# lachinov/brats2019

Measured on AMD Instinct MI355X. Metric: volumes_per_sec_fwd_bwd_128cubed_x4ch, higher is better.
Workload: dtype bf16

## Files before the change

brats2019_amd/_lib.py:

```python
from __future__ import annotations

import ctypes as C
import os

import torch

_PKG = os.path.dirname(os.path.abspath(__file__))
LIB_PATH = os.environ.get("RU_LIB_PATH") or os.path.join(_PKG, "lib", "libresunet_hip.so")

_lib = None
PRECISIONS = {"f32": 0, "bf16x3": 1}
GRAD_PRECISIONS = {"bf16x3": 1, "bf16": 2}
FUSE_GN_BWD_STATS, FUSE_GN_BWD_APPLY, FUSE_SIDE_STREAM, FUSE_BATCH_WREDUCE, FUSE_TAIL_FINALIZE, FUSE_PW_DGRAD = 1, 2, 4, 8, 16, 32

_vp, _f, _d, _i, _sz = C.c_void_p, C.c_float, C.c_double, C.c_int, C.c_size_t

SIGNATURES = {
    "ru_last_error": (C.c_char_p, []),
    "ru_version": (_i, []),
    "ru_device_ok": (_i, []),
    "ru_conv3d_workspace_bytes": (_sz, [_i] * 7),
    "ru_conv3d_fwd": (_i, [_vp, _vp, _vp, _vp] + [_i] * 7 + [_vp, _sz, _vp]),
    "ru_conv3d_bwd_data": (_i, [_vp, _vp, _vp] + [_i] * 7 + [_vp, _sz, _vp]),
    "ru_conv3d_fwd_p": (_i, [_vp, _vp, _vp, _vp] + [_i] * 8 + [_vp, _sz, _vp]),
# ... 65 lines not shown
    "ru_unet_probe": (_i, [_vp, _i]),
    "ru_unet_probe_read": (_i, [_vp, C.POINTER(C.c_double), C.POINTER(_i)]),
    "ru_unet_probe_read_families": (_i, [_vp, C.POINTER(C.c_double), C.POINTER(_i), _i]),
    "ru_unet_param_count": (_i, [_vp]),
    "ru_unet_param_name": (C.c_char_p, [_vp, _i]),
    "ru_unet_param_ndim": (_i, [_vp, _i]),
    "ru_unet_param_dim": (_i, [_vp, _i, _i]),
    "ru_unet_param_offset": (_sz, [_vp, _i]),
    "ru_unet_param_total": (_sz, [_vp]),
    "ru_unet_param_is_dead": (_i, [_vp, _i]),
    "ru_unet_workspace_bytes": (_sz, [_vp] + [_i] * 5),
    "ru_unet_forward": (_i, [_vp, _vp, _vp, _vp] + [_i] * 5 + [_vp, _sz, _vp]),
    "ru_unet_backward": (_i, [_vp] * 6),
    "ru_unet_backward_criterion": (_i, [_vp, _vp, _vp, _vp, _d, _f, _f, _f, _f, _vp, _vp, _vp]),
    "ru_unet_gn_stats": (_i, [_vp, _i, _vp, _vp, _vp]),
    "ru_comm_unique_id": (_i, [_vp]),
    "ru_comm_init": (_i, [C.POINTER(_vp), _vp, _i, _i]),
    "ru_comm_destroy": (_i, [_vp]),
    "ru_comm_rank": (_i, [_vp]),
    "ru_comm_world": (_i, [_vp]),
    "ru_allreduce": (_i, [_vp, _vp, _sz, _i, _vp]),
    "ru_comm_group_begin": (_i, []),
    "ru_comm_group_end": (_i, []),
    "ru_tta_merge": (_i, [_vp, _i, C.c_uint, _vp, _vp, _vp, _i, _i, _i, _i, _vp]),
    "ru_compose_labels": (_i, [_vp, _vp, C.c_ulonglong, _vp, _sz, _vp]),
    "ru_dice_counts": (_i, [_vp, _vp, _vp, _i, _i, _sz, _vp]),
    "ru_dice_accumulate": (_i, [_vp, _vp, _i, _i, _i, _vp]),
    "ru_hausdorff_workspace_bytes": (_sz, [_i] * 6),
    "ru_hausdorff_sq": (_i, [_vp, _vp] + [_i] * 6 + [_vp, _vp, _sz, _vp]),
    "ru_hausdorff_accumulate": (_i, [_vp, _vp] + [_i] * 4 + [_vp]),
    "ru_label_confusion": (_i, [_vp, _vp, _i, _i, _i, _sz, _vp, _vp, _vp]),
    "ru_overlap_accumulate": (_i, [_vp, _i, _i, _i, _i, _vp, _vp, _vp]),
    "ru_dice1d_accumulate": (_i, [_vp, _vp, _i, _i, _i, _vp]),
    "ru_rmse_accumulate": (_i, [_vp, _vp, _vp]),
    "ru_surface_workspace_bytes": (_sz, [_i] * 6),
    "ru_surface_metrics": (_i, [_vp, _vp] + [_i] * 6 + [_d, _vp, _vp, _vp, _sz, _vp]),
    "ru_surface_accumulate": (_i, [_vp, _vp] + [_i] * 4 + [_vp]),
    "ru_lesion_workspace_bytes": (_sz, [_i] * 7),
    "ru_lesion_metrics": (_i, [_vp, _vp] + [_i] * 7 + [C.c_longlong, _d, _vp, _vp, _vp, _i, _vp, _sz, _vp]),
    "ru_lesion_accumulate": (_i, [_vp, _vp] + [_i] * 4 + [_vp]),
    "ru_tile_gather": (_i, [_vp, _vp] + [_i] * 6 + [C.POINTER(_i), _i, _i, _i, _vp]),
    "ru_tile_scatter": (_i, [_vp, _vp] + [_i] * 6 + [C.POINTER(_i), _i, _i, _i, C.POINTER(_i), C.POINTER(_i), _vp]),
    "ru_blend_accumulate": (_i, [_vp, _vp, _vp] + [_i] * 8 + [C.POINTER(_i), _i, C.POINTER(_i), _i, C.POINTER(_i), _i, _i, _i, _vp]),
    "ru_blend_finalize": (_i, [_vp, _vp, _vp] + [_i] * 8 + [C.POINTER(_i), _i, C.POINTER(_i), _i, C.POINTER(_i), _i, _vp]),
    "ru_case_bbox": (_i, [_vp, _vp, _i, _i, _i, _i, _vp]),
    "ru_case_workspace_bytes": (_sz, [_i, _i, _i, _i]),
    "ru_case_stats": (_i, [_vp, _vp, _i, _i, _i, _i, C.POINTER(_i), C.POINTER(_i), _vp, _sz, _vp]),
    "ru_case_prepare": (_i, [_vp, _vp, _vp, _i, _i, _i, _i, C.POINTER(_i), C.POINTER(_i), C.POINTER(_i), C.POINTER(_i), _i, C.c_uint, _vp]),
    "ru_tta_merge_box": (_i, [_vp, _i, C.c_uint, _vp, _vp, _vp, _i, _i, _i, _i, C.POINTER(_i), C.POINTER(_i), _vp]),
    "ru_cc_workspace_bytes": (_sz, [_i, _i, _i]),
    "ru_cc_reject": (_i, [_vp, _i, _i, _i, _d, _vp, _sz, _vp]),
    "ru_paste_labels": (_i, [_vp, _vp, _i, _i, _i, C.POINTER(_i), C.POINTER(_i), _vp]),
    "ru_postprocess_workspace_bytes": (_sz, [_i, _i, _i, _i]),
    "ru_postprocess_regions": (_i, [_vp, _vp, _i, _i, _i, _i, C.POINTER(C.c_longlong), C.POINTER(C.c_ulonglong), C.c_uint, C.c_uint, _i, _vp, _vp, _vp, _vp, _sz, _vp]),
    "ru_ens_accumulate": (_i, [_vp, _i, C.c_uint, _vp, _i, _i, _i, _i, _i, C.POINTER(_i), C.POINTER(_i), _vp]),
    "ru_ens_finalize": (_i, [_vp, _i, _vp, _vp, _vp, _i, _sz, _vp]),
    "ru_ens_accumulate_finalize": (_i, [_vp, _i, C.c_uint, _vp, _i, _i, _vp, _vp, _vp, _i, _i, _i, _i, C.POINTER(_i), C.POINTER(_i), _vp]),
    "ru_ens_argmax": (_i, [_vp, _i, _vp, _i, _sz, _vp]),
    "ru_paste_probs": (_i, [_vp, _vp, _i, _i, _i, _i, C.POINTER(_i), C.POINTER(_i), _vp]),
    "ru_unc_accumulate": (_i, [_vp, _i, C.c_uint, _vp, _vp, _i, _i, _i, _i, _i, C.POINTER(_i), C.POINTER(_i), _vp]),
    "ru_unc_accumulate_finalize": (_i, [_vp, _i, C.c_uint, _vp, _vp, _i, _i, _i, _vp, _vp, _vp, _vp, _i, _i, _i, _i, C.POINTER(_i), C.POINTER(_i), _vp]),
    "ru_unc_finalize": (_i, [_vp, _vp, _i, _i, _i, _vp, _vp, _vp, _vp, _i, _sz, _vp]),
    "ru_unc_histogram": (_i, [_vp, _vp, _vp, _i, _i, _i, _vp, _vp, _vp]),
    "ru_unc_score": (_i, [_vp, C.POINTER(_i), _i, _vp, _vp, _vp]),
    "ru_paste_u8c": (_i, [_vp, _vp, _i, _i, _i, _i, C.POINTER(_i), C.POINTER(_i), _vp]),
    "ru_zscore_workspace_bytes": (_sz, [_i, _sz]),
    "ru_zscore_stats": (_i, [_vp, _vp, _i, _sz, _vp, _sz, _vp]),
    "ru_augment_patch": (_i, [_vp, _vp, _vp, _vp, _i, _i, _i, _i, _vp, _vp, _vp, _i, _vp, _vp, _vp, _vp, _vp]),
    "ru_augment_patch_soft": (_i, [_vp, _vp, _vp, _vp, _vp, _i, _i, _i, _i, _vp, _vp, _vp, _i, _vp, _vp, _vp, _vp, _vp]),
    "ru_augment_patch_affine": (_i, [_vp, _vp, _vp, _vp, _vp, _i, _i, _i, _i, _vp, _vp, _vp, _i, _vp, _vp, _i, _vp, _vp, _vp]),
    "ru_case_probe": (_i, [_vp, _vp, _vp, _i, _i, _i, _i, _vp, _vp]),
    "ru_case_pack": (_i, [_vp, _vp, _vp, _i, _i, _i, _i, _vp, _vp, _i, _vp, _vp, _vp, _vp]),
    "ru_case_unpack": (_i, [_vp, _vp, _vp, _i, _i, _i, _i, _i, _vp, _vp, _vp, _vp, _vp, _vp]),
    "ru_augment_batch_packed": (_i, [_vp, _vp, _i, _vp, _vp, _vp, _vp]),
    "ru_elastic_workspace_bytes": (_sz, [_i, _i, _i]),
    "ru_elastic_noise": (_i, [C.c_ulonglong, _i, _i, _i, _vp, _vp]),
    "ru_elastic_field": (_i, [_vp, _d, _d, _i, _i, _i, _vp, _vp, _sz, _vp]),
    "ru_elastic_warp": (_i, [_vp, _i, _vp, _i, _vp, _i, _i, _i, _i, _vp, _vp, _vp, _vp, _vp]),
    "ru_intensity_workspace_bytes": (_sz, [_i, _i, _i, _i]),
    "ru_intensity_augment": (_i, [_vp, _vp, _i, _i, _i, _i, _vp, _vp, _sz, _vp]),
    "ru_layout_convert": (_i, [_vp, _vp, _i, _i, _sz, _i, _vp]),
    "ru_upsample2x_trilinear_fwd_l": (_i, [_vp, _vp] + [_i] * 5 + [_f, _vp]),
    "ru_upsample2x_trilinear_bwd_l": (_i, [_vp, _vp] + [_i] * 5 + [_vp]),
    "ru_conv3d_fwd_l": (_i, [_vp, _vp, _vp, _vp] + [_i] * 7 + [_vp, _sz, _vp]),
    "ru_conv3d_bwd_weight_l": (_i, [_vp, _vp, _vp] + [_i] * 7 + [_vp, _sz, _vp]),
    "ru_conv1_l_workspace_bytes": (_sz, [_i, _i, _i]),
    "ru_conv1_l": (_i, [_vp, _i, _vp, _i, _vp, _i, _vp, _vp, _i, _vp, _f, _vp, _f, _i, _i, _sz, _i, _i, _i, _i, _vp, _vp, _f, _vp, _sz,
                        C.POINTER(_i), C.POINTER(_i), _vp, _sz, _vp]),
    "ru_conv3_l_workspace_bytes": (_sz, [_i] * 7),
    "ru_conv3_l": (_i, [_vp, _vp, _vp, _vp] + [_i] * 8 + [_vp, _vp, _vp, _f, _vp, _vp, _i, _i, _vp, _vp, _f, _vp, _sz, C.POINTER(_i), C.POINTER(_i), _vp, _sz, _vp, _vp]),
    "ru_gn_finalize_l": (_i, [_vp, _i] + [_vp] * 7 + [_i, _i, _sz, _i, _f, _i, _vp]),
    "ru_gn_apply_l": (_i, [_vp] * 7 + [_i, _i, _sz, _f, _f, _vp]),
    "ru_gn_bwd_finalize_l": (_i, [_vp, _i] + [_vp] * 6 + [_i, _i, _sz, _i, _i, _vp]),
    "ru_gn_bwd_l_nblk": (_i, [_sz]),
    "ru_gn_bwd_l_workspace_bytes": (_sz, [_i, _i, _sz]),
    "ru_gn_bwd_l": (_i, [_vp] * 7 + [_f] + [_vp] * 5 + [_i, _i, _sz, _i, _i, _vp, _sz, _vp]),
    "ru_head_grad_l_workspace_bytes": (_sz, [_i, _i, _sz, _i]),
    "ru_head_grad_l": (_i, [_vp] * 4 + [_d, _f, _f, _f, _f] + [_vp] * 3 + [_i, _i, _sz, _i, _vp, _sz, _vp]),
    "ru_wgrad1_l_workspace_bytes": (_sz, [_i, _i, _i, _sz]),
    "ru_wgrad3_l_workspace_bytes": (_sz, [_i] * 7),
    "ru_wgrad3_l": (_i, [_vp, _vp, _vp] + [_i] * 8 + [_vp, _vp, _f, _i, _i, _vp, _vp, _vp, _vp, _vp, _f, _vp, C.POINTER(_i), _vp, _sz, _vp]),
    "ru_wgrad1_l": (_i, [_vp, _vp, _i, _vp, _vp, _i, _i, _i, _i, _sz] + [_i] * 6 + [_vp, _i, _vp, _vp, _f, C.POINTER(_i), _vp, _sz, _vp]),
}


CRIT_KINDS = {"Dice_loss_joint": 0, "BCE_Loss": 1, "MSE_Loss": 2, "CE_Loss": 3, "Dice1D": 4, "GDL_joint": 5, "sens_loss_joint": 6,
              "Dice_loss_separate": 7}
CRIT_MOMENTS, CRIT_MAX_TERMS = 7, 8
CRIT_MASK_LOGS, CRIT_MASK_ALL = (1 << 4) | (1 << 5), 0x7F
CRIT_M_D2 = 6

CONF_PROB, CONF_LABEL, OVERLAP_MAX_LABELS = 0, 1, 8
OVERLAP_MODES = {"itk": 0, "wt": 1, "validate": 2}

UNC_MEASURES = {"std": 0, "entropy": 1}
UNC_REGIONS, UNC_LEVELS, UNC_CLASSES = 3, 101, 4

SURFACE_PROB, SURFACE_LABEL, SURFACE_REGIONS, SURFACE_COUNTS = 0, 1, 3, 6
SURFACE_COLUMNS = {"dice": 0, "sensitivity": 1, "specificity": 2, "hd95": 3}

LESION_COUNTS, LESION_TABLE_COLUMNS, LESION_CHUNK = 6, 5, 8
LESION_COLUMNS = {"dice": 0, "hd95": 1}

POSTPROCESS_MASKS, POSTPROCESS_LABELS, POSTPROCESS_REGIONS, POSTPROCESS_STATS = 0, 1, 3, 6


INT_BLUR, INT_LOWRES, INT_NOISE, INT_BRIGHTNESS, INT_CONTRAST, INT_GAMMA, INT_GAMMA_INVERT, INT_GAMMA_RETAIN = 1, 2, 4, 8, 16, 32, 64, 128
INT_MAXC, INT_MAX_RADIUS = 8, 8


AFFINE_MAPPINGS = {"default": 0, "row": 1, "brick": 2}


PACK_F32, PACK_U16 = 0, 1
PACK_KINDS = {"float32": PACK_F32, "uint16": PACK_U16}
AUG_ZOOM, AUG_AFFINE = 0, 1
AUG_BATCH_MAX = 8


class FinDesc(C.Structure):
    _fields_ = [("kind", _i), ("G", _i), ("s2_sign", _i), ("keep_ticket", _i), ("eps", _f), ("nblk", _i), ("N", _i), ("C", _i),
                ("gamma", _vp), ("beta", _vp), ("mean", _vp), ("rstd", _vp), ("scale", _vp), ("shift", _vp), ("bst_k", _vp),
                ("coef", _vp), ("dgamma", _vp), ("dbeta", _vp)]


class CaseDesc(C.Structure):
    _fields_ = [("image", _vp), ("label", _vp), ("soft", _vp), ("kind", _i), ("C", _i), ("dims", _i * 3), ("box_lo", _i * 3), ("box_size", _i * 3),
                ("mean", _f * 8), ("inv_std", _f * 8)]


class PatchDesc(C.Structure):
    _fields_ = [("mode", _i), ("flags", _i), ("mapping", _i), ("crop_lo", _i * 3), ("scale", _d * 3), ("matrix", _d * 9), ("offset", _d * 3),
                ("gain", _f * 8), ("bias", _f * 8)]


class IntensityParams(C.Structure):
    _fields_ = [("mask", _i * 8), ("blur_sigma", _d * 8), ("lowres_zoom", _d * 8), ("noise_variance", _d * 8), ("noise_seed", C.c_ulonglong * 8),
                ("brightness", _d * 8), ("contrast", _d * 8), ("gamma", _d * 8)]


class CritTerm(C.Structure):
    _fields_ = [("kind", _i), ("weight", _d), ("priority", _d), ("bg_weight", _d)]


def load():
    global _lib
# ... 57 lines not shown
```

brats2019_amd/csrc/engine.hip:

```cpp
#include "ru_common.h"
#include "arena.hpp"

#include <vector>
#include <math.h>
#include <stdlib.h>
#include <string.h>

#include <string>
#include <type_traits>

namespace ru {

static thread_local char g_err[512] = "";
void set_error(const char* fmt, ...) {
    va_list ap;
    va_start(ap, fmt);
    vsnprintf(g_err, sizeof(g_err), fmt, ap);
    va_end(ap);
}
int hip_fail(hipError_t e, const char* what) {
    set_error("%s: %s", what, hipGetErrorString(e));
    return RU_EHIP;
}

constexpr float kSlope = 1e-2f;
constexpr int kGroups = 8;
constexpr float kEps = 1e-5f;
constexpr int kInCh = 4;

static bool env_is(const char* name, char c) { const char* e = getenv(name); return e && *e == c; }
Switches switches_from_env() {
    Switches sw;
    sw.wz = !env_is("RU_WZ", '0');
    sw.wz32 = !(conv3_wz16_form_built() && env_is("RU_WZ32", '0'));
    sw.mx = !env_is("RU_MX", '0');
    sw.mx_wz = sw.mx && !env_is("RU_MX", '1');
    sw.mxg = !env_is("RU_MXG", '0');
    sw.head_form = !env_is("RU_HEAD_FORM", '0');
    sw.head_res = !env_is("RU_HEAD_RES", '0');
    return sw;
}
bool env_trace() { static const bool on = [] { const char* e = getenv("RU_TRACE"); return e && *e && *e != '0'; }(); return on; }
bool env_f32c_off() { static const bool off = env_is("RU_F32C", '0'); return off; }
bool env_sb1_no22() { static const bool on = env_is("RU_SB1_NO22", '1'); return on; }
int env_c1_scatter_cob() { static const int forced = [] { const char* e = getenv("RU_C1_SCATTER_COB"); return e ? atoi(e) : 0; }(); return forced; }
bool env_c1_pair_off() { static const bool off = env_is("RU_C1_PAIR", '0'); return off; }
unsigned env_fusion(unsigned fusion) {
    if (env_is("RU_SIDE_STREAM", '0')) fusion &= ~(unsigned)RU_FUSE_SIDE_STREAM;
    if (const char* e = getenv("RU_FUSION_OFF")) fusion &= ~(unsigned)strtoul(e, nullptr, 0);
    if (const char* e = getenv("RU_FUSION_ON")) fusion |= (unsigned)strtoul(e, nullptr, 0) & 63u;
    return fusion;
}

static int trace_sync(const char* what, hipStream_t s) {
    fprintf(stderr, "[ru] %s\n", what);
    const hipError_t e = hipStreamSynchronize(s);
    if (e != hipSuccess) { fprintf(stderr, "[ru]   -> %s\n", hipGetErrorString(e)); return hip_fail(e, what); }
    return RU_OK;
}

enum { FAM_CONV_L0 = 0, FAM_CONV_DEEP, FAM_WGRAD_L0, FAM_WGRAD_DEEP, FAM_GN, FAM_PW, FAM_OTHER, FAM_COUNT };
enum { INST_CONV16_FWD = 0, INST_CONV16_DGRAD, INST_CONV_DEEP_FWD, INST_CONV_DEEP_DGRAD, INST_WGRAD16_FUSED, INST_WGRAD16_PLAIN, INST_WGRAD_DEEP, INST_COUNT };
struct FamilySink {
    std::vector<hipEvent_t> ev;
    std::vector<int> fam;
    std::vector<int> inst;
    size_t used = 0;
    ~FamilySink() { for (hipEvent_t e : ev) (void)hipEventDestroy(e); }
};
static thread_local FamilySink* t_sink = nullptr;
static thread_local int t_hint_c = 16;
static thread_local int t_hint_inst = -1;
struct RedQueues { WgradRedList main, side; hipStream_t side_stream = nullptr; };
static thread_local RedQueues* t_red = nullptr;
static WgradRedList* red_for(hipStream_t s) { return t_red ? ((t_red->side_stream && s == t_red->side_stream) ? &t_red->side : &t_red->main) : nullptr; }
static int family_of(const char* call) {
    auto has = [&](const char* k) { return strstr(call, k) != nullptr; };
    if (has("wgrad3_launch")) return t_hint_c <= 16 ? FAM_WGRAD_L0 : FAM_WGRAD_DEEP;
    if (has("wgrad_reduce_flush")) return FAM_WGRAD_DEEP;
    if (has("conv3_launch") || has("conv3_sb_launch")) return t_hint_c <= 16 ? FAM_CONV_L0 : FAM_CONV_DEEP;
    if (has("gn_")) return FAM_GN;
    if (has("conv1_") || has("wgrad1_launch") || has("up2_") || has("s2d_launch") || has("d2s_launch") || has("lrelu_bwd_launch")) return FAM_PW;
    return FAM_OTHER;
}
static void sink_begin(const char* call, hipStream_t s) {
    FamilySink& k = *t_sink;
    while (k.ev.size() < k.used + 2) {
        hipEvent_t e;
        if (hipEventCreate(&e) != hipSuccess) return;
        k.ev.push_back(e);
    }
    if (k.fam.size() < k.ev.size() / 2) { k.fam.resize(k.ev.size() / 2); k.inst.resize(k.ev.size() / 2); }
    k.fam[k.used / 2] = family_of(call);
    k.inst[k.used / 2] = t_hint_inst;
    t_hint_inst = -1;
    (void)hipEventRecord(k.ev[k.used], s);
}
static void sink_end(hipStream_t s) {
    FamilySink& k = *t_sink;
    if (k.ev.size() < k.used + 2) return;
    (void)hipEventRecord(k.ev[k.used + 1], s);
    k.used += 2;
}

template <class F>
static int run_probed(const char* call, hipStream_t s, F&& launch) {
    if (t_sink) sink_begin(call, s);
    const int rc = launch();
    if (t_sink) sink_end(s);
    if (rc != RU_OK) return rc;
    return env_trace() ? trace_sync(call, s) : RU_OK;
}
#define RU_RUN(call) RU_ARENA_RUN(run_probed(#call, s, [&] { return (call); }))

}

using namespace ru;

struct ParamInfo {
    std::string name;
    int ndim;
    int dims[5];
    size_t offset, numel;
    bool dead;
};

struct PackRef { size_t off = 0; unsigned forms = 0; };

struct BlockP {
    int down = -1, conv1 = -1, conv2 = -1, n1w = -1, n1b = -1, n2w = -1, n2b = -1;
    int cin_down = 0, c = 0;
    size_t pk_f1 = 0, pk_f2 = 0, pk_d1 = 0, pk_d2 = 0, pk_downT = 0, pk_down16 = 0;
    PackRef fk_f1, fk_f2, fk_d1, fk_d2;
};

struct GNSave {
    float *mean = nullptr, *rstd = nullptr, *scale = nullptr, *shift = nullptr;
    float act_slope = 0.01f;
    float* k = nullptr;
};

struct BlockSave {
    const BlockP* bp = nullptr;
    const float* xprev = nullptr;
    const BlockSave* xprev_block = nullptr;
    float* xs2d = nullptr;
    const float* x = nullptr;
    const GNSave* xg = nullptr;
    float *y1 = nullptr, *y2 = nullptr, *out = nullptr;
    GNSave g1, g2;
    int N = 0, C = 0, D = 0, H = 0, W = 0;
};

struct DecSave {
    const float* z = nullptr;
    const BlockSave* z_block = nullptr;
    float *u = nullptr, *v = nullptr, *c = nullptr;
    const float* skip = nullptr;
    int level = 0;
};

constexpr int kOneProduct = 0x100;
struct ru_unet {
    int depth = 0, nout = 0;
    std::vector<int> enc, dec, ch;
    std::vector<ParamInfo> params;
    size_t total = 0;
    std::vector<std::vector<BlockP>> enc_blocks, dec_blocks;
    std::vector<BlockP> first_blocks;
    std::vector<int> up_w, dec1_w;
    std::vector<size_t> pk_upT, pk_decT;
    int conv_in = -1, nin_w = -1, nin_b = -1, conv_out_w = -1, conv_out_b = -1;
    size_t pk_in = 0, pk_out = 0, pk_out_d = 0, pk_total = 0;
    PackRef fk_in, fk_out, fk_out_d;
    size_t fk_total = 0;
    void set_pack(Conv3Args& a, const PackRef& r) const { conv3_set_pack(a, fpack + r.off, r.forms); }
    int precision = RU_PREC_F32;
    unsigned fusion = RU_FUSE_GN_BWD_STATS | RU_FUSE_GN_BWD_APPLY | RU_FUSE_SIDE_STREAM | RU_FUSE_BATCH_WREDUCE | RU_FUSE_PW_DGRAD;
    int grad_precision = RU_PREC_BF16X3;
    int grad_products() const { return (precision == RU_PREC_BF16X3 && grad_precision == RU_PREC_BF16) ? 1 : 3; }
    int wgrad_mode() const { return precision | (grad_products() == 1 ? kOneProduct : 0); }
    bool c16 = false;
    char* fpack = nullptr;

    bool have_fwd = false, training = false;
    int N = 0, D = 0, H = 0, W = 0;
    char* ws = nullptr;
    size_t ws_bytes = 0, fwd_end = 0, fwd_keep = 0;
    float* pack = nullptr;
    const float* x_in = nullptr;
    const float* x_in4 = nullptr;
    bool x_in4_planned = false;
    bool params_frozen = false;
    const float* packed_params = nullptr;
    const void* packed_base = nullptr;
    int packed_prec = -1;
    bool packed_c16 = false;
    ru::Switches sw;
    ru::Switches pack_sw;
    float *y0 = nullptr, *t0 = nullptr, *probs = nullptr;
    GNSave g0;
    const float* head_in = nullptr;
    const BlockSave* head_block = nullptr;
    std::vector<BlockSave> first_s;
    std::vector<std::vector<BlockSave>> enc_s, dec_s;
    std::vector<DecSave> dstage;
    std::vector<const float*> skips;
    std::vector<GNSave> gn_order;
    bool probe_on = false;
    bool probe_families = false;
    ru::FamilySink* sink = nullptr;
    std::vector<hipEvent_t> probe_ev;
    size_t probe_used = 0;
    hipStream_t side = nullptr;
    std::vector<hipEvent_t> fork_ev;
    ru::RedQueues red;
    unsigned* tickets = nullptr;
    int ticket_next = 0;
    unsigned* next_ticket() { return tickets ? tickets + (ticket_next++ & 255) : nullptr; }
    bool tails() const { return c16 && (fusion & RU_FUSE_TAIL_FINALIZE) && tickets != nullptr; }
    size_t fork_used = 0;
    ~ru_unet() {
        for (hipEvent_t e : probe_ev) (void)hipEventDestroy(e);
        for (hipEvent_t e : fork_ev) (void)hipEventDestroy(e);
        if (side) (void)hipStreamDestroy(side);
        if (tickets) (void)hipFree(tickets);
        delete sink;
    }
};

static int add_param(ru_unet* h, const std::string& name, std::initializer_list<int> dims, bool dead = false) {
    ParamInfo p;
    p.name = name;
    p.ndim = (int)dims.size();
    size_t n = 1;
    int i = 0;
    for (int d : dims) { p.dims[i++] = d; n *= (size_t)d; }
    for (; i < 5; ++i) p.dims[i] = 1;
    p.offset = h->total;
    p.numel = n;
    p.dead = dead;
    h->total += n;
    h->params.push_back(p);
    return (int)h->params.size() - 1;
}

static BlockP add_block(ru_unet* h, const std::string& prefix, int cin_down, int c, bool dead = false) {
    BlockP b;
    b.c = c;
    b.cin_down = cin_down;
    if (cin_down > 0) b.down = add_param(h, prefix + "downsample.0.weight", {c, cin_down, 2, 2, 2}, dead);
    b.conv1 = add_param(h, prefix + "conv1.conv1.weight", {c, c, 3, 3, 3}, dead);
    b.conv2 = add_param(h, prefix + "conv2.conv1.weight", {c, c, 3, 3, 3}, dead);
    b.n1w = add_param(h, prefix + "norm1.weight", {c}, dead);
    b.n1b = add_param(h, prefix + "norm1.bias", {c}, dead);
    b.n2w = add_param(h, prefix + "norm2.weight", {c}, dead);
    b.n2b = add_param(h, prefix + "norm2.bias", {c}, dead);
    return b;
}

static std::string fmt(const char* f, int a, int b = 0) {
    char buf[128];
    snprintf(buf, sizeof(buf), f, a, b);
    return buf;
}

static void assign_block_packs(ru_unet* h, BlockP& b) {
    const size_t n = conv3_packed_floats(b.c, b.c);
    b.pk_f1 = h->pk_total; h->pk_total += n;
    b.pk_f2 = h->pk_total; h->pk_total += n;
    b.pk_d1 = h->pk_total; h->pk_total += n;
    b.pk_d2 = h->pk_total; h->pk_total += n;
    if (b.down >= 0) {
        b.pk_downT = h->pk_total; h->pk_total += (size_t)8 * b.cin_down * b.c;
        b.pk_down16 = h->pk_total; h->pk_total += (size_t)2 * 8 * b.cin_down * b.c;
    }
    const size_t f = conv3_sb_frag_bytes(b.c, b.c);
    for (PackRef* r : {&b.fk_f1, &b.fk_f2, &b.fk_d1, &b.fk_d2}) { r->off = h->fk_total; h->fk_total += f; }
}

extern "C" ru_unet_t ru_unet_create(int depth, const int* encoder_layers, const int* decoder_layers,
                                    const int* number_of_channels, int number_of_outputs) {
    if (depth < 2 || depth > 8 || !encoder_layers || !decoder_layers || !number_of_channels || number_of_outputs < 1) {
        set_error("ru_unet_create: bad configuration");
        return nullptr;
    }
    for (int i = 0; i < depth; ++i) {
        if (number_of_channels[i] % kGroups != 0 || number_of_channels[i] <= 0 || encoder_layers[i] < 1 || decoder_layers[i] < 1) {
            set_error("ru_unet_create: channels must be positive multiples of 8 (GroupNorm(8, C)) and layer counts >= 1");
            return nullptr;
        }
    }
    ru_unet* h = new ru_unet();
    h->fusion = env_fusion(h->fusion);
    h->depth = depth;
    h->nout = number_of_outputs;
    h->enc.assign(encoder_layers, encoder_layers + depth);
    h->dec.assign(decoder_layers, decoder_layers + depth);
    h->ch.assign(number_of_channels, number_of_channels + depth);
    const std::vector<int>& ch = h->ch;
    h->enc_blocks.resize(depth - 1);
    for (int i = 0; i < depth - 1; ++i)
        for (int j = 0; j < h->enc[i + 1]; ++j)
            h->enc_blocks[i].push_back(add_block(h, fmt("encoder_convs.%d.%d.", i, j), j == 0 ? ch[i] : 0, ch[i + 1]));
    for (int i = 0; i < depth - 1; ++i) h->up_w.push_back(add_param(h, fmt("upsampling.%d.1.weight", i), {ch[i], ch[i + 1], 1, 1, 1}));
    h->dec_blocks.resize(depth);
    for (int i = 0; i < depth; ++i)
        for (int j = 0; j < h->dec[i]; ++j)
            h->dec_blocks[i].push_back(add_block(h, fmt("decoder_convs.%d.%d.", i, j), 0, ch[i], i == depth - 1));
    for (int i = 0; i < depth; ++i)
        h->dec1_w.push_back(add_param(h, fmt("decoder_convs1x1.%d.weight", i), {ch[i], 2 * ch[i], 1, 1, 1}, i == depth - 1));
    h->conv_in = add_param(h, "conv_input.weight", {ch[0], kInCh, 3, 3, 3});
    h->nin_w = add_param(h, "norm_input.weight", {ch[0]});
// ... 282 lines not shown
    for (int i = 0; i < depth; ++i) { Dl[i] = h->D >> i; Hl[i] = h->H >> i; Wl[i] = h->W >> i; }
    auto Vl = [&](int i) { return (size_t)Dl[i] * Hl[i] * Wl[i]; };
    h->gn_order.clear();
    const bool f32c_off = env_f32c_off();
    const bool f32c_fits = (size_t)h->D * h->H * h->W * 64 < ((size_t)1 << 31);
    h->c16 = (h->precision == RU_PREC_BF16X3 || (h->precision == RU_PREC_F32 && !h->training && !f32c_off && f32c_fits)) && (h->W & 3) == 0;
    for (int c : h->ch) h->c16 = h->c16 && (c % 16 == 0);
    h->pack = A.alloc(h->pk_total);
    h->fpack = reinterpret_cast<char*>(A.alloc(h->fk_total / sizeof(float) + 64));
    float* wf4_in = A.alloc(conv3_sb4_frag_bytes(h->ch[0]) / sizeof(float) + 64);
    const bool reuse_packs = h->params_frozen && !h->training && !A.dry && h->packed_params == params && h->packed_base == (const void*)h->pack &&
                             h->packed_prec == h->precision && h->packed_c16 == h->c16;
    int rc = RU_OK;
    if (!reuse_packs) {
        rc = pack_all(h, params, A, s);
        if (rc) return rc;
    }

    const int C0 = h->ch[0];
    const BlockSave* res_block = nullptr;
    h->x_in = x;
    h->x_in4 = nullptr;
    h->x_in4_planned = false;
    h->y0 = A.alloc((size_t)N * C0 * Vl(0));
    const size_t stem_mark = A.off;
    if (h->c16 && h->precision == RU_PREC_BF16X3 && conv3_sb4_usable(N, kInCh, C0, Dl[0], Hl[0], Wl[0])) {
        float* x4 = A.alloc((size_t)N * 4 * Vl(0));
        float* wf4 = wf4_in;
        h->x_in4 = x4;
        h->x_in4_planned = true;
        RU_RUN(pad_to_c4_launch(x, x4, N, kInCh, Vl(0), s));
        if (!reuse_packs) RU_RUN(conv3_sb4_pack_weights(P(h, params, h->conv_in), wf4, kInCh, C0, 0, s));
        rc = conv3_gn(h, A, s, x4, nullptr, wf4, PACK_HAS_SB4, h->y0, nullptr, P(h, params, h->nin_w), P(h, params, h->nin_b), h->g0,
                      N, kInCh, C0, Dl[0], Hl[0], Wl[0], false, true);
    } else {
        rc = conv3_gn(h, A, s, x, h->pack + h->pk_in, h->fpack + h->fk_in.off, h->fk_in.forms, h->y0, nullptr, P(h, params, h->nin_w), P(h, params, h->nin_b), h->g0, N, kInCh, C0, Dl[0], Hl[0], Wl[0], false);
    }
    if (rc) return rc;
    if (!h->training) A.rewind(stem_mark);
    h->g0.act_slope = 1.0f;
    const bool stem_fused = h->c16 && !h->first_blocks.empty() && h->first_blocks[0].down < 0;
    h->t0 = nullptr;
    if (!stem_fused) {
        h->t0 = A.alloc((size_t)N * C0 * Vl(0));
        if (h->c16) RU_RUN(gn_apply16_launch(h->y0, h->g0.scale, h->g0.shift, nullptr, h->t0, N, C0, Vl(0), 1.0f, s));
        else RU_RUN(gn_apply_launch(h->y0, h->g0.scale, h->g0.shift, nullptr, h->t0, N, C0, Vl(0), 1.0f, s));
    }
    const float* cur = stem_fused ? h->y0 : h->t0;
    const BlockSave* cur_block = nullptr;
    h->first_s.assign(h->first_blocks.size(), BlockSave());
    for (size_t j = 0; j < h->first_blocks.size(); ++j) {
        rc = block_fwd(h, params, A, s, h->first_blocks[j], cur, cur_block, N, Dl[0], Hl[0], Wl[0], h->first_s[j], &cur, (stem_fused && j == 0) ? &h->g0 : nullptr);
        if (rc) return rc;
        cur_block = &h->first_s[j];
    }
    h->skips.assign(depth - 1, nullptr);
    h->enc_s.assign(depth - 1, {});
    for (int i = 0; i < depth - 1; ++i) {
        h->skips[i] = cur;
        h->enc_s[i].assign(h->enc_blocks[i].size(), BlockSave());
        for (size_t j = 0; j < h->enc_blocks[i].size(); ++j) {
            const int lv = j == 0 ? i : i + 1;
            rc = block_fwd(h, params, A, s, h->enc_blocks[i][j], cur, cur_block, N, Dl[lv], Hl[lv], Wl[lv], h->enc_s[i][j], &cur);
            if (rc) return rc;
            cur_block = &h->enc_s[i][j];
        }
    }
    h->dstage.assign(depth - 1, DecSave());
    h->dec_s.assign(depth - 1, {});
    for (int i = depth - 2; i >= 0; --i) {
        DecSave& ds = h->dstage[i];
        ds.level = i;
        ds.z = cur;
        ds.z_block = cur_block;
        ds.skip = h->skips[i];
        const int Ci = h->ch[i], Cc = h->ch[i + 1];
        const bool recycle = !h->training;
        float* c_early = recycle ? A.alloc((size_t)N * Ci * Vl(i)) : nullptr;
        const size_t dmark = A.off;
        if (!h->c16) {
            ds.u = A.alloc((size_t)N * Cc * Vl(i));
            RU_RUN(up2_fwd_launch(cur, ds.u, N, Cc, Dl[i + 1], Hl[i + 1], Wl[i + 1], s));
        }
        ds.v = A.alloc((size_t)N * Ci * Vl(i));
        Conv1Args c1{};
        c1.x0 = ds.u; c1.C0 = Cc; c1.y = ds.v; c1.out_slope = kSlope;
        c1.N = N; c1.Cout = Ci; c1.V = Vl(i);
        ds.c = recycle ? c_early : A.alloc((size_t)N * Ci * Vl(i));
        Conv1Args c2{};
        c2.x0 = ds.skip; c2.C0 = Ci; c2.x1 = ds.v; c2.C1 = Ci;
        c2.y = ds.c; c2.out_slope = 1.f; c2.N = N; c2.Cout = Ci; c2.V = Vl(i);
        if (h->c16) {
            float* zc = A.alloc((size_t)N * Ci * Vl(i + 1));
            c1.x0 = cur; c1.y = zc; c1.out_slope = 1.f; c1.V = Vl(i + 1);
            c1.wT = P(h, params, h->up_w[i]); c1.ldw = Cc;
            RU_RUN(conv1_16_launch(c1, s));
            RU_RUN(up2_fwd16_launch(zc, ds.v, N, Ci, Dl[i + 1], Hl[i + 1], Wl[i + 1], kSlope, s));
            c2.wT = P(h, params, h->dec1_w[i]); c2.ldw = 2 * Ci;
            RU_RUN(conv1_16_launch(c2, s));
        } else {
            c1.wT = h->pack + h->pk_upT[i]; c1.ldw = Ci;
            RU_RUN(conv1_launch(c1, s));
            c2.wT = h->pack + h->pk_decT[i]; c2.ldw = Ci;
            RU_RUN(conv1_launch(c2, s));
        }
        if (recycle) A.rewind(dmark);
        cur = ds.c;
        cur_block = nullptr;
        h->dec_s[i].assign(h->dec_blocks[i].size(), BlockSave());
        for (size_t j = 0; j < h->dec_blocks[i].size(); ++j) {
            const bool defer = i == 0 && j + 1 == h->dec_blocks[i].size() && h->c16 &&
                               (h->precision == RU_PREC_BF16X3 ? conv3_sb_head_takes_residual(h->sw, N, C0, h->nout, Dl[0], Hl[0], Wl[0])
                                                               : (!h->training && conv3_f32c_head_takes_residual(h->sw, C0, h->nout, Wl[0])));
            rc = block_fwd(h, params, A, s, h->dec_blocks[i][j], cur, cur_block, N, Dl[i], Hl[i], Wl[i], h->dec_s[i][j], &cur, nullptr, defer);
            if (rc) return rc;
            cur_block = &h->dec_s[i][j];
            if (defer) res_block = cur_block;
        }
    }
    h->head_in = cur;
    h->head_block = cur_block;
    t_hint_c = C0;
    float* pdst = probs_out;
    h->probs = probs_out;
    Conv3Args a{};
    a.x = cur; a.wp = h->pack + h->pk_out; a.bias = P(h, params, h->conv_out_b); a.y = pdst; a.sigmoid = 1;
    a.mode = h->precision; h->set_pack(a, h->fk_out); a.in_c16 = h->c16;
    a.N = N; a.Cin = C0; a.Cout = h->nout; a.D = Dl[0]; a.H = Hl[0]; a.W = Wl[0];
    if (res_block) {
        a.x = res_block->y2; a.in_scale = res_block->g2.scale; a.in_shift = res_block->g2.shift; a.in_slope = kSlope; a.in_res = res_block->x;
        a.in_sum_out = res_block->out;
    }
    RU_RUN(conv3_launch(a, h->sw, s));
    if (!A.dry) { h->packed_params = h->training ? nullptr : params; h->packed_base = h->pack; h->packed_prec = h->precision; h->packed_c16 = h->c16; h->pack_sw = h->sw; }
    return RU_OK;
}

struct NormRef {
    const float* y = nullptr;
    const GNSave* g = nullptr;
    float slope = kSlope;
    const float* gamma = nullptr;
    float *dgamma = nullptr, *dbeta = nullptr;
    int C = 0;
};
static NormRef norm1_of(const ru_unet* h, const float* params, float* grads, const BlockSave& b) {
    return {b.y1, &b.g1, kSlope, P(h, params, b.bp->n1w), G(h, grads, b.bp->n1w), G(h, grads, b.bp->n1b), b.C};
}
static NormRef norm2_of(const ru_unet* h, const float* params, float* grads, const BlockSave& b) {
    return {b.y2, &b.g2, kSlope, P(h, params, b.bp->n2w), G(h, grads, b.bp->n2w), G(h, grads, b.bp->n2b), b.C};
}
static NormRef norm_input_of(const ru_unet* h, const float* params, float* grads) {
    return {h->y0, &h->g0, 1.0f, P(h, params, h->nin_w), G(h, grads, h->nin_w), G(h, grads, h->nin_b), h->ch[0]};
}

struct FusedSums { float* part = nullptr; int nblk = 0; float* coef = nullptr; bool done = false; };
struct Grad { const float* d = nullptr; FusedSums sums; };

static void fill_bwd_tail(ru_unet* h, FinTail& f, const FusedSums& fs, const NormRef& n, size_t V, int s2_sign) {
    f.ticket = h->next_ticket(); f.kind = 2; f.nblk = fs.nblk; f.N = h->N; f.C = n.C; f.G = kGroups; f.V = V; f.eps = kEps; f.s2_sign = s2_sign;
    f.gamma = n.gamma; f.mean = n.g->mean; f.rstd = n.g->rstd; f.coef = fs.coef; f.dgamma = n.dgamma; f.dbeta = n.dbeta;
}

static int bst_nblk(const ru_unet* h, const Conv3Args& a) { return sb_nblk(h, a); }
static int bst_nblk(const ru_unet*, const Conv1Args& a) { return conv1_16_bst_nblk(a); }
template <class Args>
static FusedSums take_bwd_sums(ru_unet* h, Arena& A, Args& a, const NormRef& n, bool may) {
    FusedSums fs;
    if (!may) return fs;
    a.bst_y = n.y; a.bst_k = n.g->k; a.bst_slope = n.slope;
    fs.nblk = bst_nblk(h, a);
    fs.part = A.alloc((size_t)h->N * n.C * fs.nblk * 2);
    fs.coef = A.alloc((size_t)h->N * n.C * 3);
    a.stat_partials = fs.part;
    if constexpr (std::is_same<Args, Conv3Args>::value) {
        if (!A.dry && h->tails()) {
            fill_bwd_tail(h, a.fin, fs, n, (size_t)a.D * a.H * a.W, 1);
            fs.done = true;
        }
    }
// ... 382 lines not shown
            if (rc) return rc;
        }
        if (!joined) {
            const size_t n = (size_t)N * h->ch[i] * level_voxels(h, i);
            float* sum = A.alloc(n);
            RU_RUN(add_launch(g.d, dskip[i], sum, n, s));
            g = Grad{sum};
        }
    }
    for (int j = (int)h->first_s.size() - 1; j >= 0; --j) {
        const NormRef prev = fed_by(h->first_s[j]);
        rc = block_bwd(h, params, grads, A, s, h->first_s[j], g, &prev);
        if (rc) return rc;
    }
    rc = stem_bwd(h, params, grads, dx_in, A, s, g);
    if (rc) return rc;
    if (t_red && !t_red->side.e.empty()) RU_RUN(wgrad_reduce_flush(t_red->side, h->side));
    if (!A.dry) { rc = side_join(h, s); if (rc) return rc; }
    if (t_red && !t_red->main.e.empty()) RU_RUN(wgrad_reduce_flush(t_red->main, s));
    return RU_OK;
}

static int check_dims(ru_unet* h, int N, int D, int H, int W) {
    const int m = 1 << (h->depth - 1);
    RU_REQUIRE(N > 0 && D > 0 && H > 0 && W > 0, "ru_unet: bad extents");
    RU_REQUIRE(D % m == 0 && H % m == 0 && W % m == 0, "ru_unet: D,H,W must be divisible by %d (model.py:361 stride-2 convs)", m);
    return RU_OK;
}

extern "C" size_t ru_unet_workspace_bytes(ru_unet_t h, int N, int D, int H, int W, int training) {
    if (!h || check_dims(h, N, D, H, W) != RU_OK) return 0;
    ru_unet tmp = *h;
    tmp.probe_ev.clear();
    tmp.probe_on = false;
    tmp.sink = nullptr;
    tmp.side = nullptr;
    tmp.tickets = nullptr;
    tmp.fork_ev.clear();
    tmp.N = N; tmp.D = D; tmp.H = H; tmp.W = W; tmp.training = training != 0;
    tmp.sw = switches_from_env();
    Arena A;
    A.dry = true;
    if (unet_forward_impl(&tmp, nullptr, nullptr, nullptr, A, nullptr) != RU_OK) return 0;
    if (training) {
        if (unet_backward_impl(&tmp, nullptr, nullptr, nullptr, (float*)1, A, nullptr) != RU_OK) return 0;
    }
    return A.need() + 4096;
}

extern "C" int ru_unet_forward(ru_unet_t h, const float* params, const float* x, float* probs, int N, int D, int H, int W, int training,
                               void* ws, size_t ws_bytes, ru_stream_t stream) {
    RU_REQUIRE(h && params && x && probs && ws, "ru_unet_forward: null argument");
    int rc = check_dims(h, N, D, H, W);
    if (rc) return rc;
    h->have_fwd = false;
    h->sw = switches_from_env();
    h->N = N; h->D = D; h->H = H; h->W = W; h->training = training != 0;
    h->ws = (char*)ws; h->ws_bytes = ws_bytes;
    Arena A;
    A.dry = false; A.base = (char*)ws; A.cap = ws_bytes;
    if (!h->tickets && (h->fusion & RU_FUSE_TAIL_FINALIZE)) {
        hipError_t e = hipMalloc((void**)&h->tickets, 256 * sizeof(unsigned));
        if (e != hipSuccess) { h->tickets = nullptr; return hip_fail(e, "ru_unet_forward: ticket words"); }
    }
    if (h->tickets && (h->fusion & RU_FUSE_TAIL_FINALIZE)) {
        hipError_t e = hipMemsetAsync(h->tickets, 0, 256 * sizeof(unsigned), (hipStream_t)stream);
        if (e != hipSuccess) return hip_fail(e, "ru_unet_forward: ticket words");
    }
    h->ticket_next = 0;
    ru::t_sink = h->probe_families ? h->sink : nullptr;
    rc = unet_forward_impl(h, params, x, probs, A, (hipStream_t)stream);
    ru::t_sink = nullptr;
    if (rc) return rc;
    if (A.failed) { set_error("ru_unet_forward: workspace too small (%zu bytes given)", ws_bytes); return RU_ENOMEM; }
    h->fwd_end = A.off;
    h->fwd_keep = A.keep;
    h->have_fwd = true;
    return RU_OK;
}

static int backward_entry(ru_unet_t h, const float* params, const float* dprobs, const CritGradArgs* crit, float* grads, float* dx, ru_stream_t stream) {
    if (!h->have_fwd || !h->training) { set_error("ru_unet_backward: needs a preceding training-mode ru_unet_forward"); return RU_ESTATE; }
    h->sw = switches_from_env();
    RU_REQUIRE(h->precision != RU_PREC_BF16X3 || h->pack_sw.pack_bits() == h->sw.pack_bits(),
               "ru_unet_backward: RU_WZ / RU_MX / RU_MXG changed since the forward whose packs this backward reads (signature %d then, %d now)", h->pack_sw.pack_bits(), h->sw.pack_bits());
    Arena A;
    A.dry = false; A.base = h->ws; A.cap = h->ws_bytes; A.off = h->fwd_end; A.keep = h->fwd_keep;
    ru::t_sink = h->probe_families ? h->sink : nullptr;
    h->red.main.e.clear();
    h->red.side.e.clear();
    ru::t_red = (h->fusion & RU_FUSE_BATCH_WREDUCE) && !env_trace() ? &h->red : nullptr;
    int rc = unet_backward_impl(h, params, dprobs, grads, dx, A, (hipStream_t)stream, crit);
    ru::t_red = nullptr;
    ru::t_sink = nullptr;
    if (rc && h->side) {
        (void)side_join(h, (hipStream_t)stream);
        h->fork_used = 0;
    }
    if (rc) return rc;
    if (A.failed) { set_error("ru_unet_backward: workspace too small"); return RU_ENOMEM; }
    return RU_OK;
}
extern "C" int ru_unet_backward_criterion(ru_unet_t h, const float* params, const float* target, const double* sums, double count,
                                          float w_dice, float w_bce, float bg_weight, float priority, float* grads, float* dx, ru_stream_t stream) {
    RU_REQUIRE(h && params && target && sums && grads && count > 0.0, "ru_unet_backward_criterion: null argument");
    const CritGradArgs cg{target, sums, count, w_dice, w_bce, bg_weight, priority};
    return backward_entry(h, params, nullptr, &cg, grads, dx, stream);
}

extern "C" int ru_unet_backward(ru_unet_t h, const float* params, const float* dprobs, float* grads, float* dx, ru_stream_t stream) {
    RU_REQUIRE(h && params && dprobs && grads, "ru_unet_backward: null argument");
    return backward_entry(h, params, dprobs, nullptr, grads, dx, stream);
}

extern "C" int ru_unet_gn_stats(ru_unet_t h, int idx, float* mean, float* rstd, ru_stream_t stream) {
    RU_REQUIRE(h && h->have_fwd, "ru_unet_gn_stats: no forward state");
    if (idx < 0) return (int)h->gn_order.size();
    RU_REQUIRE(idx < (int)h->gn_order.size() && mean && rstd, "ru_unet_gn_stats: bad index");
    const size_t bytes = (size_t)h->N * kGroups * sizeof(float);
    hipError_t e = hipMemcpyAsync(mean, h->gn_order[idx].mean, bytes, hipMemcpyDeviceToDevice, (hipStream_t)stream);
    if (e == hipSuccess) e = hipMemcpyAsync(rstd, h->gn_order[idx].rstd, bytes, hipMemcpyDeviceToDevice, (hipStream_t)stream);
    if (e != hipSuccess) return hip_fail(e, "ru_unet_gn_stats");
    return RU_OK;
}

extern "C" const char* ru_last_error(void) { return g_err; }
extern "C" int ru_version(void) { return 100; }
extern "C" int ru_device_ok(void) {
    int n = 0;
    return (hipGetDeviceCount(&n) == hipSuccess && n > 0) ? 1 : 0;
}
```

brats2019_amd/csrc/op_abi.hip:

```cpp
#include "ru_common.h"
#include "arena.hpp"

#include <math.h>

namespace ru {

__global__ void gn_scale_shift_kernel(const float* __restrict__ gamma, const float* __restrict__ beta, const float* __restrict__ mean,
                                      const float* __restrict__ rstd, float* __restrict__ scale, float* __restrict__ shift, int N, int C, int G) {
    const int i = blockIdx.x * blockDim.x + threadIdx.x;
    if (i >= N * C) return;
    const int n = i / C, c = i % C, g = c / (C / G);
    const float a = gamma[c] * rstd[n * G + g];
    scale[i] = a;
    shift[i] = beta[c] - mean[n * G + g] * a;
}
static int gn_scale_shift_launch(const float* gamma, const float* beta, const float* mean, const float* rstd, float* scale, float* shift, int N, int C, int G, hipStream_t s) {
    hipLaunchKernelGGL(gn_scale_shift_kernel, dim3(cdiv(N * C, 256)), dim3(256), 0, s, gamma, beta, mean, rstd, scale, shift, N, C, G);
    RU_CHECK_LAUNCH("gn_scale_shift_kernel");
    return RU_OK;
}

}

using namespace ru;
// ... 249 lines not shown
extern "C" int ru_groupnorm_bwd(const float* x, const float* gamma, const float* beta, const float* mean, const float* rstd, const float* dy,
                                float* dx, float* dgamma, float* dbeta, int N, int C, size_t V, int G, float slope,
                                void* ws, size_t ws_bytes, ru_stream_t stream) {
    RU_REQUIRE(x && gamma && beta && mean && rstd && dy && dx, "ru_groupnorm_bwd: null argument");
    RU_REQUIRE(C % G == 0, "ru_groupnorm_bwd: C %% G != 0");
    Arena A = arena_over(ws, ws_bytes);
    return walk_result(A, groupnorm_bwd_walk(x, gamma, beta, mean, rstd, dy, dx, dgamma, dbeta, N, C, V, G, slope, A, (hipStream_t)stream));
}

extern "C" int ru_leaky_relu_fwd(const float* x, float* y, size_t n, float slope, ru_stream_t stream) { return lrelu_fwd_launch(x, y, n, slope, (hipStream_t)stream); }
extern "C" int ru_leaky_relu_bwd(const float* y, const float* dy, float* dx, size_t n, float slope, ru_stream_t stream) { return lrelu_bwd_launch(y, dy, dx, n, slope, (hipStream_t)stream); }
extern "C" int ru_upsample2x_trilinear_fwd(const float* x, float* y, int N, int C, int D, int H, int W, ru_stream_t stream) { return up2_fwd_launch(x, y, N, C, D, H, W, (hipStream_t)stream); }
extern "C" int ru_upsample2x_trilinear_bwd(const float* dy, float* dx, int N, int C, int D, int H, int W, ru_stream_t stream) { return up2_bwd_launch(dy, dx, N, C, D, H, W, (hipStream_t)stream); }
extern "C" int ru_sigmoid_fwd(const float* x, float* y, size_t n, ru_stream_t stream) { return sigmoid_launch(x, y, n, (hipStream_t)stream); }

extern "C" size_t ru_criterion_workspace_bytes(int N, int C, size_t V) { return 4096 + (size_t)N * C * crit_tiles(V) * 3 * sizeof(float); }
extern "C" int ru_criterion_sums(const float* p, const float* g, double* sums, int N, int C, size_t V, float bg_weight, void* ws, size_t ws_bytes, ru_stream_t stream) {
    RU_REQUIRE(p && g && sums, "ru_criterion_sums: null argument");
    return crit_sums_launch(p, g, sums, N, C, V, bg_weight, ws, ws_bytes, (hipStream_t)stream);
}
extern "C" int ru_criterion_grad(const float* p, const float* g, const double* sums, double count, float w_dice, float w_bce, float bg_weight,
                                 float priority, float* dp, int N, int C, size_t V, ru_stream_t stream) {
    RU_REQUIRE(p && g && sums && dp && count > 0, "ru_criterion_grad: bad argument");
    return crit_grad_launch(p, g, sums, count, w_dice, w_bce, bg_weight, priority, dp, N, C, V, (hipStream_t)stream);
}
extern "C" int ru_criterion_value(const double* sums_host, int C, double count, double priority, double* dice, double* bce) {
    RU_REQUIRE(sums_host && C > 0 && count > 0, "ru_criterion_value: bad argument");
    double acc = 0.0;
    for (int c = 0; c < C; ++c) acc += 2.0 * (sums_host[c] + 1e-6) / (sums_host[C + c] + 2e-6);
    if (dice) *dice = priority * (1.0 - acc / C);
    if (bce) *bce = -sums_host[2 * C] / count;
    return RU_OK;
}
extern "C" int ru_criterion_value_device(const double* sums, int C, double count, double priority, double w_dice, double w_bce, double* out3,
                                         ru_stream_t stream) {
    RU_REQUIRE(sums && out3 && C > 0 && C <= 64 && count > 0, "ru_criterion_value_device: bad argument");
    return crit_value_launch(sums, C, count, priority, w_dice, w_bce, out3, (hipStream_t)stream);
}
extern "C" int ru_adam_amsgrad_step(float* w, const float* g, float* m, float* v, float* vmax, size_t n, float lr, float beta1, float beta2,
                                    float eps, float weight_decay, int step, ru_stream_t stream) {
    RU_REQUIRE(w && g && m && v && vmax, "ru_adam_amsgrad_step: null argument");
    return adam_launch(w, g, m, v, vmax, n, lr, beta1, beta2, eps, weight_decay, step, (hipStream_t)stream);
}

extern "C" int ru_adam_step(float* w, const float* g, float* m, float* v, float* vmax_or_null, size_t n, float lr, float beta1, float beta2,
                            float eps, float weight_decay, int step, ru_stream_t stream) {
    RU_REQUIRE(w && g && m && v, "ru_adam_step: null argument");
    return adam_launch(w, g, m, v, vmax_or_null, n, lr, beta1, beta2, eps, weight_decay, step, (hipStream_t)stream);
}

extern "C" int ru_tta_merge(const float* probs, int K, unsigned flips, float* mean_out, unsigned char* mask, unsigned long long* counts,
                            int C, int D, int H, int W, ru_stream_t stream) {
    RU_REQUIRE(probs && mask && counts, "ru_tta_merge: null argument");
    return tta_merge_launch(probs, K, flips, mean_out, mask, counts, C, D, H, W, (hipStream_t)stream);
}
extern "C" int ru_compose_labels(const unsigned char* mask, const unsigned long long* counts, unsigned long long et_min, unsigned char* labels,
                                 size_t V, ru_stream_t stream) {
    RU_REQUIRE(mask && counts && labels, "ru_compose_labels: null argument");
    return compose_labels_launch(mask, counts, et_min, labels, V, (hipStream_t)stream);
}

extern "C" int ru_dice_accumulate(const unsigned long long* counts, double* acc, int N, int C, int nacc, ru_stream_t stream) {
    return dice_accumulate_launch(counts, acc, N, C, nacc, (hipStream_t)stream);
}
extern "C" int ru_dice_counts(const float* p, const float* g, unsigned long long* counts, int N, int C, size_t V, ru_stream_t stream) {
    RU_REQUIRE(p && g && counts && N > 0 && C > 0, "ru_dice_counts: bad argument");
    return dice_counts_launch(p, g, counts, N * C, V, (hipStream_t)stream);
}

extern "C" int ru_layout_convert(const float* src, float* dst, int N, int C, size_t V, int to_c16, ru_stream_t stream) {
    RU_REQUIRE(src && dst && N > 0, "ru_layout_convert: bad argument");
    return layout_convert_launch(src, dst, N, C, V, to_c16, (hipStream_t)stream);
}

extern "C" int ru_upsample2x_trilinear_fwd_l(const float* x, float* y, int N, int C, int D, int H, int W, float out_slope, ru_stream_t stream) {
    RU_REQUIRE(x && y && N > 0 && C > 0 && D > 0 && H > 0 && W > 0, "ru_upsample2x_trilinear_fwd_l: bad argument");
    return up2_fwd16_launch(x, y, N, C, D, H, W, out_slope, (hipStream_t)stream);
}
extern "C" int ru_upsample2x_trilinear_bwd_l(const float* dy, float* dx, int N, int C, int D, int H, int W, ru_stream_t stream) {
    RU_REQUIRE(dy && dx && N > 0 && C > 0 && D > 0 && H > 0 && W > 0, "ru_upsample2x_trilinear_bwd_l: bad argument");
    return up2_bwd16_launch(dy, dx, N, C, D, H, W, (hipStream_t)stream);
}

static void fill_fin(FinTail& f, const ru_fin_desc& d, unsigned* ticket, int nblk, int N, int C, size_t V) {
    f.ticket = ticket; f.kind = d.kind; f.nblk = d.nblk ? d.nblk : nblk; f.N = d.N ? d.N : N; f.C = d.C ? d.C : C; f.G = d.G; f.V = V; f.eps = d.eps; f.s2_sign = d.s2_sign;
    f.gamma = d.gamma; f.beta = d.beta; f.mean = d.mean; f.rstd = d.rstd; f.scale = d.scale; f.shift = d.shift; f.bst_k = d.bst_k;
    f.coef = d.coef; f.dgamma = d.dgamma; f.dbeta = d.dbeta;
}
static int fin_desc_check(const char* who, const ru_fin_desc& d, int C) {
    RU_REQUIRE(d.kind == 1 || d.kind == 2, "%s: the tail's kind is 1 (statistics) or 2 (GroupNorm-backward sums)", who);
    RU_REQUIRE(d.G > 0 && C % d.G == 0, "%s: the tail needs G groups with C %% G == 0", who);
    RU_REQUIRE(d.gamma && d.mean && d.rstd, "%s: the tail needs gamma, mean and rstd", who);
    RU_REQUIRE(d.kind != 1 || (d.beta && d.scale && d.shift), "%s: a kind-1 tail needs beta, scale and shift", who);
    RU_REQUIRE(d.kind != 2 || d.coef, "%s: a kind-2 tail needs coef", who);
    return RU_OK;
}
static int conv3_l_walk(const char* who, Conv3Args a, const float* w, int flags, int weight_mode, size_t stat_floats, int* nblk, int* route, Arena& A, hipStream_t s,
                        const ru_fin_desc* fd = nullptr) {
    const Switches sw = switches_from_env();
    const int N = a.N, Cin = a.Cin, Cout = a.Cout, D = a.D, H = a.H, W = a.W;
    const bool f32 = (flags & 16) != 0;
    void* wf = A.alloc((f32 ? conv3_f32c_frag_bytes(Cin, Cout) : conv3_sb_frag_bytes(Cin, Cout)) / 4 + 64);
    if (flags & 32) a.products = 2;
    RU_REQUIRE(!f32 || ((flags & 3) != 0 && !(flags & (4 | 8))), "%s: the exact-f32 form needs a voxel-major side and takes neither the 4-channel copy nor a split-form input", who);
    const bool gop = (flags & 64) && !f32 && (flags & 3) == 3 && !(flags & (4 | 8)) && !a.bias && conv3_mxg_usable(sw, N, Cin, Cout, D, H, W);
    const int Cin_f = weight_mode ? Cout : Cin, Cout_f = weight_mode ? Cin : Cout;
    a.mode = f32 ? RU_PREC_F32 : RU_PREC_BF16X3;
    a.in_c16 = flags & 1; a.out_c16 = (flags >> 1) & 1;
    int forms = PACK_ALL | (gop ? PACK_MX_GRAD : 0);
    if (flags & 128) {
        Conv3Args fwd{};
        fwd.mode = a.mode; fwd.N = N; fwd.Cin = Cin; fwd.Cout = Cout; fwd.D = D; fwd.H = H; fwd.W = W;
        fwd.in_c16 = a.in_c16; fwd.out_c16 = a.out_c16; fwd.products = a.products;
        forms = sb_pack_forms(sw, weight_mode) | ((weight_mode == 0 && conv3_route_skips_direct(conv3_sb_route(fwd, sw))) ? PACK_SKIP_DIRECT : 0);
    }
    unsigned wforms = 0;
    RU_ARENA_RUN(f32 ? conv3_f32c_pack_weights(w, wf, Cin_f, Cout_f, weight_mode, s) : conv3_sb_pack_weights(w, wf, Cin_f, Cout_f, weight_mode, s, forms, &wforms));
    conv3_set_pack(a, wf, wforms);
    a.in_s16 = (flags >> 3) & 1;
    RU_REQUIRE(!a.in_s16 || a.in_c16, "%s: the split form is a voxel-major layout", who);
    if (gop) {
        const size_t nvox = (size_t)N * D * H * W;
        float* g16 = A.alloc(nvox * 16);
        RU_ARENA_RUN(conv3_mxg_split_launch(a.x, g16, nvox, s));
        a.x = g16; a.in_s16 = 1; a.in_g16 = 1; a.products = 0;
    }
    if (flags & 4) {
        RU_REQUIRE(!(flags & 1) && conv3_sb4_usable(N, Cin, Cout, D, H, W), "%s: shape does not fit the 4-channel kernel", who);
        const size_t V = (size_t)D * H * W;
        float* x4 = A.alloc((size_t)N * 4 * V);
        void* wf4 = A.alloc(conv3_sb4_frag_bytes(Cout) / 4 + 64);
        RU_ARENA_RUN(pad_to_c4_launch(a.x, x4, N, Cin, V, s));
        RU_ARENA_RUN(conv3_sb4_pack_weights(w, wf4, Cin_f, Cout_f, weight_mode, s));
        a.x = x4; conv3_set_pack(a, wf4, PACK_HAS_SB4); a.in_c4 = 1;
    }
    unsigned* ticket = (fd || (flags & 256)) ? reinterpret_cast<unsigned*>(A.alloc(64)) : nullptr;
    if (route || nblk || a.stat_partials) {
        const int r = f32 ? conv3_f32c_route(a) : conv3_sb_route(a, sw);
        if (route) *route = r;
        const int nb = f32 ? conv3_f32c_tiles_per_sample(N, Cin, Cout, D, H, W) : conv3_sb_route_nblk(r, N, Cout, D, H, W);
        if (nblk) *nblk = nb;
        RU_REQUIRE(!a.stat_partials || stat_floats >= (size_t)N * Cout * nb * 2, "%s: statistics buffer too small", who);
        if (fd && a.stat_partials && !A.dry && !A.failed) fill_fin(a.fin, *fd, ticket, nb, N, Cout, (size_t)D * H * W);
    }
    if (fd && !fd->keep_ticket) RU_ARENA_RUN(fill_launch(reinterpret_cast<float*>(ticket), 0.f, 1, s));
    RU_ARENA_RUN(f32 ? conv3_launch(a, sw, s) : conv3_sb_launch(a, sw, s));
    return RU_OK;
}
static size_t conv3_l_need(int N, int Cin, int Cout, int D, int H, int W, int flags) {
    Conv3Args a{};
    a.N = N; a.Cin = Cin; a.Cout = Cout; a.D = D; a.H = H; a.W = W;
    return dry_need([&](Arena& A) { return conv3_l_walk("ru_conv3_l", a, nullptr, flags, 0, 0, nullptr, nullptr, A, nullptr); });
}
extern "C" size_t ru_conv3_l_workspace_bytes(int N, int Cin, int Cout, int D, int H, int W, int flags) { return kSlack + conv3_l_need(N, Cin, Cout, D, H, W, flags); }

extern "C" int ru_conv3_l(const float* x, const float* w, const float* bias, float* y, int N, int Cin, int Cout, int D, int H, int W, int flags, int weight_mode,
                          const float* add, const float* in_scale, const float* in_shift, float in_slope, const float* in_res, float* in_sum_out,
                          int sigmoid, int products, const float* bst_y, const float* bst_k, float bst_slope, float* stat_partials, size_t stat_floats,
                          int* nblk, int* route, void* ws, size_t ws_bytes, ru_stream_t stream, const ru_fin_desc* fin) {
    RU_REQUIRE(x && w && y, "ru_conv3_l: null argument");
    RU_REQUIRE(!fin || stat_partials, "ru_conv3_l: the tail finalizes the statistics of this launch (stat_partials)");
    if (fin) { const int rc = fin_desc_check("ru_conv3_l", *fin, Cout); if (rc) return rc; }
    RU_REQUIRE(N > 0 && Cin > 0 && Cout > 0 && D > 0 && H > 0 && W > 0, "ru_conv3_l: bad shape");
    RU_REQUIRE(weight_mode == 0 || weight_mode == 1, "ru_conv3_l: weight_mode is 0 (forward packing) or 1 (data-gradient packing)");
    Conv3Args a{};
    a.x = x; a.bias = bias; a.y = y; a.N = N; a.Cin = Cin; a.Cout = Cout; a.D = D; a.H = H; a.W = W;
// ... 89 lines not shown
}
extern "C" int ru_gn_bwd_l_nblk(size_t V) { return gn_bwd_tiles16(V); }
extern "C" size_t ru_gn_bwd_l_workspace_bytes(int N, int C, size_t V) {
    return kSlack + dry_need([&](Arena& A) { return gn_bwd_l_walk(nullptr, nullptr, nullptr, nullptr, nullptr, nullptr, nullptr, 1.f, nullptr, nullptr, nullptr, nullptr, nullptr,
                                                                  N, C, V, 8, 0, A, nullptr); });
}
extern "C" int ru_gn_bwd_l(const float* x, const float* dact, const float* gamma, const float* scale, const float* shift, const float* mean, const float* rstd, float slope,
                           float* dx, float* dgamma, float* dbeta, float* coef_out, float* partials_out, int N, int C, size_t V, int G, int flags,
                           void* ws, size_t ws_bytes, ru_stream_t stream) {
    RU_REQUIRE(x && dact && gamma && scale && shift && mean && rstd && (dx || (flags & 4)), "ru_gn_bwd_l: null argument");
    RU_REQUIRE(N > 0 && C > 0 && G > 0 && V > 0, "ru_gn_bwd_l: bad shape");
    Arena A = arena_over(ws, ws_bytes);
    return walk_result(A, gn_bwd_l_walk(x, dact, gamma, scale, shift, mean, rstd, slope, dx, dgamma, dbeta, coef_out, partials_out, N, C, V, G, flags, A, (hipStream_t)stream));
}

static int head_grad_l_walk(const float* p, const float* dp, const CritGradArgs& cg, float* d4, float* db, float* dlog, int N, int C, size_t V, int route,
                            Arena& A, hipStream_t s) {
    const size_t wsb = bias_grad_workspace_bytes(N, C, V);
    float* wsp = A.alloc(wsb / sizeof(float) + 1);
    if (route == 1) {
        RU_ARENA_RUN(head_grad_c4_crit_launch(p, cg, d4, db, N, C, V, wsp, wsb, s));
    } else if (route == 0) {
        RU_ARENA_RUN(head_grad_c4_launch(p, dp, d4, db, N, C, V, wsp, wsb, s));
        if (dlog) RU_ARENA_RUN(sigmoid_bwd_launch(p, dp, dlog, (size_t)N * C * V, s));
    } else {
        RU_ARENA_RUN(sigmoid_bwd_launch(p, dp, dlog, (size_t)N * C * V, s));
        RU_ARENA_RUN(bias_grad_launch(dlog, db, N, C, V, wsp, wsb, s));
    }
    return RU_OK;
}
extern "C" size_t ru_head_grad_l_workspace_bytes(int N, int C, size_t V, int route) {
    return kSlack + dry_need([&](Arena& A) { return head_grad_l_walk(nullptr, nullptr, CritGradArgs{}, nullptr, nullptr, nullptr, N, C, V, route, A, nullptr); });
}
extern "C" int ru_head_grad_l(const float* p, const float* dp, const float* target, const double* sums, double count, float w_dice, float w_bce, float bg_weight,
                              float priority, float* d4, float* db, float* dlog, int N, int C, size_t V, int route, void* ws, size_t ws_bytes, ru_stream_t stream) {
    RU_REQUIRE(route >= 0 && route <= 2, "ru_head_grad_l: route is 0 (4-channel pass), 1 (4-channel pass with the criterion) or 2 (sigmoid backward, then bias gradient)");
    RU_REQUIRE(p && db && (route == 1 || dp) && (route == 2 ? dlog != nullptr : d4 != nullptr), "ru_head_grad_l: null argument");
    RU_REQUIRE(route != 1 || (!dlog && count > 0), "ru_head_grad_l: the criterion route writes no dlog and needs a positive count");
    RU_REQUIRE(N > 0 && C > 0 && V > 0, "ru_head_grad_l: bad shape");
    const CritGradArgs cg{target, sums, count, w_dice, w_bce, bg_weight, priority};
    Arena A = arena_over(ws, ws_bytes);
    return walk_result(A, head_grad_l_walk(p, dp, cg, d4, db, dlog, N, C, V, route, A, (hipStream_t)stream));
}

static int conv1_l_walk(Conv1Args a, const float* w, size_t stat_floats, int* nblk, int* inst, Arena& A, hipStream_t s) {
    if (a.s2d) {
        const int co = a.s2d == 1 ? a.Cout : a.C0, ci = (a.s2d == 1 ? a.C0 : a.Cout) / 8;
        float* wd = A.alloc((size_t)8 * ci * co);
        float* wdT = A.alloc((size_t)8 * ci * co);
        RU_ARENA_RUN(pack_down16_launch(w, wd, wdT, co, ci, s));
        a.wT = a.s2d == 1 ? wd : wdT;
        a.ldw = a.C0;
    }
    if (inst) *inst = conv1_16_choose(a).packed();
    if (nblk) *nblk = 0;
    if (a.bst_y) {
        const int nb = conv1_16_bst_nblk(a);
        RU_REQUIRE(nb == 0 || (a.stat_partials && stat_floats >= (size_t)a.N * (a.s2d == 2 ? a.Cout / 8 : a.Cout) * nb * 2), "ru_conv1_l: statistics buffer too small");
        if (nblk) *nblk = nb;
    }
    RU_ARENA_RUN(conv1_16_launch(a, s));
    return RU_OK;
}
extern "C" size_t ru_conv1_l_workspace_bytes(int C0, int Cout, int s2d) {
    Conv1Args a{};
    a.C0 = C0; a.Cout = Cout; a.s2d = s2d;
    return kSlack + dry_need([&](Arena& A) { return conv1_l_walk(a, nullptr, 0, nullptr, nullptr, A, nullptr); });
}
extern "C" int ru_conv1_l(const float* x0, int C0, const float* x1, int C1, const float* w, int ldw, float* y, float* y1, int Cout0,
                          const float* add, float out_slope, const float* mask, float mask_slope, int N, int Cout, size_t V,
                          int s2d, int Dc, int Hc, int Wc, const float* bst_y, const float* bst_k, float bst_slope,
                          float* stat_partials, size_t stat_floats, int* nblk, int* inst, void* ws, size_t ws_bytes, ru_stream_t stream) {
    RU_REQUIRE(x0 && w && y, "ru_conv1_l: null argument");
    RU_REQUIRE(s2d >= 0 && s2d <= 2, "ru_conv1_l: s2d is 0 (plain), 1 (gather) or 2 (scatter)");
    RU_REQUIRE(!s2d || (C0 > 0 && Cout > 0 && (s2d == 1 ? C0 : Cout) % 8 == 0), "ru_conv1_l: stride-2 modes need 8 x channels on the gathered side");
    Conv1Args a{};
    a.x0 = x0; a.C0 = C0; a.x1 = x1; a.C1 = C1; a.wT = w; a.ldw = ldw; a.y = y; a.add = add; a.out_slope = out_slope;
    a.N = N; a.Cout = Cout; a.V = V; a.s2d = s2d; a.Dc = Dc; a.Hc = Hc; a.Wc = Wc; a.mask = mask; a.mask_slope = mask_slope;
    a.y1 = y1; a.Cout0 = Cout0; a.bst_y = bst_y; a.bst_k = bst_k; a.bst_slope = bst_slope; a.stat_partials = stat_partials;
    Arena A = arena_over(ws, ws_bytes);
    return walk_result(A, conv1_l_walk(a, w, stat_floats, nblk, inst, A, (hipStream_t)stream));
}

static int wgrad1_l_walk(Wgrad1Args a, int* inst, Arena& A, hipStream_t s) {
    a.ws_bytes = wgrad1_workspace_bytes(a.N, a.Cin, a.Cout, a.V);
    a.ws = A.alloc(a.ws_bytes / 4);
    if (inst) *inst = wgrad1_inst(a);
    RU_ARENA_RUN(wgrad1_launch(a, s));
    return RU_OK;
}
extern "C" size_t ru_wgrad1_l_workspace_bytes(int N, int Cin, int Cout, size_t V) {
    Wgrad1Args a{};
    a.N = N; a.Cin = Cin; a.Cout = Cout; a.V = V;
    return kSlack + dry_need([&](Arena& A) { return wgrad1_l_walk(a, nullptr, A, nullptr); });
}
extern "C" int ru_wgrad1_l(const float* x, const float* x1, int C0, const float* dy, float* dw, int ldw, int N, int Cin, int Cout, size_t V,
                           int c16, int s2d, int Dc, int Hc, int Wc, int tap_split, const float* dg_w, int dg_ldw, float* dg_y0, float* dg_y1,
                           float dg_mask_slope, int* inst, void* ws, size_t ws_bytes, ru_stream_t stream) {
    RU_REQUIRE(x && dy && dw, "ru_wgrad1_l: null argument");
    RU_REQUIRE(N > 0 && Cin > 0 && Cout > 0 && V > 0, "ru_wgrad1_l: bad shape");
    Wgrad1Args a{};
    a.x = x; a.x1 = x1; a.C0 = C0; a.dy = dy; a.dw = dw; a.ldw = ldw; a.N = N; a.Cin = Cin; a.Cout = Cout; a.V = V;
    a.c16 = c16; a.s2d = s2d; a.Dc = Dc; a.Hc = Hc; a.Wc = Wc; a.tap_split = tap_split;
    a.dg_w = dg_w; a.dg_ldw = dg_ldw; a.dg_y0 = dg_y0; a.dg_y1 = dg_y1; a.dg_mask_slope = dg_mask_slope;
    Arena A = arena_over(ws, ws_bytes);
    return walk_result(A, wgrad1_l_walk(a, inst, A, (hipStream_t)stream));
}

static int wgrad3_l_walk(Wgrad3Args a, int flags, int* inst, Arena& A, hipStream_t s) {
    a.ws_bytes = wgrad3_tr_workspace_bytes(a.N, a.Cin, a.Cout, a.D, a.H, a.W);
    a.ws = A.alloc(a.ws_bytes / 4);
    const size_t V = (size_t)a.D * a.H * a.W;
    if (a.x_c4) {
        float* c4 = A.alloc((size_t)a.N * 4 * V);
        RU_ARENA_RUN(pad_to_c4_launch(a.x, c4, a.N, a.dw_cin, V, s));
        a.x = c4;
    }
    if (a.dy_c4) {
        float* c4 = A.alloc((size_t)a.N * 4 * V);
        RU_ARENA_RUN(pad_to_c4_launch(a.dy, c4, a.N, a.dw_cout, V, s));
        a.dy = c4;
    }
    if (inst) *inst = wgrad3_tr_inst(a);
    WgradRedList own;
    if (flags & 32) a.defer = &own;
    RU_ARENA_RUN(wgrad3_tr_launch(a, s));
    if (flags & 32) RU_ARENA_RUN(wgrad_reduce_flush(own, s));
    return RU_OK;
}
extern "C" size_t ru_wgrad3_l_workspace_bytes(int N, int Cin, int Cout, int D, int H, int W, int flags) {
    Wgrad3Args a{};
    a.N = N; a.Cin = Cin; a.Cout = Cout; a.D = D; a.H = H; a.W = W; a.x_c4 = (flags >> 1) & 1; a.dy_c4 = (flags >> 2) & 1;
    return kSlack + dry_need([&](Arena& A) { return wgrad3_l_walk(a, flags, nullptr, A, nullptr); });
}
extern "C" int ru_wgrad3_l(const float* x, const float* dy, float* dw, int N, int Cin, int Cout, int D, int H, int W, int flags, int products,
                           const float* in_scale, const float* in_shift, float in_slope, int dw_cin, int dw_cout,
                           const float* gb_y, const float* gb_d, const float* gb_scale, const float* gb_shift, const float* gb_coef, float gb_slope, float* gb_out,
                           int* inst, void* ws, size_t ws_bytes, ru_stream_t stream) {
    RU_REQUIRE(x && (dy || gb_y) && dw, "ru_wgrad3_l: null argument");
    RU_REQUIRE(N > 0 && Cin > 0 && Cout > 0 && D > 0 && H > 0 && W > 0, "ru_wgrad3_l: bad shape");
    RU_REQUIRE((!(flags & 2) || (dw_cin > 0 && dw_cin <= 4)) && (!(flags & 4) || (dw_cout > 0 && dw_cout <= 4 && dy)),
               "ru_wgrad3_l: a 4-channel copy holds 1..4 channels (dw_cin / dw_cout)");
    Wgrad3Args a{};
    a.x = x; a.dy = dy ? dy : gb_y; a.dw = dw; a.mode = RU_PREC_BF16X3; a.x_c16 = 1; a.dy_c16 = 1;
    a.N = N; a.Cin = Cin; a.Cout = Cout; a.D = D; a.H = H; a.W = W;
    a.in_scale = in_scale; a.in_shift = in_shift; a.in_slope = in_slope; a.dw_cin = dw_cin; a.dw_cout = dw_cout;
    a.dy_s16 = flags & 1; a.x_c4 = (flags >> 1) & 1; a.dy_c4 = (flags >> 2) & 1; a.swapped = (flags >> 3) & 1; a.gb_g16 = (flags >> 4) & 1; a.products = products;
    a.gb_y = gb_y; a.gb_d = gb_d; a.gb_scale = gb_scale; a.gb_shift = gb_shift; a.gb_coef = gb_coef; a.gb_slope = gb_slope; a.gb_out = gb_out;
    Arena A = arena_over(ws, ws_bytes);
    return walk_result(A, wgrad3_l_walk(a, flags, inst, A, (hipStream_t)stream));
}

extern "C" size_t ru_zscore_workspace_bytes(int C, size_t V) { return zscore_workspace_bytes(C, V) + 256; }
extern "C" int ru_zscore_stats(const float* image, double* stats, int C, size_t V, void* ws, size_t ws_bytes, ru_stream_t stream) {
    RU_REQUIRE(image && stats && C > 0 && V > 0, "ru_zscore_stats: bad argument");
    return zscore_stats_launch(image, stats, C, V, ws, ws_bytes, (hipStream_t)stream);
}
static int augment_patch_impl(const float* image, const unsigned char* label, const float* soft, const float* mean, const float* inv_std, int C, int D, int H, int W,
                              const int* crop_lo, const int* patch, const double* scale, int flags, const float* gain, const float* bias,
                              float* data_out, float* target_out, ru_stream_t stream) {
    RU_REQUIRE(image && (label || soft) && mean && inv_std && crop_lo && patch && scale && gain && bias && data_out && target_out, "ru_augment_patch: null argument");
    RU_REQUIRE(C > 0 && C <= RU_AUG_MAXC, "ru_augment_patch: 1..%d channels", RU_AUG_MAXC);
    const int dims[3] = {D, H, W};
    AugmentArgs a{};
    a.image = image; a.label = label; a.soft = soft; a.data = data_out; a.target = target_out; a.C = C; a.D = D; a.H = H; a.W = W; a.flags = flags;
    for (int i = 0; i < 3; ++i) {
// ... 22 lines not shown
```

brats2019_amd/csrc/pointwise_c16.hip:

```cpp
#include "pw_helpers.hpp"
#include "fin_tail.hpp"
#include <type_traits>
#include <stdlib.h>

namespace ru {

typedef float f32x4_c16 __attribute__((ext_vector_type(4)));
template <int I, int N, class F> __device__ __forceinline__ void static_for_c1_impl(F&& f) {
    if constexpr (I < N) { f(std::integral_constant<int, I>{}); static_for_c1_impl<I + 1, N>(f); }
}
template <int N, class F> __device__ __forceinline__ void static_for_c1(F&& f) { static_for_c1_impl<0, N>(f); }

static inline dim3 c16_grid(size_t V, int blocks_nc, unsigned cap = 2048) {
    size_t bx = (V * 4 + 255) / 256;
    if (bx > cap) bx = cap;
    if (bx < 1) bx = 1;
    return dim3((unsigned)bx, (unsigned)blocks_nc);
}

template <int RES, bool NT = false>
__global__ __launch_bounds__(256) void gn_apply16_kernel(const float* __restrict__ x, const float* __restrict__ scale, const float* __restrict__ shift,
                                                         const float* __restrict__ res, float* __restrict__ y, int C, size_t V, float slope,
                                                         const float* __restrict__ rscale, const float* __restrict__ rshift, float rslope) {
    const int nb = blockIdx.y, CB = C >> 4;
// ... 115 lines not shown
    const int nb = blockIdx.y, CB = C >> 4;
    const int n = nb / CB, cb = nb - n * CB;
    const int q = threadIdx.x & 3;
    const size_t row = (size_t)n * C + cb * 16 + 4 * q;
    float a[4], b[4], cA[4], cB[4], cC[4];
#pragma unroll
    for (int k = 0; k < 4; ++k) {
        a[k] = scale[row + k]; b[k] = shift[row + k];
        cA[k] = coef[(row + k) * 3]; cB[k] = coef[(row + k) * 3 + 1]; cC[k] = coef[(row + k) * 3 + 2];
    }
    const size_t base = (size_t)nb * V * 4, F = V * 4;
    const float4* xp = reinterpret_cast<const float4*>(x) + base;
    const float4* dp = reinterpret_cast<const float4*>(dy) + base;
    float4* op = reinterpret_cast<float4*>(dx) + base;
    for (size_t f = (size_t)blockIdx.x * 256 + threadIdx.x; f < F; f += (size_t)gridDim.x * 256) {
        const float4 t = xp[f], d = dp[f];
        float4 o;
        o.x = cA[0] * ((t.x * a[0] + b[0]) > 0.f ? d.x : d.x * slope) + (cB[0] * t.x + cC[0]);
        o.y = cA[1] * ((t.y * a[1] + b[1]) > 0.f ? d.y : d.y * slope) + (cB[1] * t.y + cC[1]);
        o.z = cA[2] * ((t.z * a[2] + b[2]) > 0.f ? d.z : d.z * slope) + (cB[2] * t.z + cC[2]);
        o.w = cA[3] * ((t.w * a[3] + b[3]) > 0.f ? d.w : d.w * slope) + (cB[3] * t.w + cC[3]);
        op[f] = o;
    }
}
__global__ __launch_bounds__(256) void gn_bwd_apply16_split_kernel(const float* __restrict__ x, const float* __restrict__ dy, const float* __restrict__ scale,
                                                                   const float* __restrict__ shift, const float* __restrict__ coef, float slope,
                                                                   float* __restrict__ dx, int C, size_t V) {
    const int nb = blockIdx.y, CB = C >> 4;
    const int n = nb / CB, cb = nb - n * CB;
    const int hf = threadIdx.x & 1;
    const size_t row = (size_t)n * C + cb * 16 + 8 * hf;
    float a[8], b[8], cA[8], cB[8], cC[8];
#pragma unroll
    for (int k = 0; k < 8; ++k) {
        a[k] = scale[row + k]; b[k] = shift[row + k];
        cA[k] = coef[(row + k) * 3]; cB[k] = coef[(row + k) * 3 + 1]; cC[k] = coef[(row + k) * 3 + 2];
    }
    const size_t base = (size_t)nb * V * 4, F = V * 2;
    const float4* xp = reinterpret_cast<const float4*>(x) + base;
    const float4* dp = reinterpret_cast<const float4*>(dy) + base;
    pw_u32x4* op = reinterpret_cast<pw_u32x4*>(dx) + base;
    for (size_t f = (size_t)blockIdx.x * 256 + threadIdx.x; f < F; f += (size_t)gridDim.x * 256) {
        const size_t v = f >> 1;
        const float4 t0 = xp[v * 4 + 2 * hf], t1 = xp[v * 4 + 2 * hf + 1], d0 = dp[v * 4 + 2 * hf], d1 = dp[v * 4 + 2 * hf + 1];
        const float tx[8] = {t0.x, t0.y, t0.z, t0.w, t1.x, t1.y, t1.z, t1.w}, dd[8] = {d0.x, d0.y, d0.z, d0.w, d1.x, d1.y, d1.z, d1.w};
        float o[8];
#pragma unroll
        for (int k = 0; k < 8; ++k) o[k] = cA[k] * ((tx[k] * a[k] + b[k]) > 0.f ? dd[k] : dd[k] * slope) + (cB[k] * tx[k] + cC[k]);
        pw_u32x4 hi, lo;
        pw_split8(o, hi, lo);
        op[v * 4 + hf] = hi;
        op[v * 4 + 2 + hf] = lo;
    }
}
int gn_bwd_apply16_launch(const float* x, const float* dy, const float* scale, const float* shift, const float* coef, float slope, float* dx,
                          int N, int C, size_t V, int split, hipStream_t s) {
    RU_REQUIRE(C % 16 == 0, "gn_bwd_apply16: C must be a multiple of 16");
    if (split) {
        size_t bx = (V * 2 + 255) / 256;
        if (bx > 2048) bx = 2048;
        hipLaunchKernelGGL(gn_bwd_apply16_split_kernel, dim3((unsigned)bx, (unsigned)(N * (C / 16))), dim3(256), 0, s, x, dy, scale, shift, coef, slope, dx, C, V);
    } else {
        hipLaunchKernelGGL(gn_bwd_apply16_kernel, c16_grid(V, N * (C / 16)), dim3(256), 0, s, x, dy, scale, shift, coef, slope, dx, C, V);
    }
    RU_CHECK_LAUNCH("gn_bwd_apply16_kernel");
    return RU_OK;
}

__global__ __launch_bounds__(256) void up2_fwd16_kernel(const float* __restrict__ x, float* __restrict__ y, int D, int H, int W, float slope) {
    const int Do = 2 * D, Ho = 2 * H, Wo = 2 * W;
    const size_t nb = blockIdx.y;
    const size_t Vi = (size_t)D * H * W, Vo = Vi * 8;
    const float4* xp = reinterpret_cast<const float4*>(x) + nb * Vi * 4;
    float4* yp = reinterpret_cast<float4*>(y) + nb * Vo * 4;
    const bool nt_out = (size_t)gridDim.y * Vo * 16 * sizeof(float) >= ((size_t)128 << 20);
    const size_t total = (size_t)(D + 1) * (H + 1) * Wo * 4;
    for (size_t f = (size_t)blockIdx.x * 256 + threadIdx.x; f < total; f += (size_t)gridDim.x * 256) {
        const int q = (int)(f & 3);
        size_t r = f >> 2;
        const int xo = (int)(r % Wo); r /= Wo;
        const int ky = (int)(r % (H + 1)) - 1;
        const int kz = (int)(r / (H + 1)) - 1;
        int x0, x1; float lx0, lx1;
        up2_src(xo, W, x0, x1, lx0, lx1);
        const int zA = kz < 0 ? 0 : kz, zB = kz + 1 > D - 1 ? D - 1 : kz + 1;
        const int yA = ky < 0 ? 0 : ky, yB = ky + 1 > H - 1 ? H - 1 : ky + 1;
        const size_t rAA = ((size_t)zA * H + yA) * W, rAB = ((size_t)zA * H + yB) * W, rBA = ((size_t)zB * H + yA) * W, rBB = ((size_t)zB * H + yB) * W;
        const float4 a00 = xp[(rAA + x0) * 4 + q], b00 = xp[(rAA + x1) * 4 + q];
        const float4 a01 = xp[(rAB + x0) * 4 + q], b01 = xp[(rAB + x1) * 4 + q];
        const float4 a10 = xp[(rBA + x0) * 4 + q], b10 = xp[(rBA + x1) * 4 + q];
        const float4 a11 = xp[(rBB + x0) * 4 + q], b11 = xp[(rBB + x1) * 4 + q];
        float4 e00, e01, e10, e11;
#define RU_UPX(c) e00.c = lx0 * a00.c + lx1 * b00.c; e01.c = lx0 * a01.c + lx1 * b01.c; e10.c = lx0 * a10.c + lx1 * b10.c; e11.c = lx0 * a11.c + lx1 * b11.c
        RU_UPX(x); RU_UPX(y); RU_UPX(z); RU_UPX(w);
#undef RU_UPX
#pragma unroll
        for (int dz = 0; dz < 2; ++dz) {
            const int zo = 2 * kz + 1 + dz;
            if (zo < 0 || zo >= Do) continue;
            int z0, z1; float lz0, lz1;
            up2_src(zo, D, z0, z1, lz0, lz1);
#pragma unroll
            for (int dy = 0; dy < 2; ++dy) {
                const int yo = 2 * ky + 1 + dy;
                if (yo < 0 || yo >= Ho) continue;
                int y0, y1; float ly0, ly1;
                up2_src(yo, H, y0, y1, ly0, ly1);
                float4 o;
#define RU_UP2(c) o.c = lrelu(lz0 * (ly0 * e00.c + ly1 * e01.c) + lz1 * (ly0 * e10.c + ly1 * e11.c), slope)
                RU_UP2(x); RU_UP2(y); RU_UP2(z); RU_UP2(w);
#undef RU_UP2
                if (nt_out) __builtin_nontemporal_store(f32x4_c16{o.x, o.y, o.z, o.w}, reinterpret_cast<f32x4_c16*>(yp + (((size_t)zo * Ho + yo) * Wo + xo) * 4 + q));
                else yp[(((size_t)zo * Ho + yo) * Wo + xo) * 4 + q] = o;
            }
        }
    }
}
int up2_fwd16_launch(const float* x, float* y, int N, int C, int D, int H, int W, float slope, hipStream_t s) {
    RU_REQUIRE(C % 16 == 0, "up2_fwd16: C must be a multiple of 16");
    const size_t total = (size_t)(D + 1) * (H + 1) * (2 * W) * 4;
    size_t bx = (total + 255) / 256;
    if (bx > 16384) bx = 16384;
    hipLaunchKernelGGL(up2_fwd16_kernel, dim3((unsigned)bx, (unsigned)(N * (C / 16))), dim3(256), 0, s, x, y, D, H, W, slope);
    RU_CHECK_LAUNCH("up2_fwd16_kernel");
    return RU_OK;
}

#ifndef RU_UP2B_ZC
#define RU_UP2B_ZC 8
#endif
constexpr int UP2B_ZC = RU_UP2B_ZC;
__global__ __launch_bounds__(256) void up2_bwd16_kernel(const float* __restrict__ dy, float* __restrict__ dx, int D, int H, int W) {
    const int Do = 2 * D, Ho = 2 * H, Wo = 2 * W;
    const size_t nb = blockIdx.y;
    const size_t Vi = (size_t)D * H * W, Vo = Vi * 8;
    const float4* dp = reinterpret_cast<const float4*>(dy) + nb * Vo * 4;
    float4* op = reinterpret_cast<float4*>(dx) + nb * Vi * 4;
    const int nch = (D + UP2B_ZC - 1) / UP2B_ZC;
    const size_t total = (size_t)nch * H * W * 4;
    for (size_t f = (size_t)blockIdx.x * 256 + threadIdx.x; f < total; f += (size_t)gridDim.x * 256) {
        const int q = (int)(f & 3);
        size_t r = f >> 2;
        const int kx = (int)(r % W); r /= W;
        const int ky = (int)(r % H);
        const int k0 = (int)(r / H) * UP2B_ZC;
        const int k1 = k0 + UP2B_ZC < D ? k0 + UP2B_ZC : D;
        float wy[4], wx[4];
        size_t oy[4], ox[4];
#pragma unroll
        for (int t = 0; t < 4; ++t) {
            const int y = 2 * ky - 1 + t, xx = 2 * kx - 1 + t;
            wy[t] = (y >= 0 && y < Ho) ? up2_coef(y, H, ky) : 0.f;
            wx[t] = (xx >= 0 && xx < Wo) ? up2_coef(xx, W, kx) : 0.f;
            oy[t] = (size_t)(y < 0 ? 0 : (y >= Ho ? Ho - 1 : y)) * Wo;
            ox[t] = (size_t)(xx < 0 ? 0 : (xx >= Wo ? Wo - 1 : xx)) * 4 + q;
        }
        float4 accP = make_float4(0.f, 0.f, 0.f, 0.f), accC = accP;
        for (int m = k0; m <= k1; ++m) {
#pragma unroll
            for (int h = 0; h < 2; ++h) {
                const int z = 2 * m - 1 + h;
                const bool in = z >= 0 && z < Do;
                const size_t zrow = (size_t)(z < 0 ? 0 : (z >= Do ? Do - 1 : z)) * Ho * Wo;
                float4 pz = make_float4(0.f, 0.f, 0.f, 0.f);
#pragma unroll
                for (int b = 0; b < 4; ++b) {
                    const float4* row = dp + (zrow + oy[b]) * 4;
                    const float4 p0 = row[ox[0]], p1 = row[ox[1]], p2 = row[ox[2]], p3 = row[ox[3]];
                    pz.x += wy[b] * (wx[0] * p0.x + wx[1] * p1.x + wx[2] * p2.x + wx[3] * p3.x);
                    pz.y += wy[b] * (wx[0] * p0.y + wx[1] * p1.y + wx[2] * p2.y + wx[3] * p3.y);
                    pz.z += wy[b] * (wx[0] * p0.z + wx[1] * p1.z + wx[2] * p2.z + wx[3] * p3.z);
                    pz.w += wy[b] * (wx[0] * p0.w + wx[1] * p1.w + wx[2] * p2.w + wx[3] * p3.w);
                }
                const float cP = (in && m - 1 >= k0) ? up2_coef(z, D, m - 1) : 0.f;
                const float cC = (in && m < k1) ? up2_coef(z, D, m) : 0.f;
                accP.x += cP * pz.x; accP.y += cP * pz.y; accP.z += cP * pz.z; accP.w += cP * pz.w;
                accC.x += cC * pz.x; accC.y += cC * pz.y; accC.z += cC * pz.z; accC.w += cC * pz.w;
            }
            if (m - 1 >= k0) op[(((size_t)(m - 1) * H + ky) * W + kx) * 4 + q] = accP;
            accP = accC;
            accC = make_float4(0.f, 0.f, 0.f, 0.f);
        }
    }
}
int up2_bwd16_launch(const float* dy, float* dx, int N, int C, int D, int H, int W, hipStream_t s) {
    RU_REQUIRE(C % 16 == 0, "up2_bwd16: C must be a multiple of 16");
    const size_t total = (size_t)((D + UP2B_ZC - 1) / UP2B_ZC) * H * W * 4;
    size_t bx = (total + 255) / 256;
    if (bx > 16384) bx = 16384;
    hipLaunchKernelGGL(up2_bwd16_kernel, dim3((unsigned)bx, (unsigned)(N * (C / 16))), dim3(256), 0, s, dy, dx, D, H, W);
    RU_CHECK_LAUNCH("up2_bwd16_kernel");
    return RU_OK;
}

__global__ void pack_down16_kernel(const float* __restrict__ w, float* __restrict__ wd, float* __restrict__ wdT, int Cout, int Cin) {
    const int i = blockIdx.x * blockDim.x + threadIdx.x;
    if (i >= Cout * Cin * 8) return;
    const int tap = i & 7, c = (i >> 3) % Cin, o = i / (8 * Cin);
    const float v = w[i];
    wd[(size_t)o * 8 * Cin + tap * Cin + c] = v;
    wdT[(size_t)(tap * Cin + c) * Cout + o] = v;
}
int pack_down16_launch(const float* w, float* wd, float* wdT, int Cout, int Cin, hipStream_t s) {
    const int total = Cout * Cin * 8;
    hipLaunchKernelGGL(pack_down16_kernel, dim3(cdiv(total, 256)), dim3(256), 0, s, w, wd, wdT, Cout, Cin);
    RU_CHECK_LAUNCH("pack_down16_kernel");
    return RU_OK;
}

template <int COB, int S2D, int NSLOT, bool PAIR = false>
__global__ __launch_bounds__(256, (PAIR || NSLOT > 0) ? 2 : 1) void conv1_16_kernel(const Conv1Args a, int nvt) {
    static_assert(!PAIR || (S2D == 2 && COB == 4 && (NSLOT == 1 || NSLOT == 2)), "paired stores: the scatter mode with statistics, four blocks per workgroup");
    constexpr bool BST = NSLOT > 0;
    constexpr int NSL = BST ? NSLOT : 1;
    __shared__ float red[BST ? 4 * NSL * 16 * 2 : 1];
    const int lane = threadIdx.x & 63, wave = threadIdx.x >> 6;
    const int n = blockIdx.z, cog = blockIdx.y;
    const size_t V = a.V;
    const int r = lane & 15, g = lane >> 4;
    const int nkb0 = a.C0 >> 4, nkb1 = a.C1 >> 4, nkb = nkb0 + nkb1, CBo = a.Cout >> 4;
    const int Hf = 2 * a.Hc, Wf = 2 * a.Wc;
    const size_t Vf = V * 8;
    const int CBf_out = CBo >> 3;
    const int Cstat = S2D == 2 ? (a.Cout >> 3) : a.Cout;
    f32x4_c16 bs1[NSL], bs2[NSL], bk[NSL][3];
    if constexpr (BST) {
#pragma unroll
        for (int sl = 0; sl < NSL; ++sl) {
            bs1[sl] = f32x4_c16{0.f, 0.f, 0.f, 0.f}; bs2[sl] = f32x4_c16{0.f, 0.f, 0.f, 0.f};
            const int cob = cog * COB + sl, chb = S2D == 2 ? cob % CBf_out : cob;
            const float* kp = a.bst_k + (size_t)n * 3 * Cstat + (cob < CBo ? chb : 0) * 16 + 4 * g;
#pragma unroll
            for (int t3 = 0; t3 < 3; ++t3) { const float4 q = *reinterpret_cast<const float4*>(kp + (size_t)t3 * Cstat); bk[sl][t3] = f32x4_c16{q.x, q.y, q.z, q.w}; }
        }
    }
    const bool nt_out = (size_t)a.N * a.Cout * V * sizeof(float) >= ((size_t)128 << 20);
    const int vt = blockIdx.x * 4 + wave;
    const bool live = vt < nvt;
    if (!live) { if constexpr (!BST) return; }
    if (live) {
    const size_t v0 = (size_t)vt * 64;
    size_t vb[4], fv[4];
#pragma unroll
    for (int t = 0; t < 4; ++t) {
        size_t v = v0 + 16 * t + r;
        if (v >= V) v = V - 1;
        vb[t] = v * 16 + 4 * g;
        fv[t] = 0;
        if constexpr (S2D != 0) {
            const int xc = (int)(v % a.Wc);
            const size_t rr = v / a.Wc;
            const int yc = (int)(rr % a.Hc), zc = (int)(rr / a.Hc);
            fv[t] = ((size_t)(2 * zc) * Hf + 2 * yc) * Wf + 2 * xc;
        }
    }
    const float* wrow[COB];
#pragma unroll
    for (int cb = 0; cb < COB; ++cb) {
        const int cob = cog * COB + cb;
        wrow[cb] = a.wT + (size_t)((cob < CBo ? cob : CBo - 1) * 16 + r) * a.ldw + 4 * g;
    }
    f32x4_c16 acc[4][COB];
#pragma unroll
    for (int t = 0; t < 4; ++t)
#pragma unroll
        for (int cb = 0; cb < COB; ++cb) acc[t][cb] = f32x4_c16{0.f, 0.f, 0.f, 0.f};
    const int CBf_in = nkb0 >> 3;
    auto kstep = [&](int kb) __attribute__((always_inline)) {
        float4 xb[4];
        if constexpr (S2D == 1) {
            const int tap = kb / CBf_in, cbf = kb - tap * CBf_in;
            const size_t toff = ((size_t)(tap >> 2) * Hf + ((tap >> 1) & 1)) * Wf + (tap & 1);
            const float* src = a.x0 + ((size_t)(n * CBf_in + cbf) * Vf) * 16 + 4 * g;
#pragma unroll
            for (int t = 0; t < 4; ++t) xb[t] = *reinterpret_cast<const float4*>(src + (fv[t] + toff) * 16);
        } else {
            const float* src = kb < nkb0 ? a.x0 + ((size_t)(n * nkb0 + kb) * V) * 16 : a.x1 + ((size_t)(n * nkb1 + kb - nkb0) * V) * 16;
#pragma unroll
            for (int t = 0; t < 4; ++t) xb[t] = *reinterpret_cast<const float4*>(src + vb[t]);
        }
#pragma unroll
        for (int cb = 0; cb < COB; ++cb) {
            const float4 wv = *reinterpret_cast<const float4*>(wrow[cb] + kb * 16);
#pragma unroll
            for (int t = 0; t < 4; ++t) {
                acc[t][cb] = __builtin_amdgcn_mfma_f32_16x16x4f32(wv.x, xb[t].x, acc[t][cb], 0, 0, 0);
                acc[t][cb] = __builtin_amdgcn_mfma_f32_16x16x4f32(wv.y, xb[t].y, acc[t][cb], 0, 0, 0);
                acc[t][cb] = __builtin_amdgcn_mfma_f32_16x16x4f32(wv.z, xb[t].z, acc[t][cb], 0, 0, 0);
                acc[t][cb] = __builtin_amdgcn_mfma_f32_16x16x4f32(wv.w, xb[t].w, acc[t][cb], 0, 0, 0);
            }
        }
    };
    int kb = 0;
    for (; kb + 1 < nkb; kb += 2) { kstep(kb); kstep(kb + 1); }
    if (kb < nkb) kstep(kb);
    if constexpr (PAIR) {
        const int k = r & 1;
        constexpr int CBf = NSLOT;
        const bool has_add = a.add != nullptr;
        const float* addp = has_add ? a.add : a.bst_y;
#pragma unroll
        for (int t = 0; t < 4; ++t) {
            size_t idx[2][2];
            bool ok[2];
            int srcl[2];
            float4 dadd[2][2], dyq[2][2];
#pragma unroll
            for (int h = 0; h < 2; ++h) {
                srcl[h] = 16 * g + 8 * h + (r >> 1);
                ok[h] = v0 + 16 * t + 8 * h + (r >> 1) < V;
                const unsigned flo = __shfl((unsigned)(fv[t] & 0xffffffffu), srcl[h]), fhi = __shfl((unsigned)(fv[t] >> 32), srcl[h]);
                const size_t fvs = ((size_t)fhi << 32) | flo;
#pragma unroll
                for (int pa = 0; pa < 2; ++pa) {
                    const int cbA = CBf == 1 ? 2 * pa : pa;
                    const int cobA = cog * COB + cbA, tapA = cobA / CBf, cbf = cobA - tapA * CBf;
                    const size_t toff = ((size_t)(tapA >> 2) * Hf + ((tapA >> 1) & 1)) * Wf + k;
                    idx[h][pa] = ((size_t)(n * CBf + cbf) * Vf + fvs + toff) * 16 + 4 * g;
                }
            }
#pragma unroll
            for (int h = 0; h < 2; ++h)
#pragma unroll
                for (int pa = 0; pa < 2; ++pa) {
                    dadd[h][pa] = *reinterpret_cast<const float4*>(addp + idx[h][pa]);
                    dyq[h][pa] = *reinterpret_cast<const float4*>(a.bst_y + idx[h][pa]);
                }
#pragma unroll
            for (int h = 0; h < 2; ++h) {
#pragma unroll
                for (int pa = 0; pa < 2; ++pa) {
                    const int cbA = CBf == 1 ? 2 * pa : pa, cbB = CBf == 1 ? 2 * pa + 1 : pa + 2;
                    f32x4_c16 o4;
#pragma unroll
                    for (int e = 0; e < 4; ++e) {
                        const float va = __shfl(acc[t][cbA][e], srcl[h]), vb = __shfl(acc[t][cbB][e], srcl[h]);
                        o4[e] = k ? vb : va;
                    }
                    float4 o = make_float4(lrelu(o4[0], a.out_slope), lrelu(o4[1], a.out_slope), lrelu(o4[2], a.out_slope), lrelu(o4[3], a.out_slope));
                    const float4 d = dadd[h][pa];
                    if (has_add) { o.x += d.x; o.y += d.y; o.z += d.z; o.w += d.w; }
                    if (ok[h]) {
                        if (nt_out) __builtin_nontemporal_store(f32x4_c16{o.x, o.y, o.z, o.w}, reinterpret_cast<f32x4_c16*>(a.y + idx[h][pa]));
                        else *reinterpret_cast<float4*>(a.y + idx[h][pa]) = o;
                    }
                    const float4 yq = dyq[h][pa];
                    const float okf = ok[h] ? 1.f : 0.f;
                    const f32x4_c16 ov = f32x4_c16{o.x, o.y, o.z, o.w} * okf, os = ov * a.bst_slope;
                    const int sl_ = CBf == 1 ? 0 : pa;
                    static_for_c1<NSL>([&](auto SL) {
                        constexpr int s_ = decltype(SL)::value;
                        if (sl_ == s_) {
                            const f32x4_c16 u = f32x4_c16{yq.x, yq.y, yq.z, yq.w} * bk[s_][0] + bk[s_][1];
                            f32x4_c16 dh;
#pragma unroll
                            for (int e = 0; e < 4; ++e) dh[e] = u[e] > bk[s_][2][e] ? ov[e] : os[e];
                            bs1[s_] += dh;
                            bs2[s_] += dh * u;
                        }
                    });
                }
            }
        }
    } else if constexpr (BST) {
#pragma unroll
    for (int t = 0; t < 4; ++t) {
        const size_t v = v0 + 16 * t + r;
        const bool vok = v < V;
        const size_t vc = vok ? v : V - 1;
        size_t idx[COB];
        float* ydst[COB];
        bool second[COB];
#pragma unroll
        for (int cb = 0; cb < COB; ++cb) {
            int cob = cog * COB + cb;
            if (cob >= CBo) cob = CBo - 1;
            ydst[cb] = a.y;
            second[cb] = false;
            if constexpr (S2D == 2) {
                const int tap = cob / CBf_out, cbf = cob - tap * CBf_out;
                const size_t toff = ((size_t)(tap >> 2) * Hf + ((tap >> 1) & 1)) * Wf + (tap & 1);
                idx[cb] = ((size_t)(n * CBf_out + cbf) * Vf + fv[t] + toff) * 16 + 4 * g;
            } else {
                int cbt = CBo, cl = cob;
                if (a.y1) {
                    const int CB0o = a.Cout0 >> 4;
                    second[cb] = cob >= CB0o;
                    cbt = second[cb] ? CBo - CB0o : CB0o;
                    cl = second[cb] ? cob - CB0o : cob;
                    ydst[cb] = second[cb] ? a.y1 : a.y;
                }
                idx[cb] = ((size_t)(n * cbt + cl) * V + vc) * 16 + 4 * g;
            }
        }
        float4 mq[COB], dq[COB], yq[BST ? COB : 1];
        if (a.mask) {
#pragma unroll
            for (int cb = 0; cb < COB; ++cb) mq[cb] = *reinterpret_cast<const float4*>(a.mask + ((second[cb] || !a.y1) ? idx[cb] : 0));
        }
        if (a.add) {
#pragma unroll
            for (int cb = 0; cb < COB; ++cb) dq[cb] = *reinterpret_cast<const float4*>(a.add + idx[cb]);
        }
        if constexpr (BST) {
#pragma unroll
            for (int cb = 0; cb < COB; ++cb) yq[cb] = *reinterpret_cast<const float4*>(a.bst_y + idx[cb]);
        }
#pragma unroll
        for (int cb = 0; cb < COB; ++cb) {
            if (!vok || cog * COB + cb >= CBo) continue;
            float4 o = make_float4(lrelu(acc[t][cb][0], a.out_slope), lrelu(acc[t][cb][1], a.out_slope),
                                   lrelu(acc[t][cb][2], a.out_slope), lrelu(acc[t][cb][3], a.out_slope));
            if (a.mask && (second[cb] || !a.y1)) {
                const float4 m = mq[cb];
                o.x = m.x > 0.f ? o.x : o.x * a.mask_slope; o.y = m.y > 0.f ? o.y : o.y * a.mask_slope;
                o.z = m.z > 0.f ? o.z : o.z * a.mask_slope; o.w = m.w > 0.f ? o.w : o.w * a.mask_slope;
            }
            if (a.add) { const float4 d = dq[cb]; o.x += d.x; o.y += d.y; o.z += d.z; o.w += d.w; }
            if (nt_out) __builtin_nontemporal_store(f32x4_c16{o.x, o.y, o.z, o.w}, reinterpret_cast<f32x4_c16*>(ydst[cb] + idx[cb]));
            else *reinterpret_cast<float4*>(ydst[cb] + idx[cb]) = o;
            if constexpr (BST) {
                const f32x4_c16 ov = f32x4_c16{o.x, o.y, o.z, o.w}, os = ov * a.bst_slope;
                static_for_c1<NSL>([&](auto SL) {
                    constexpr int s_ = decltype(SL)::value;
                    if (cb % NSL == s_) {
                        const f32x4_c16 u = f32x4_c16{yq[cb].x, yq[cb].y, yq[cb].z, yq[cb].w} * bk[s_][0] + bk[s_][1];
                        f32x4_c16 dh;
#pragma unroll
                        for (int e = 0; e < 4; ++e) dh[e] = u[e] > bk[s_][2][e] ? ov[e] : os[e];
                        bs1[s_] += dh;
                        bs2[s_] += dh * u;
                    }
                });
            }
        }
    }
    } else {
#pragma unroll
    for (int t = 0; t < 4; ++t) {
        const size_t v = v0 + 16 * t + r;
        if (v >= V) continue;
#pragma unroll
        for (int cb = 0; cb < COB; ++cb) {
            const int cob = cog * COB + cb;
            if (cob >= CBo) continue;
            size_t idx;
            float* ydst = a.y;
            bool second = false;
            if constexpr (S2D == 2) {
                const int tap = cob / CBf_out, cbf = cob - tap * CBf_out;
                const size_t toff = ((size_t)(tap >> 2) * Hf + ((tap >> 1) & 1)) * Wf + (tap & 1);
                idx = ((size_t)(n * CBf_out + cbf) * Vf + fv[t] + toff) * 16 + 4 * g;
            } else {
                int cbt = CBo, cl = cob;
                if (a.y1) {
                    const int CB0o = a.Cout0 >> 4;
                    second = cob >= CB0o;
                    cbt = second ? CBo - CB0o : CB0o;
                    cl = second ? cob - CB0o : cob;
                    ydst = second ? a.y1 : a.y;
                }
                idx = ((size_t)(n * cbt + cl) * V + v) * 16 + 4 * g;
            }
            float4 o = make_float4(lrelu(acc[t][cb][0], a.out_slope), lrelu(acc[t][cb][1], a.out_slope),
                                   lrelu(acc[t][cb][2], a.out_slope), lrelu(acc[t][cb][3], a.out_slope));
            if (a.mask && (second || !a.y1)) {
                const float4 m = *reinterpret_cast<const float4*>(a.mask + idx);
                o.x = m.x > 0.f ? o.x : o.x * a.mask_slope; o.y = m.y > 0.f ? o.y : o.y * a.mask_slope;
                o.z = m.z > 0.f ? o.z : o.z * a.mask_slope; o.w = m.w > 0.f ? o.w : o.w * a.mask_slope;
            }
            if (a.add) { const float4 d = *reinterpret_cast<const float4*>(a.add + idx); o.x += d.x; o.y += d.y; o.z += d.z; o.w += d.w; }
            if (nt_out) __builtin_nontemporal_store(f32x4_c16{o.x, o.y, o.z, o.w}, reinterpret_cast<f32x4_c16*>(ydst + idx));
            else *reinterpret_cast<float4*>(ydst + idx) = o;
            if constexpr (BST) {
                constexpr int sl = 0;
                (void)sl;
                const float4 yq = *reinterpret_cast<const float4*>(a.bst_y + idx);
                const f32x4_c16 ov = f32x4_c16{o.x, o.y, o.z, o.w}, os = ov * a.bst_slope;
                static_for_c1<NSL>([&](auto SL) {
                    constexpr int s_ = decltype(SL)::value;
                    if (cb % NSL == s_) {
                        const f32x4_c16 u = f32x4_c16{yq.x, yq.y, yq.z, yq.w} * bk[s_][0] + bk[s_][1];
                        f32x4_c16 dh;
#pragma unroll
                        for (int e = 0; e < 4; ++e) dh[e] = u[e] > bk[s_][2][e] ? ov[e] : os[e];
                        bs1[s_] += dh;
                        bs2[s_] += dh * u;
                    }
                });
            }
        }
    }
    }
    }
    if constexpr (BST) {
#pragma unroll
        for (int sl = 0; sl < NSL; ++sl) {
#pragma unroll
            for (int e = 0; e < 4; ++e) {
#pragma unroll
                for (int o = 1; o < 16; o <<= 1) { bs1[sl][e] += __shfl_xor(bs1[sl][e], o); bs2[sl][e] += __shfl_xor(bs2[sl][e], o); }
            }
            if (r == 0) {
#pragma unroll
                for (int e = 0; e < 4; ++e) { red[((wave * NSL + sl) * 16 + 4 * g + e) * 2] = bs1[sl][e]; red[((wave * NSL + sl) * 16 + 4 * g + e) * 2 + 1] = bs2[sl][e]; }
            }
        }
        __syncthreads();
        const int nblk = S2D == 2 ? gridDim.x * gridDim.y : gridDim.x;
        const int blk = S2D == 2 ? blockIdx.y * gridDim.x + blockIdx.x : blockIdx.x;
        for (int i = threadIdx.x; i < NSL * 16; i += 256) {
            const int slot = i >> 4, c = i & 15;
            const int cob0 = cog * COB + slot;
            if (cob0 >= CBo) continue;
            const int chb = S2D == 2 ? cob0 % CBf_out : cob0;
            float u1 = 0.f, u2 = 0.f;
#pragma unroll
            for (int w = 0; w < 4; ++w) { u1 += red[((w * NSL + slot) * 16 + c) * 2]; u2 += red[((w * NSL + slot) * 16 + c) * 2 + 1]; }
            float* p = a.stat_partials + (((size_t)n * Cstat + chb * 16 + c) * nblk + blk) * 2;
            p[0] = u1; p[1] = u2;
        }
    }
}
Conv1Inst conv1_16_choose(const Conv1Args& a) {
    const int CBo = a.Cout / 16;
    Conv1Inst c{CBo >= 4 ? 4 : (CBo >= 2 ? 2 : 1), a.s2d, 0, 0};
    if (a.s2d == 2) {
        const int forced = env_c1_scatter_cob();
        if ((forced == 2 || forced == 4 || forced == 1) && forced <= CBo) c.cob = forced;
    }
    if (a.bst_y) c.nslot = a.s2d == 2 ? (CBo >> 3) : c.cob;
    c.pair = a.s2d == 2 && a.bst_y && !env_c1_pair_off() && a.Wc % 8 == 0 && c.cob == 4 && !a.mask && (c.nslot == 1 || c.nslot == 2);
    return c;
}
int conv1_16_bst_nblk(const Conv1Args& a) {
    if (a.s2d == 1 || a.y1 || a.Cout % 16 || a.V == 0) return 0;
    const int nvt = (int)((a.V + 63) / 64), CBo = a.Cout / 16;
    const int cob = conv1_16_choose(a).cob;
    const int gx = cdiv(nvt, 4), gy = cdiv(CBo, cob);
    if (a.s2d == 2) {
        const int cbf = CBo >> 3;
        if (a.Cout % 128 || (cbf != 1 && cbf != 2 && cbf != 4) || !(cob % cbf == 0 || cbf % cob == 0)) return 0;
        if (cbf > cob) return 0;
        return gx * gy;
    }
    return gx;
}
int conv1_16_launch(const Conv1Args& a, hipStream_t s) {
    RU_REQUIRE(a.N > 0 && a.C0 > 0 && a.Cout > 0 && a.V > 0, "conv1_16: bad shape");
    RU_REQUIRE(a.C0 % 16 == 0 && a.C1 % 16 == 0 && a.Cout % 16 == 0 && a.ldw >= a.C0 + a.C1 && a.ldw % 4 == 0, "conv1_16: channels must be multiples of 16");
    RU_REQUIRE(!a.y1 || (!a.s2d && !a.add && a.Cout0 > 0 && a.Cout0 < a.Cout && a.Cout0 % 16 == 0), "conv1_16: a split output needs the plain mode, no residual and a split at a multiple of 16");
    if (a.s2d) {
        RU_REQUIRE(a.Dc > 0 && a.Hc > 0 && a.Wc > 0 && (size_t)a.Dc * a.Hc * a.Wc == a.V && a.C1 == 0, "conv1_16: bad stride-2 geometry");
        RU_REQUIRE(a.s2d == 1 ? a.C0 % 128 == 0 : a.Cout % 128 == 0, "conv1_16: stride-2 modes need 8 x (multiple of 16) channels");
    }
    const int nvt = (int)((a.V + 63) / 64), CBo = a.Cout / 16;
    const Conv1Inst c = conv1_16_choose(a);
    const bool bst = a.bst_y != nullptr;
    RU_REQUIRE(!bst || (a.bst_k && a.stat_partials && a.s2d != 1 && !a.y1 && conv1_16_bst_nblk(a) > 0), "conv1_16: fused GroupNorm-backward statistics need the plain or scatter mode with whole channel blocks per workgroup");
    dim3 grid((unsigned)cdiv(nvt, 4), (unsigned)cdiv(CBo, c.cob), (unsigned)a.N);
    switch (c.packed()) {
#define RU_C1_CASE(COB_, S2D_, NSLOT_, PAIR_)                                                                      \
    case COB_ | (S2D_ << 4) | (NSLOT_ << 8) | (PAIR_ << 12):                                                        \
        hipLaunchKernelGGL((conv1_16_kernel<COB_, S2D_, NSLOT_, PAIR_ != 0>), grid, dim3(256), 0, s, a, nvt);       \
        break
        RU_C1_CASE(4, 0, 0, 0); RU_C1_CASE(2, 0, 0, 0); RU_C1_CASE(1, 0, 0, 0);
        RU_C1_CASE(4, 0, 4, 0); RU_C1_CASE(2, 0, 2, 0); RU_C1_CASE(1, 0, 1, 0);
        RU_C1_CASE(4, 1, 0, 0); RU_C1_CASE(2, 1, 0, 0); RU_C1_CASE(1, 1, 0, 0);
        RU_C1_CASE(4, 2, 0, 0); RU_C1_CASE(2, 2, 0, 0); RU_C1_CASE(1, 2, 0, 0);
        RU_C1_CASE(4, 2, 1, 1); RU_C1_CASE(4, 2, 2, 1);
        RU_C1_CASE(4, 2, 1, 0); RU_C1_CASE(4, 2, 2, 0); RU_C1_CASE(4, 2, 4, 0);
        RU_C1_CASE(2, 2, 1, 0); RU_C1_CASE(2, 2, 2, 0); RU_C1_CASE(1, 2, 1, 0);
#undef RU_C1_CASE
    default:
        set_error("conv1_16: no kernel for cob %d, mode %d, %d statistic slots", c.cob, c.s2d, c.nslot);
        return RU_EINVAL;
    }
    RU_CHECK_LAUNCH("conv1_16_kernel");
    return RU_OK;
}

}
```

brats2019_amd/csrc/pw_helpers.hpp:

```cpp
#pragma once
#include "ru_common.h"

namespace ru {

__device__ __forceinline__ float wave_sum(float v) {
#pragma unroll
    for (int o = 32; o > 0; o >>= 1) v += __shfl_xor(v, o);
    return v;
}
__device__ __forceinline__ double wave_sum_d(double v) {
#pragma unroll
    for (int o = 32; o > 0; o >>= 1) v += __shfl_xor(v, o);
    return v;
}
__device__ __forceinline__ float block_sum(float v, float* buf) {
    v = wave_sum(v);
    __syncthreads();
    if ((threadIdx.x & 63) == 0) buf[threadIdx.x >> 6] = v;
    __syncthreads();
    return buf[0] + buf[1] + buf[2] + buf[3];
}
__device__ __forceinline__ double block_sum_d(double v, double* buf) {
    v = wave_sum_d(v);
    __syncthreads();
    if ((threadIdx.x & 63) == 0) buf[threadIdx.x >> 6] = v;
    __syncthreads();
    return buf[0] + buf[1] + buf[2] + buf[3];
}
__device__ __forceinline__ float lrelu(float v, float slope) { return v > 0.f ? v : v * slope; }

__device__ __forceinline__ float crit_grad_value(float pv, float gv, float kg, float kp, float cb, float bgw, float one_eps) {
#pragma clang fp contract(off)
    const float bce = -(gv / (pv + 1e-6f) - bgw * (1.f - gv) / (one_eps - pv));
    return __builtin_fmaf(cb, bce, __builtin_fmaf(kp, pv, kg * gv));
}

static inline unsigned grid1d(size_t n, int per_block, unsigned cap = 1u << 20) {
    size_t b = (n + per_block - 1) / per_block;
    if (b < 1) b = 1;
    return (unsigned)(b > cap ? cap : b);
}

typedef __bf16 pw_bf16x2 __attribute__((ext_vector_type(2)));
typedef unsigned int pw_u32x4 __attribute__((ext_vector_type(4)));
__device__ __forceinline__ void pw_split8(const float (&t)[8], pw_u32x4& hi, pw_u32x4& lo) {
    split_n<4>(t, hi, lo);
}

__device__ __forceinline__ void up2_src(int o, int n, int& i0, int& i1, float& l0, float& l1) {
    float src = 0.5f * (float)o - 0.25f;
    if (src < 0.f) src = 0.f;
    i0 = (int)src;
    l1 = src - (float)i0;
    l0 = 1.f - l1;
    i1 = i0 + (i0 < n - 1 ? 1 : 0);
}

__device__ __forceinline__ float up2_coef(int o, int n, int k) {
    int i0, i1; float l0, l1;
    up2_src(o, n, i0, i1, l0, l1);
    return (i0 == k ? l0 : 0.f) + (i1 == k ? l1 : 0.f);
}

}
```

brats2019_amd/csrc/ru_common.h:

```cpp
#pragma once
#include <hip/hip_runtime.h>
#include <stddef.h>
#include <stdint.h>
#include <stdio.h>
#include <stdarg.h>

#include <vector>

#include "../../include/resunet_hip.h"
#include "switches.hpp"
#include "conv3_pack_layout.hpp"

namespace ru {

typedef __bf16 ru_bf16x2 __attribute__((ext_vector_type(2)));
__device__ __forceinline__ void split_pair(float a, float b, unsigned& hb, unsigned& lb) {
    ru_bf16x2 h;
    h[0] = (__bf16)a;
    h[1] = (__bf16)b;
    hb = __builtin_bit_cast(unsigned, h);
    const float h0 = __builtin_bit_cast(float, __builtin_amdgcn_perm(hb, hb, 0x01000c0cu));
    const float h1 = __builtin_bit_cast(float, hb & 0xffff0000u);
    ru_bf16x2 l;
    l[0] = (__bf16)(a - h0);
// ... 196 lines not shown
    float* dw;
    float* db;
    void* ws;
    size_t ws_bytes;
    int N, Cin, Cout, D, H, W;
    int mode;
    int x_c16, dy_c16;
    int dw_cin, dw_cout;
    int dy_s16;
    int x_c4, dy_c4;
    const float* gb_y;
    const float* gb_d;
    const float* gb_scale;
    const float* gb_shift;
    const float* gb_coef;
    float gb_slope;
    float* gb_out;
    int gb_g16;
    int products;
    int swapped;
    struct WgradRedList* defer;
};
size_t wgrad3_workspace_bytes(int N, int Cin, int Cout, int D, int H, int W);
int wgrad3_launch(const Wgrad3Args& a, hipStream_t s);
struct WgradRedEntry { const float* partials; float* dw; int nparts, taps, CoP, CiP, Cout, Cin, so, sc, split, flip, lo, blk0; };
struct WgradRedList { std::vector<WgradRedEntry> e; };
int wgrad_reduce_launch(const float* partials, int nparts, int taps, int CoP, int CiP, int Cout, int Cin, float* dw, int so, int sc, int split, hipStream_t s,
                        int flip_taps = 0, WgradRedList* defer = nullptr);
int wgrad_reduce_flush(WgradRedList& l, hipStream_t s);
struct W3Inst { int kernel, ot, ct, x16, dy16, nbx, ntile; };
W3Inst wgrad3_inst(const Wgrad3Args& a);
W3Inst wgrad3_sb_inst(const Wgrad3Args& a);
size_t wgrad3_sb_workspace_bytes(int N, int Cin, int Cout, int D, int H, int W);
int wgrad3_sb_launch(const Wgrad3Args& a, hipStream_t s);
size_t wgrad3_tr_workspace_bytes(int N, int Cin, int Cout, int D, int H, int W);
int wgrad3_tr_launch(const Wgrad3Args& a, hipStream_t s);
int wgrad3_tr_inst(const Wgrad3Args& a);

struct Wgrad1Args {
    const float* x;
    const float* dy;
    float* dw;
    int ldw;
    void* ws;
    size_t ws_bytes;
    int N, Cin, Cout;
    size_t V;
    int c16;
    int s2d, Dc, Hc, Wc;
    int tap_split;
    const float* x1;
    int C0;
    struct WgradRedList* defer;
    const float* dg_w;
    int dg_ldw;
    float* dg_y0;
    float* dg_y1;
    float dg_mask_slope;
};
size_t wgrad1_workspace_bytes(int N, int Cin, int Cout, size_t V);
int wgrad1_launch(const Wgrad1Args& a, hipStream_t s);
int wgrad1_inst(const Wgrad1Args& a);
void wgrad1_walk(const Wgrad1Args& a, int* nbx, int* nchunk);

struct Conv1Args {
    const float* x0; int C0;
    const float* x1; int C1;
    const float* wT;
    int ldw;
    float* y;
    const float* add;
    float out_slope;
    int N, Cout;
    size_t V;
    int s2d, Dc, Hc, Wc;
    const float* mask;
    float mask_slope;
    float* y1;
    int Cout0;
    const float* bst_y;
    const float* bst_k;
    float bst_slope;
    float* stat_partials;
};
int conv1_16_bst_nblk(const Conv1Args& a);
int conv1_launch(const Conv1Args& a, hipStream_t s);
int conv1_inst(const Conv1Args& a);
int transpose_launch(const float* src, float* dst, int rows, int cols, hipStream_t s);
int layout_convert_launch(const float* src, float* dst, int N, int C, size_t V, int to_c16, hipStream_t s);
int pad_to_c16_launch(const float* src, float* dst, int N, int C, size_t V, hipStream_t s);
int pad_to_c4_launch(const float* src, float* dst, int N, int C, size_t V, hipStream_t s);

int s2d_launch(const float* x, float* y, int N, int C, int D, int H, int W, hipStream_t s);
int d2s_launch(const float* y, float* x, int N, int C, int D, int H, int W, hipStream_t s);

int gn_stats_tiles(size_t V);
int gn_stats_launch(const float* x, float* partials, int N, int C, size_t V, hipStream_t s);
int gn_finalize_launch(const float* partials, int nblk, const float* gamma, const float* beta, float* mean, float* rstd,
                       float* scale, float* shift, int N, int C, size_t V, int G, float eps, hipStream_t s, float* bst_k = nullptr,
                       bool centred = false);
int gn_apply_launch(const float* x, const float* scale, const float* shift, const float* res, float* y,
                    int N, int C, size_t V, float slope, hipStream_t s);
int gn_bwd_tiles(size_t V);
int gn_bwd_reduce_launch(const float* x, const float* dy, const float* scale, const float* shift, const float* mean,
                         const float* rstd, float slope, float* partials, int N, int C, size_t V, int G, hipStream_t s);
int gn_bwd_finalize_launch(const float* partials, int nblk, const float* gamma, const float* mean, const float* rstd,
                           float* coef, float* dgamma, float* dbeta, int N, int C, size_t V, int G, hipStream_t s, int s2_sign = 0);
bool conv3_sb_bst_usable(int N, int Cout, int D, int H, int W);
int gn_bwd_apply_launch(const float* x, const float* dy, const float* scale, const float* shift, const float* coef,
                        float slope, float* dx, int N, int C, size_t V, hipStream_t s);

int lrelu_fwd_launch(const float* x, float* y, size_t n, float slope, hipStream_t s);
int lrelu_bwd_launch(const float* y, const float* dy, float* dx, size_t n, float slope, hipStream_t s);
int sigmoid_launch(const float* x, float* y, size_t n, hipStream_t s);
int sigmoid_bwd_launch(const float* p, const float* dp, float* dz, size_t n, hipStream_t s);
int add_launch(const float* a, const float* b, float* y, size_t n, hipStream_t s);
int fill_launch(float* p, float v, size_t n, hipStream_t s);
int up2_fwd_launch(const float* x, float* y, int N, int C, int D, int H, int W, hipStream_t s);
int up2_bwd_launch(const float* dy, float* dx, int N, int C, int D, int H, int W, hipStream_t s);
int bias_grad_launch(const float* dy, float* db, int N, int C, size_t V, void* ws, size_t ws_bytes, hipStream_t s);
size_t bias_grad_workspace_bytes(int N, int C, size_t V);
int head_grad_c4_launch(const float* p, const float* dp, float* d4, float* db, int N, int C, size_t V, void* ws, size_t ws_bytes, hipStream_t s);
struct CritGradArgs { const float* target; const double* sums; double count; float w_dice, w_bce, bgw, priority; };
int head_grad_c4_crit_launch(const float* p, const CritGradArgs& cg, float* d4, float* db, int N, int C, size_t V, void* ws, size_t ws_bytes, hipStream_t s);

int gn_apply16_launch(const float* x, const float* scale, const float* shift, const float* res, float* y, int N, int C, size_t V, float slope, hipStream_t s,
                      const float* rscale = nullptr, const float* rshift = nullptr, float rslope = 1.f);
int gn_bwd_tiles16(size_t V);
int gn_bwd_reduce16_launch(const float* x, const float* dy, const float* scale, const float* shift, const float* mean, const float* rstd,
                           float slope, float* partials, int N, int C, size_t V, int G, hipStream_t s, const FinTail* fin = nullptr);
int gn_bwd_apply16_launch(const float* x, const float* dy, const float* scale, const float* shift, const float* coef, float slope, float* dx,
                          int N, int C, size_t V, int split, hipStream_t s);
int up2_fwd16_launch(const float* x, float* y, int N, int C, int D, int H, int W, float slope, hipStream_t s);
int up2_bwd16_launch(const float* dy, float* dx, int N, int C, int D, int H, int W, hipStream_t s);
int pack_down16_launch(const float* w, float* wd, float* wdT, int Cout, int Cin, hipStream_t s);
int conv1_16_launch(const Conv1Args& a, hipStream_t s);
struct Conv1Inst { int cob, s2d, nslot, pair; int packed() const { return cob | (s2d << 4) | (nslot << 8) | (pair << 12); } };
Conv1Inst conv1_16_choose(const Conv1Args& a);

int crit_tiles(size_t total);
int crit_sums_launch(const float* p, const float* g, double* sums, int N, int C, size_t V, float bgw, void* ws, size_t ws_bytes, hipStream_t s);
int crit_grad_launch(const float* p, const float* g, const double* sums, double count, float w_dice, float w_bce,
                     float bgw, float priority, float* dp, int N, int C, size_t V, hipStream_t s);
int crit_value_launch(const double* sums, int C, double count, double priority, double w_dice, double w_bce, double* out3, hipStream_t s);
int tta_merge_launch(const float* p, int K, unsigned flips, float* mean_out, unsigned char* mask, unsigned long long* counts, int C, int D, int H, int W, hipStream_t s);
int compose_labels_launch(const unsigned char* mask, const unsigned long long* counts, unsigned long long et_min, unsigned char* labels, size_t V, hipStream_t s);
int dice_counts_launch(const float* p, const float* g, unsigned long long* counts, int rows, size_t V, hipStream_t s);
int dice_accumulate_launch(const unsigned long long* counts, double* acc, int N, int C, int nacc, hipStream_t s);
constexpr int RU_AUG_MAXC = 8;
struct AugmentArgs {
    const float* image;
    const unsigned char* label;
    const float* soft;
    float* data;
    float* target;
    int C, D, H, W;
    int lo[3], P[3];
    double scale[3];
    int flags;
    float mean[RU_AUG_MAXC], istd[RU_AUG_MAXC], gain[RU_AUG_MAXC], bias[RU_AUG_MAXC];
};
size_t zscore_workspace_bytes(int C, size_t V);
int zscore_stats_launch(const float* x, double* stats, int C, size_t V, void* ws, size_t ws_bytes, hipStream_t s);
int augment_patch_launch(const AugmentArgs& a, hipStream_t s);
int adam_launch(float* w, const float* g, float* m, float* v, float* vmax, size_t n, float lr, float b1, float b2,
                float eps, float wd, int step, hipStream_t s);

}
```

brats2019_amd/csrc/switches.hpp:

```cpp
#pragma once

namespace ru {

struct Switches {
    bool wz = true, wz32 = true, mx = true, mx_wz = true, mxg = true, head_form = true, head_res = true;
    int pack_bits() const { return (wz ? 1 : 0) | (wz32 ? 2 : 0) | (mx ? 4 : 0) | (mx_wz ? 8 : 0) | (mxg ? 16 : 0); }
    bool operator==(const Switches& o) const { return pack_bits() == o.pack_bits() && head_form == o.head_form && head_res == o.head_res; }
};
Switches switches_from_env();

bool env_trace();
bool env_f32c_off();
bool env_sb1_no22();
int env_c1_scatter_cob();
bool env_c1_pair_off();
unsigned env_fusion(unsigned fusion);

}
```

brats2019_amd/ops.py:

```python
from __future__ import annotations

import collections
import ctypes as C

import torch

from . import _lib as L

LEAKY_SLOPE = 1e-2


def _dims5(x):
    if x.dim() != 5:
        raise ValueError("expected an NCDHW tensor, got shape %s" % (tuple(x.shape),))
    return [int(v) for v in x.shape]


def _prep(t):
    L.require_gpu()
    if t is None:
        return None
    return t.contiguous().float() if (not t.is_contiguous() or t.dtype != torch.float32) else t


# ... 962 lines not shown
    L.check(lib.ru_surface_metrics(L.ptr(pred), L.ptr(target), kind, n, c, d, h, w, float(empty_value), L.ptr(values), L.ptr(counts),
                                   L.ptr(ws), ws.numel(), L.stream()), "ru_surface_metrics")
    return values, counts


def surface_accumulate(values, acc, nacc, column):
    n, k = int(values.shape[0]), int(values.shape[1])
    assert values.dtype == torch.float64 and values.is_contiguous() and values.shape == (n, k, 4)
    assert acc.dtype == torch.float64 and acc.is_contiguous() and acc.numel() >= nacc
    L.check(L.load().ru_surface_accumulate(L.ptr(values), L.ptr(acc), n, k, int(nacc), L.SURFACE_COLUMNS[column], L.stream()),
            "ru_surface_accumulate")
    return acc


LESION_MAX = 1024


def lesion_metrics(pred, target, dilation=3, min_volume=50, empty_value=HD95_EMPTY, want_table=False, max_lesions=LESION_MAX):
    if tuple(pred.shape) != tuple(target.shape) or pred.dtype != target.dtype:
        raise ValueError("lesion_metrics: shapes or dtypes differ: %s %s / %s %s" % (tuple(pred.shape), pred.dtype, tuple(target.shape), target.dtype))
    if int(dilation) < 0 or int(min_volume) < 0 or int(max_lesions) < 1:
        raise ValueError("lesion_metrics: dilation %s and min_volume %s must be >= 0, max_lesions %s >= 1" % (dilation, min_volume, max_lesions))
    if pred.dtype == torch.uint8:
        if pred.dim() != 4:
            raise ValueError("lesion_metrics: uint8 label volumes are [N, D, H, W], got %s" % (tuple(pred.shape),))
        L.require_gpu()
        pred, target = pred.contiguous(), target.contiguous()
        kind, (n, d, h, w), c, k = L.SURFACE_LABEL, (int(v) for v in pred.shape), 1, L.SURFACE_REGIONS
    else:
        pred, target = _prep(pred), _prep(target)
        kind, (n, c, d, h, w) = L.SURFACE_PROB, _dims5(pred)
        k = c
    lib = L.load()
    summary = torch.empty((n, k, 2), dtype=torch.float64, device=pred.device)
    counts = torch.empty((n, k, L.LESION_COUNTS), dtype=torch.int64, device=pred.device)
    table = torch.zeros((n, k, int(max_lesions), L.LESION_TABLE_COLUMNS), dtype=torch.float64, device=pred.device) if want_table else None
    ws = L.workspace(lib.ru_lesion_workspace_bytes(kind, n, c, d, h, w, int(max_lesions)), pred.device)
    L.check(lib.ru_lesion_metrics(L.ptr(pred), L.ptr(target), kind, n, c, d, h, w, int(dilation), int(min_volume), float(empty_value),
                                  L.ptr(summary), L.ptr(counts), L.ptr(table, allow_none=True), int(max_lesions), L.ptr(ws), ws.numel(),
                                  L.stream()), "ru_lesion_metrics")
    return (summary, counts, table) if want_table else (summary, counts)


def lesion_accumulate(summary, acc, nacc, column):
    n, k = int(summary.shape[0]), int(summary.shape[1])
    assert summary.dtype == torch.float64 and summary.is_contiguous() and summary.shape == (n, k, 2)
    assert acc.dtype == torch.float64 and acc.is_contiguous() and acc.numel() >= nacc
    L.check(L.load().ru_lesion_accumulate(L.ptr(summary), L.ptr(acc), n, k, int(nacc), L.LESION_COLUMNS[column], L.stream()),
            "ru_lesion_accumulate")
    return acc


def to_c16(x):
    x = _prep(x)
    n, c, d, h, w = _dims5(x)
    y = torch.empty((n, c // 16, d, h, w, 16), dtype=torch.float32, device=x.device)
    L.check(L.load().ru_layout_convert(L.f32(x), L.f32(y), n, c, d * h * w, 1, L.stream()), "ru_layout_convert")
    return y


def from_c16(x):
    x = _prep(x)
    n, cb, d, h, w, _ = (int(v) for v in x.shape)
    y = torch.empty((n, cb * 16, d, h, w), dtype=torch.float32, device=x.device)
    L.check(L.load().ru_layout_convert(L.f32(x), L.f32(y), n, cb * 16, d * h * w, 0, L.stream()), "ru_layout_convert")
    return y


def upsample2x_c16(x, out_slope=1.0, out=None):
    x = _prep(x)
    n, cb, d, h, w, _ = (int(v) for v in x.shape)
    y = _out(out, (n, cb, 2 * d, 2 * h, 2 * w, 16), x.device)
    L.check(L.load().ru_upsample2x_trilinear_fwd_l(L.f32(x), L.f32(y), n, cb * 16, d, h, w, float(out_slope), L.stream()),
            "ru_upsample2x_trilinear_fwd_l")
    return y


def upsample2x_bwd_c16(dy, out=None):
    dy = _prep(dy)
    n, cb, d2, h2, w2, _ = (int(v) for v in dy.shape)
    dx = _out(out, (n, cb, d2 // 2, h2 // 2, w2 // 2, 16), dy.device)
    L.check(L.load().ru_upsample2x_trilinear_bwd_l(L.f32(dy), L.f32(dx), n, cb * 16, d2 // 2, h2 // 2, w2 // 2, L.stream()),
            "ru_upsample2x_trilinear_bwd_l")
    return dx


def to_split_c16(x_c16):
    hi = x_c16.to(torch.bfloat16)
    lo = (x_c16 - hi.to(torch.float32)).to(torch.bfloat16)
    return torch.cat([hi, lo], dim=-1).contiguous().view(torch.float32)


def conv3d_layout(x, w, bias=None, in_c16=False, out_c16=False, few_channels=False, in_split=False, exact_f32=False, activations=False, gradient=False):
    x, w, bias = _prep(x), _prep(w), _prep(bias)
    if in_c16:
        n, cb, d, h, wd, _ = (int(v) for v in x.shape)
        cin = cb * 16
    else:
        n, cin, d, h, wd = _dims5(x)
    cout = int(w.shape[0])
    y = torch.empty((n, cout // 16, d, h, wd, 16) if out_c16 else (n, cout, d, h, wd), dtype=torch.float32, device=x.device)
    lib = L.load()
    flags = int(in_c16) | (int(out_c16) << 1) | (int(few_channels) << 2) | (int(in_split) << 3) | (int(exact_f32) << 4) | (int(activations) << 5) | (int(gradient) << 6)
    ws = L.workspace(lib.ru_conv3_l_workspace_bytes(n, cin, cout, d, h, wd, flags), x.device)
    L.check(lib.ru_conv3d_fwd_l(L.f32(x), L.f32(w), L.ptr(bias, True), L.f32(y), n, cin, cout, d, h, wd, flags, L.ptr(ws), ws.numel(), L.stream()), "ru_conv3d_fwd_l")
    return y


def conv3d_bwd_weight_layout(x, dy, x_c16=False, dy_c16=False, out=None):
    x, dy = _prep(x), _prep(dy)
    if x_c16:
        n, cb, d, h, wd, _ = (int(v) for v in x.shape)
        cin = cb * 16
    else:
        n, cin, d, h, wd = _dims5(x)
    cout = int(dy.shape[1]) * 16 if dy_c16 else int(dy.shape[1])
    dw = _out(out, (cout, cin, 3, 3, 3), x.device)
    lib = L.load()
    ws = L.workspace(lib.ru_conv3d_workspace_bytes(n, cin, cout, d, h, wd, 3), x.device)
    L.check(lib.ru_conv3d_bwd_weight_l(L.f32(x), L.f32(dy), L.f32(dw), n, cin, cout, d, h, wd, int(x_c16) | (int(dy_c16) << 1),
                                       L.ptr(ws), ws.numel(), L.stream()), "ru_conv3d_bwd_weight_l")
    return dw


Conv1Result = collections.namedtuple("Conv1Result", "y y1 partials nblk inst")
Wgrad1Result = collections.namedtuple("Wgrad1Result", "dw dx0 dx1 inst")


def conv1_inst(packed):
    return packed & 15, (packed >> 4) & 15, (packed >> 8) & 15, bool((packed >> 12) & 1)


def wgrad1_inst(packed):
    return packed & 15, (packed >> 4) & 15, bool(packed & 256), bool(packed & 512)


def conv1x1_c16(x0, w, x1=None, add=None, out_slope=1.0, mask=None, mask_slope=LEAKY_SLOPE, cout0=0, s2d=0,
                bst_y=None, bst_k=None, bst_slope=LEAKY_SLOPE):
    x0, w, x1, add, mask, bst_y, bst_k = (_prep(t) for t in (x0, w, x1, add, mask, bst_y, bst_k))
    lib = L.load()
    n, cb0, d, h, wd, _ = (int(v) for v in x0.shape)
    c0, c1 = cb0 * 16, (int(x1.shape[1]) * 16 if x1 is not None else 0)
    dc, hc, wc, ldw = d, h, wd, 0
    if s2d == 0:
        cout, ldw = int(w.shape[0]), int(w.shape[1])
        out_sp, cstat = (d, h, wd), cout
    elif s2d == 1:
        cout, c0 = int(w.shape[0]), 8 * c0
        dc, hc, wc = d // 2, h // 2, wd // 2
        out_sp, cstat = (dc, hc, wc), cout
    else:
        cout = 8 * int(w.shape[1])
        out_sp, cstat = (2 * d, 2 * h, 2 * wd), cout // 8
    v = dc * hc * wc
    dev = x0.device
    y1 = None
    if cout0:
        y = torch.empty((n, cout0 // 16) + (d, h, wd) + (16,), dtype=torch.float32, device=dev)
        y1 = torch.empty((n, (cout - cout0) // 16) + (d, h, wd) + (16,), dtype=torch.float32, device=dev)
    else:
        y = torch.empty((n, cstat // 16) + out_sp + (16,), dtype=torch.float32, device=dev)
    part, cap = None, 0
    if bst_y is not None:
        cap = n * cstat * ((v + 255) // 256) * max(cout // 16, 1) * 2
        part = torch.zeros(cap, dtype=torch.float32, device=dev)
    ws = L.workspace(lib.ru_conv1_l_workspace_bytes(c0, cout, s2d), dev)
    nblk, inst = C.c_int(0), C.c_int(0)
    L.check(lib.ru_conv1_l(L.f32(x0), c0, L.ptr(x1, True), c1, L.f32(w), ldw, L.f32(y), L.ptr(y1, True), cout0, L.ptr(add, True), float(out_slope),
                           L.ptr(mask, True), float(mask_slope), n, cout, v, s2d, dc, hc, wc, L.ptr(bst_y, True), L.ptr(bst_k, True), float(bst_slope),
                           L.ptr(part, True), cap, C.byref(nblk), C.byref(inst), L.ptr(ws), ws.numel(), L.stream()), "ru_conv1_l")
    if part is not None:
        part = part[:n * cstat * nblk.value * 2].view(n, cstat, nblk.value, 2)
    return Conv1Result(y, y1, part, nblk.value, inst.value)


def conv1x1_bwd_weight_c16(x, dy, x1=None, ldw=None, s2d=False, tap_split=False, dg_w=None, dg_mask_slope=LEAKY_SLOPE):
    x, dy, x1, dg_w = (_prep(t) for t in (x, dy, x1, dg_w))
    lib = L.load()
    n, cbo, d, h, wd, _ = (int(v) for v in dy.shape)
    c0 = int(x.shape[1]) * 16
    cin = 8 * c0 if s2d else c0 + (int(x1.shape[1]) * 16 if x1 is not None else 0)
    cout, v = cbo * 16, d * h * wd
    ldw = cin if ldw is None else int(ldw)
    dev = x.device
    dw = torch.zeros((cout, cin // 8, 2, 2, 2) if tap_split else (cout, ldw), dtype=torch.float32, device=dev)
    dx0 = torch.empty_like(x) if dg_w is not None else None
    dx1 = torch.empty_like(x1) if dg_w is not None and x1 is not None else None
    ws = L.workspace(lib.ru_wgrad1_l_workspace_bytes(n, cin, cout, v), dev)
    inst = C.c_int(0)
    L.check(lib.ru_wgrad1_l(L.f32(x), L.ptr(x1, True), c0 if x1 is not None else 0, L.f32(dy), L.f32(dw), ldw, n, cin, cout, v, 1, int(bool(s2d)), d, h, wd,
                            cin // 8 if tap_split else 0, L.ptr(dg_w, True), int(dg_w.shape[1]) if dg_w is not None else 0, L.ptr(dx0, True), L.ptr(dx1, True),
                            float(dg_mask_slope), C.byref(inst), L.ptr(ws), ws.numel(), L.stream()), "ru_wgrad1_l")
    return Wgrad1Result(dw, dx0, dx1, inst.value)


Conv3Result = collections.namedtuple("Conv3Result", "y in_sum partials nblk route fin", defaults=(None,))
GnStats = collections.namedtuple("GnStats", "mean rstd scale shift bst_k")
GnBwdCoef = collections.namedtuple("GnBwdCoef", "coef dgamma dbeta")
GnBwdResult = collections.namedtuple("GnBwdResult", "dx dgamma dbeta coef partials")
Conv3Route = collections.namedtuple("Conv3Route", "family tz ty in16 out16 multi bst add np head grad")
CONV3_FAMILIES = {1: "sb", 2: "sb2", 3: "sb2c4", 4: "wz32", 5: "wz32mx", 6: "mx", 7: "f32c", 8: "wz16"}


def conv3_route(packed):
    bit = lambda b: bool((packed >> b) & 1)
    return Conv3Route(CONV3_FAMILIES.get(packed & 15, "none"), (packed >> 4) & 15, (packed >> 8) & 15, bit(12), bit(13), bit(14), bit(15), bit(16),
                      (packed >> 20) & 3, bit(17), bit(18))


def conv3_fused(x, w, bias=None, in_c16=False, out_c16=False, few_channels=False, in_split=False, exact_f32=False, activations=False, gradient=False,
                add=None, in_scale=None, in_shift=None, in_slope=LEAKY_SLOPE, in_res=None, in_sum_out=None, sigmoid=False, products=0,
                bst_y=None, bst_k=None, bst_slope=LEAKY_SLOPE, stats=None, weight_mode=0, pack_training=False, y=None,
                tail=0, tail_gamma=None, tail_beta=None, tail_mean=None, tail_rstd=None, tail_want_k=False, tail_s2_sign=1, tail_groups=8, tail_eps=1e-5,
                tail_override=None, tail_workspace=None, tail_keep_ticket=False):
    x, w, bias, add, in_scale, in_shift, in_res, bst_y, bst_k = (_prep(t) for t in (x, w, bias, add, in_scale, in_shift, in_res, bst_y, bst_k))
    if in_c16:
        n, cb, d, h, wd, _ = (int(v) for v in x.shape)
        cin = cb * 16
    else:
        n, cin, d, h, wd = _dims5(x)
    cout = int(w.shape[1 if weight_mode else 0])
    dev = x.device
    if y is None:
        y = torch.empty((n, cout // 16, d, h, wd, 16) if out_c16 else (n, cout, d, h, wd), dtype=torch.float32, device=dev)
    if in_sum_out is True:
        in_sum_out = torch.full_like(x, float("nan"))
    part, cap = None, 0
    if stats is None:
        stats = bst_y is not None
    if stats:
        cap = n * cout * max(((d + 1) // 2) * ((h + 1) // 2) * ((wd + 15) // 16), 1024) * 2
        part = torch.full((cap,), float("nan"), dtype=torch.float32, device=dev)
    flags = (int(in_c16) | (int(out_c16) << 1) | (int(few_channels) << 2) | (int(in_split) << 3) | (int(exact_f32) << 4) | (int(activations) << 5)
             | (int(gradient) << 6) | (int(pack_training) << 7))
    lib = L.load()
    fd, fin = None, None
    if tail:
        tail_gamma, tail_beta, tail_mean, tail_rstd = (_prep(t) for t in (tail_gamma, tail_beta, tail_mean, tail_rstd))
        new = lambda *shape: torch.full(shape, float("nan"), dtype=torch.float32, device=dev)
        fd = L.FinDesc(kind=int(tail), G=int(tail_groups), s2_sign=int(tail_s2_sign), keep_ticket=int(bool(tail_keep_ticket)), eps=float(tail_eps),
                       gamma=L.f32(tail_gamma), **{k: int(v) for k, v in (tail_override or {}).items()})
        if tail == 1:
            fin = GnStats(new(n * tail_groups), new(n * tail_groups), new(n, cout), new(n, cout), new(n, 3, cout) if tail_want_k else None)
            fd.beta, fd.mean, fd.rstd, fd.scale, fd.shift, fd.bst_k = (L.ptr(t, True) for t in (tail_beta,) + tuple(fin))
        else:
            fin = GnBwdCoef(new(n, cout, 3), new(cout), new(cout))
            fd.mean, fd.rstd, fd.coef, fd.dgamma, fd.dbeta = (L.ptr(t, True) for t in (tail_mean, tail_rstd) + tuple(fin))
    ws = tail_workspace if tail_workspace is not None else L.workspace(lib.ru_conv3_l_workspace_bytes(n, cin, cout, d, h, wd, flags | (256 if tail else 0)), dev)
    nblk, route = C.c_int(0), C.c_int(0)
    L.check(lib.ru_conv3_l(L.f32(x), L.f32(w), L.ptr(bias, True), L.f32(y), n, cin, cout, d, h, wd, flags, int(weight_mode), L.ptr(add, True),
                           L.ptr(in_scale, True), L.ptr(in_shift, True), float(in_slope), L.ptr(in_res, True), L.ptr(in_sum_out, True), int(bool(sigmoid)),
                           int(products), L.ptr(bst_y, True), L.ptr(bst_k, True), float(bst_slope), L.ptr(part, True), cap, C.byref(nblk), C.byref(route),
                           L.ptr(ws), ws.numel(), L.stream(), C.byref(fd) if fd is not None else None), "ru_conv3_l")
    if part is not None:
        part = part[:n * cout * nblk.value * 2].view(n, cout, nblk.value, 2)
    return Conv3Result(y, in_sum_out, part, nblk.value, route.value, (fin, ws) if fin is not None else None)


def _c16_dims(x):
    n, cb, d, h, w, _ = (int(v) for v in x.shape)
    return n, cb * 16, d * h * w


def gn_finalize(partials, gamma, beta, V, centred=False, want_k=False, groups=8, eps=1e-5):
    partials, gamma, beta = _prep(partials), _prep(gamma), _prep(beta)
    n, c, nblk, _ = (int(v) for v in partials.shape)
    new = lambda *shape: torch.full(shape, float("nan"), dtype=torch.float32, device=partials.device)
    r = GnStats(new(n * groups), new(n * groups), new(n, c), new(n, c), new(n, 3, c) if want_k else None)
    L.check(L.load().ru_gn_finalize_l(L.f32(partials), nblk, L.f32(gamma), L.f32(beta), L.f32(r.mean), L.f32(r.rstd), L.f32(r.scale), L.f32(r.shift),
                                      L.ptr(r.bst_k, True), n, c, int(V), int(groups), float(eps), int(bool(centred)), L.stream()), "ru_gn_finalize_l")
    return r


def gn_apply_c16(x, scale, shift, slope, res=None, res_scale=None, res_shift=None, res_slope=1.0):
    x, scale, shift, res, res_scale, res_shift = (_prep(t) for t in (x, scale, shift, res, res_scale, res_shift))
    n, c, v = _c16_dims(x)
    y = torch.full_like(x, float("nan"))
    L.check(L.load().ru_gn_apply_l(L.f32(x), L.f32(scale), L.f32(shift), L.ptr(res, True), L.ptr(res_scale, True), L.ptr(res_shift, True), L.f32(y), n, c, v,
# ... 64 lines not shown
```

include/resunet_hip.h:

```cpp
#ifndef RESUNET_HIP_H_
#define RESUNET_HIP_H_

#include <stddef.h>
#include <stdint.h>

#ifdef __cplusplus
extern "C" {
#endif

#define RU_OK 0
#define RU_EINVAL (-1)
#define RU_ENOMEM (-2)
#define RU_EHIP (-3)
#define RU_ESTATE (-4)

#define RU_PREC_F32 0
#define RU_PREC_BF16X3 1
#define RU_PREC_BF16 2

typedef void* ru_stream_t;
typedef struct ru_unet* ru_unet_t;

const char* ru_last_error(void);
int ru_version(void);
// ... 188 lines not shown
int ru_comm_init(ru_comm_t* out, const void* id, int rank, int world);
int ru_comm_destroy(ru_comm_t c);
int ru_comm_rank(ru_comm_t c);
int ru_comm_world(ru_comm_t c);
int ru_allreduce(ru_comm_t c, void* buf, size_t count, int dtype, ru_stream_t stream);
int ru_comm_group_begin(void);
int ru_comm_group_end(void);

int ru_tta_merge(const float* probs, int K, unsigned flips, float* mean_out, unsigned char* mask, unsigned long long* counts,
                 int C, int D, int H, int W, ru_stream_t stream);
int ru_compose_labels(const unsigned char* mask, const unsigned long long* counts, unsigned long long et_min, unsigned char* labels,
                      size_t V, ru_stream_t stream);

int ru_tile_gather(const float* data, float* tiles, int N, int C, int D, int H, int W, int T, const int* origins,
                   int td, int th, int tw, ru_stream_t stream);
int ru_tile_scatter(const float* tiles, float* out, int N, int C, int D, int H, int W, int T, const int* origins,
                    int td, int th, int tw, const int* border, const int* center, ru_stream_t stream);
int ru_blend_accumulate(const float* tiles, float* acc, const float* profiles, int N, int C, int D, int H, int W, int td, int th, int tw,
                        const int* starts_z, int nz, const int* starts_y, int ny, const int* starts_x, int nx, int t0, int T, ru_stream_t stream);
int ru_blend_finalize(const float* acc, float* out, const float* profiles, int N, int C, int D, int H, int W, int td, int th, int tw,
                      const int* starts_z, int nz, const int* starts_y, int ny, const int* starts_x, int nx, ru_stream_t stream);
int ru_case_bbox(const float* image, int* box, int C, int D, int H, int W, ru_stream_t stream);
size_t ru_case_workspace_bytes(int C, int D, int H, int W);
int ru_case_stats(const float* image, double* stats, int C, int D, int H, int W, const int* lo, const int* size,
                  void* ws, size_t ws_bytes, ru_stream_t stream);
int ru_case_prepare(const float* image, const double* stats, float* batch, int C, int D, int H, int W, const int* lo, const int* size,
                    const int* pad_left, const int* padded, int K, unsigned flips, ru_stream_t stream);
int ru_tta_merge_box(const float* probs, int K, unsigned flips, float* mean_out, unsigned char* mask, unsigned long long* counts,
                     int C, int D, int H, int W, const int* lo, const int* size, ru_stream_t stream);
size_t ru_cc_workspace_bytes(int D, int H, int W);
int ru_cc_reject(unsigned char* labels, int D, int H, int W, double ratio, void* ws, size_t ws_bytes, ru_stream_t stream);
int ru_paste_labels(const unsigned char* lab, unsigned char* full, int D, int H, int W, const int* lo, const int* size, ru_stream_t stream);

#define RU_POSTPROCESS_MASKS 0
#define RU_POSTPROCESS_LABELS 1
#define RU_POSTPROCESS_REGIONS 3
#define RU_POSTPROCESS_STATS 6
#define RU_POSTPROCESS_S_FOUND 0
#define RU_POSTPROCESS_S_VOLUME 1
#define RU_POSTPROCESS_S_CONFIDENCE 2
#define RU_POSTPROCESS_S_LARGEST 3
#define RU_POSTPROCESS_S_FILLED 4
#define RU_POSTPROCESS_S_INVALID 5
size_t ru_postprocess_workspace_bytes(int kind, int D, int H, int W);
int ru_postprocess_regions(const void* in, const float* probs, int kind, int D, int H, int W, const long long* min_volume,
                           const unsigned long long* conf_thr, unsigned keep_largest_bits, unsigned fill_holes_bits, int nest,
                           unsigned char* out, unsigned long long* counts, long long* stats, void* ws, size_t ws_bytes, ru_stream_t stream);

int ru_ens_accumulate(const float* probs, int K, unsigned flips, float* acc, int first, int C, int D, int H, int W, const int* lo, const int* size,
                      ru_stream_t stream);
int ru_ens_finalize(const float* acc, int M, float* mean_out, unsigned char* mask, unsigned long long* counts, int C, size_t Vbox, ru_stream_t stream);
int ru_ens_accumulate_finalize(const float* probs, int K, unsigned flips, const float* acc, int first, int M, float* mean_out, unsigned char* mask,
                               unsigned long long* counts, int C, int D, int H, int W, const int* lo, const int* size, ru_stream_t stream);
int ru_ens_argmax(const float* acc, int M, unsigned char* labels, int C, size_t V, ru_stream_t stream);
int ru_paste_probs(const float* mean, float* full, int C, int D, int H, int W, const int* lo, const int* size, ru_stream_t stream);

#define RU_UNC_STD 0
#define RU_UNC_ENTROPY 1
#define RU_UNC_TP 0
#define RU_UNC_FP 1
#define RU_UNC_FN 2
#define RU_UNC_TN 3
int ru_unc_accumulate(const float* probs, int K, unsigned flips, float* acc, float* acc2, int first, int C, int D, int H, int W, const int* lo,
                      const int* size, ru_stream_t stream);
int ru_unc_accumulate_finalize(const float* probs, int K, unsigned flips, const float* acc, const float* acc2, int first, int M, int measure,
                               float* mean_out, unsigned char* mask, unsigned long long* counts, unsigned char* unc, int C, int D, int H, int W,
                               const int* lo, const int* size, ru_stream_t stream);
int ru_unc_finalize(const float* acc, const float* acc2, int M, int K, int measure, float* mean_out, unsigned char* mask, unsigned long long* counts,
                    unsigned char* unc, int C, size_t Vbox, ru_stream_t stream);
int ru_unc_histogram(const unsigned char* pred, const unsigned char* target, const unsigned char* unc, int D, int H, int W, unsigned long long* hist,
                     unsigned long long* invalid, ru_stream_t stream);
int ru_unc_score(const unsigned long long* hist, const int* thresholds, int T, double* out, double* acc, ru_stream_t stream);
int ru_paste_u8c(const unsigned char* src, unsigned char* full, int C, int D, int H, int W, const int* lo, const int* size, ru_stream_t stream);

int ru_layout_convert(const float* src, float* dst, int N, int C, size_t V, int to_c16, ru_stream_t stream);
int ru_conv3d_fwd_l(const float* x, const float* w, const float* bias, float* y,
                    int N, int Cin, int Cout, int D, int H, int W, int flags,
                    void* ws, size_t ws_bytes, ru_stream_t stream);
int ru_conv3d_bwd_weight_l(const float* x, const float* dy, float* dw,
                           int N, int Cin, int Cout, int D, int H, int W, int flags,
                           void* ws, size_t ws_bytes, ru_stream_t stream);

size_t ru_conv1_l_workspace_bytes(int C0, int Cout, int s2d);
int ru_conv1_l(const float* x0, int C0, const float* x1, int C1, const float* w, int ldw, float* y, float* y1, int Cout0,
               const float* add, float out_slope, const float* mask, float mask_slope, int N, int Cout, size_t V,
               int s2d, int Dc, int Hc, int Wc, const float* bst_y, const float* bst_k, float bst_slope,
               float* stat_partials, size_t stat_floats, int* nblk, int* inst, void* ws, size_t ws_bytes, ru_stream_t stream);
typedef struct ru_fin_desc {
    int kind, G, s2_sign, keep_ticket;
    float eps;
    int nblk, N, C;
    const float* gamma;
    const float* beta;
    float* mean;
    float* rstd;
    float* scale;
    float* shift;
    float* bst_k;
    float* coef;
    float* dgamma;
    float* dbeta;
} ru_fin_desc;
size_t ru_conv3_l_workspace_bytes(int N, int Cin, int Cout, int D, int H, int W, int flags);
int ru_conv3_l(const float* x, const float* w, const float* bias, float* y, int N, int Cin, int Cout, int D, int H, int W, int flags, int weight_mode,
               const float* add, const float* in_scale, const float* in_shift, float in_slope, const float* in_res, float* in_sum_out,
               int sigmoid, int products, const float* bst_y, const float* bst_k, float bst_slope, float* stat_partials, size_t stat_floats,
               int* nblk, int* route, void* ws, size_t ws_bytes, ru_stream_t stream, const ru_fin_desc* fin);

int ru_gn_finalize_l(const float* partials, int nblk, const float* gamma, const float* beta, float* mean, float* rstd, float* scale, float* shift, float* bst_k,
                     int N, int C, size_t V, int G, float eps, int centred, ru_stream_t stream);
int ru_gn_apply_l(const float* x, const float* scale, const float* shift, const float* res, const float* res_scale, const float* res_shift, float* y,
                  int N, int C, size_t V, float slope, float res_slope, ru_stream_t stream);
int ru_gn_bwd_finalize_l(const float* partials, int nblk, const float* gamma, const float* mean, const float* rstd, float* coef, float* dgamma, float* dbeta,
                         int N, int C, size_t V, int G, int s2_sign, ru_stream_t stream);
int ru_gn_bwd_l_nblk(size_t V);
size_t ru_gn_bwd_l_workspace_bytes(int N, int C, size_t V);
int ru_gn_bwd_l(const float* x, const float* dact, const float* gamma, const float* scale, const float* shift, const float* mean, const float* rstd, float slope,
                float* dx, float* dgamma, float* dbeta, float* coef_out, float* partials_out, int N, int C, size_t V, int G, int flags,
                void* ws, size_t ws_bytes, ru_stream_t stream);
size_t ru_head_grad_l_workspace_bytes(int N, int C, size_t V, int route);
int ru_head_grad_l(const float* p, const float* dp, const float* target, const double* sums, double count, float w_dice, float w_bce, float bg_weight,
                   float priority, float* d4, float* db, float* dlog, int N, int C, size_t V, int route, void* ws, size_t ws_bytes, ru_stream_t stream);
size_t ru_wgrad1_l_workspace_bytes(int N, int Cin, int Cout, size_t V);
int ru_wgrad1_l(const float* x, const float* x1, int C0, const float* dy, float* dw, int ldw, int N, int Cin, int Cout, size_t V,
                int c16, int s2d, int Dc, int Hc, int Wc, int tap_split, const float* dg_w, int dg_ldw, float* dg_y0, float* dg_y1,
                float dg_mask_slope, int* inst, void* ws, size_t ws_bytes, ru_stream_t stream);
size_t ru_wgrad3_l_workspace_bytes(int N, int Cin, int Cout, int D, int H, int W, int flags);
int ru_wgrad3_l(const float* x, const float* dy, float* dw, int N, int Cin, int Cout, int D, int H, int W, int flags, int products,
                const float* in_scale, const float* in_shift, float in_slope, int dw_cin, int dw_cout,
                const float* gb_y, const float* gb_d, const float* gb_scale, const float* gb_shift, const float* gb_coef, float gb_slope, float* gb_out,
                int* inst, void* ws, size_t ws_bytes, ru_stream_t stream);

int ru_upsample2x_trilinear_fwd_l(const float* x, float* y, int N, int C, int D, int H, int W, float out_slope, ru_stream_t stream);
int ru_upsample2x_trilinear_bwd_l(const float* dy, float* dx, int N, int C, int D, int H, int W, ru_stream_t stream);

int ru_dice_counts(const float* p, const float* g, unsigned long long* counts, int N, int C, size_t V, ru_stream_t stream);
int ru_dice_accumulate(const unsigned long long* counts, double* acc, int N, int C, int nacc, ru_stream_t stream);

size_t ru_hausdorff_workspace_bytes(int N, int C, int D, int H, int W, int mode);
int ru_hausdorff_sq(const float* p, const float* g, int N, int C, int D, int H, int W, int mode, unsigned long long* out,
                    void* ws, size_t ws_bytes, ru_stream_t stream);
int ru_hausdorff_accumulate(const unsigned long long* sq, double* acc, int N, int K, int nacc, int mode, ru_stream_t stream);

#define RU_CONF_PROB 0
#define RU_CONF_LABEL 1
#define RU_OVERLAP_MAX_LABELS 8
#define RU_OVERLAP_ITK 0
#define RU_OVERLAP_WT 1
#define RU_OVERLAP_VALIDATE 2
int ru_label_confusion(const void* pred, const void* target, int kind, int N, int C, size_t V, unsigned long long* conf,
                       unsigned long long* invalid, ru_stream_t stream);
int ru_overlap_accumulate(const unsigned long long* conf, int N, int L, int mode, int nacc, double* acc, double* out, ru_stream_t stream);
int ru_dice1d_accumulate(const unsigned long long* counts, double* acc, int N, int C, int classes, ru_stream_t stream);
int ru_rmse_accumulate(const double* sums, double* acc, ru_stream_t stream);

#define RU_SURFACE_PROB 0
#define RU_SURFACE_LABEL 1
#define RU_SURFACE_REGIONS 3
#define RU_SURFACE_DICE 0
#define RU_SURFACE_SENS 1
#define RU_SURFACE_SPEC 2
#define RU_SURFACE_HD95 3
#define RU_SURFACE_COUNTS 6
#define RU_SURFACE_C_INVALID 5
size_t ru_surface_workspace_bytes(int kind, int N, int C, int D, int H, int W);
int ru_surface_metrics(const void* pred, const void* target, int kind, int N, int C, int D, int H, int W, double empty_value,
                       double* values, unsigned long long* counts, void* ws, size_t ws_bytes, ru_stream_t stream);
int ru_surface_accumulate(const double* values, double* acc, int N, int K, int nacc, int column, ru_stream_t stream);

#define RU_LESION_DICE 0
#define RU_LESION_HD95 1
#define RU_LESION_COUNTS 6
#define RU_LESION_C_INVALID 5
#define RU_LESION_COLUMNS 5
#define RU_LESION_CHUNK 8
size_t ru_lesion_workspace_bytes(int kind, int N, int C, int D, int H, int W, int max_lesions);
int ru_lesion_metrics(const void* pred, const void* target, int kind, int N, int C, int D, int H, int W, int dilation, long long min_volume,
                      double empty_value, double* summary, unsigned long long* counts, double* table, int max_lesions, void* ws,
                      size_t ws_bytes, ru_stream_t stream);
int ru_lesion_accumulate(const double* summary, double* acc, int N, int K, int nacc, int column, ru_stream_t stream);

size_t ru_zscore_workspace_bytes(int C, size_t V);
int ru_zscore_stats(const float* image, double* stats, int C, size_t V, void* ws, size_t ws_bytes, ru_stream_t stream);
int ru_augment_patch(const float* image, const unsigned char* label, const float* mean, const float* inv_std,
                     int C, int D, int H, int W, const int* crop_lo, const int* patch, const double* scale, int flags,
                     const float* gain, const float* bias, float* data_out, float* target_out, ru_stream_t stream);
int ru_augment_patch_soft(const float* image, const unsigned char* label, const float* soft, const float* mean, const float* inv_std,
                          int C, int D, int H, int W, const int* crop_lo, const int* patch, const double* scale, int flags,
                          const float* gain, const float* bias, float* data_out, float* target_out, ru_stream_t stream);

#define RU_AFFINE_MAP_DEFAULT 0
#define RU_AFFINE_MAP_ROW 1
#define RU_AFFINE_MAP_BRICK 2
int ru_augment_patch_affine(const float* image, const unsigned char* label, const float* soft, const float* mean, const float* inv_std,
                            int C, int D, int H, int W, const int* patch, const double* matrix, const double* offset, int flags,
                            const float* gain, const float* bias, int mapping, float* data_out, float* target_out, ru_stream_t stream);

size_t ru_elastic_workspace_bytes(int P0, int P1, int P2);
int ru_elastic_noise(unsigned long long seed, int P0, int P1, int P2, double* noise_out, ru_stream_t stream);
int ru_elastic_field(const double* noise, double sigma, double alpha, int P0, int P1, int P2, double* disp_out, void* ws, size_t ws_bytes,
                     ru_stream_t stream);
int ru_elastic_warp(const float* data_in, int C, const float* target_in, int T, const double* disp, int P0, int P1, int P2, int flags,
                    const float* gain, const float* bias, float* data_out, float* target_out, ru_stream_t stream);

#define RU_INT_BLUR 1
#define RU_INT_LOWRES 2
#define RU_INT_NOISE 4
#define RU_INT_BRIGHTNESS 8
#define RU_INT_CONTRAST 16
#define RU_INT_GAMMA 32
#define RU_INT_GAMMA_INVERT 64
#define RU_INT_GAMMA_RETAIN 128
typedef struct ru_intensity_params {
    int mask[8];
    double blur_sigma[8];
    double lowres_zoom[8];
    double noise_variance[8];
// ... 46 lines not shown
```

Baseline: 272.6.

## Fuse trilinear upsample into decoder 1x1 conv and tile upsample backward

In inference mode, the first two decoder levels now compute the trilinear 2x upsample inside the 1x1 conv kernel, interpolating the coarse source on the fly instead of writing and re-reading a full-resolution buffer. The upsample backward kernel gains a patch mapping (4x16 spatial tiles) plus a block-index swizzle across groups of eight, and this mapping is on by default. The patch mapping is meant to improve locality of the fine-gradient reads and balance work across the chip's compute partitions. The cost is wasted threads on partial tiles and more kernel template variants.

```diff
diff --git a/brats2019_amd/_lib.py b/brats2019_amd/_lib.py
--- a/brats2019_amd/_lib.py
+++ b/brats2019_amd/_lib.py
@@ -171,6 +171,9 @@
     "ru_layout_convert": (_i, [_vp, _vp, _i, _i, _sz, _i, _vp]),
     "ru_upsample2x_trilinear_fwd_l": (_i, [_vp, _vp] + [_i] * 5 + [_f, _vp]),
     "ru_upsample2x_trilinear_bwd_l": (_i, [_vp, _vp] + [_i] * 5 + [_vp]),
+    "ru_upsample2x_trilinear_bwd_map_l": (_i, [_vp, _vp] + [_i] * 6 + [_vp]),
+    "ru_conv1_up_l_workspace_bytes": (_sz, [_i, _i, _i]),
+    "ru_conv1_up_l": (_i, [_vp, _i, _vp, _i, _vp, _i, _vp, _vp, _f] + [_i] * 5 + [_f, C.POINTER(_i), _vp, _sz, _vp]),
     "ru_conv3d_fwd_l": (_i, [_vp, _vp, _vp, _vp] + [_i] * 7 + [_vp, _sz, _vp]),
     "ru_conv3d_bwd_weight_l": (_i, [_vp, _vp, _vp] + [_i] * 7 + [_vp, _sz, _vp]),
     "ru_conv1_l_workspace_bytes": (_sz, [_i, _i, _i]),
diff --git a/brats2019_amd/csrc/engine.hip b/brats2019_amd/csrc/engine.hip
--- a/brats2019_amd/csrc/engine.hip
+++ b/brats2019_amd/csrc/engine.hip
@@ -38,6 +38,7 @@
     sw.mxg = !env_is("RU_MXG", '0');
     sw.head_form = !env_is("RU_HEAD_FORM", '0');
     sw.head_res = !env_is("RU_HEAD_RES", '0');
+    sw.upfuse = !env_is("RU_UPFUSE", '0');
     return sw;
 }
 bool env_trace() { static const bool on = [] { const char* e = getenv("RU_TRACE"); return e && *e && *e != '0'; }(); return on; }
@@ -159,6 +160,8 @@
     const float* skip = nullptr;
     int level = 0;
 };
+
+constexpr int kUpFuseLevels = 2;
 
 constexpr int kOneProduct = 0x100;
 struct ru_unet {
@@ -229,6 +232,8 @@
     }
 };
 
+static bool up_fused(const ru_unet* h, int level) { return h->c16 && h->sw.upfuse && !h->training && level < kUpFuseLevels; }
+
 static int add_param(ru_unet* h, const std::string& name, std::initializer_list<int> dims, bool dead = false) {
     ParamInfo p;
     p.name = name;
@@ -677,7 +682,8 @@
             ds.u = A.alloc((size_t)N * Cc * Vl(i));
             RU_RUN(up2_fwd_launch(cur, ds.u, N, Cc, Dl[i + 1], Hl[i + 1], Wl[i + 1], s));
         }
-        ds.v = A.alloc((size_t)N * Ci * Vl(i));
+        const bool upf = up_fused(h, i);
+        ds.v = upf ? nullptr : A.alloc((size_t)N * Ci * Vl(i));
         Conv1Args c1{};
         c1.x0 = ds.u; c1.C0 = Cc; c1.y = ds.v; c1.out_slope = kSlope;
         c1.N = N; c1.Cout = Ci; c1.V = Vl(i);
@@ -690,7 +696,11 @@
             c1.x0 = cur; c1.y = zc; c1.out_slope = 1.f; c1.V = Vl(i + 1);
             c1.wT = P(h, params, h->up_w[i]); c1.ldw = Cc;
             RU_RUN(conv1_16_launch(c1, s));
-            RU_RUN(up2_fwd16_launch(zc, ds.v, N, Ci, Dl[i + 1], Hl[i + 1], Wl[i + 1], kSlope, s));
+            if (upf) {
+                c2.x1 = nullptr; c2.up_src = zc; c2.up_D = Dl[i + 1]; c2.up_H = Hl[i + 1]; c2.up_W = Wl[i + 1]; c2.up_slope = kSlope;
+            } else {
+                RU_RUN(up2_fwd16_launch(zc, ds.v, N, Ci, Dl[i + 1], Hl[i + 1], Wl[i + 1], kSlope, s));
+            }
             c2.wT = P(h, params, h->dec1_w[i]); c2.ldw = 2 * Ci;
             RU_RUN(conv1_16_launch(c2, s));
         } else {
@@ -1239,6 +1249,8 @@
 static int backward_entry(ru_unet_t h, const float* params, const float* dprobs, const CritGradArgs* crit, float* grads, float* dx, ru_stream_t stream) {
     if (!h->have_fwd || !h->training) { set_error("ru_unet_backward: needs a preceding training-mode ru_unet_forward"); return RU_ESTATE; }
     h->sw = switches_from_env();
+    RU_REQUIRE(h->pack_sw.upfuse == h->sw.upfuse, "ru_unet_backward: RU_UPFUSE changed since the forward this backward belongs to (%d then, %d now)",
+               (int)h->pack_sw.upfuse, (int)h->sw.upfuse);
     RU_REQUIRE(h->precision != RU_PREC_BF16X3 || h->pack_sw.pack_bits() == h->sw.pack_bits(),
                "ru_unet_backward: RU_WZ / RU_MX / RU_MXG changed since the forward whose packs this backward reads (signature %d then, %d now)", h->pack_sw.pack_bits(), h->sw.pack_bits());
     Arena A;
diff --git a/brats2019_amd/csrc/op_abi.hip b/brats2019_amd/csrc/op_abi.hip
--- a/brats2019_amd/csrc/op_abi.hip
+++ b/brats2019_amd/csrc/op_abi.hip
@@ -355,6 +355,11 @@
     return up2_bwd16_launch(dy, dx, N, C, D, H, W, (hipStream_t)stream);
 }
 
+extern "C" int ru_upsample2x_trilinear_bwd_map_l(const float* dy, float* dx, int N, int C, int D, int H, int W, int patch, ru_stream_t stream) {
+    RU_REQUIRE(dy && dx && N > 0 && C > 0 && D > 0 && H > 0 && W > 0 && (patch == 0 || patch == 1), "ru_upsample2x_trilinear_bwd_map_l: bad argument");
+    return up2_bwd16_launch(dy, dx, N, C, D, H, W, (hipStream_t)stream, patch);
+}
+
 static void fill_fin(FinTail& f, const ru_fin_desc& d, unsigned* ticket, int nblk, int N, int C, size_t V) {
     f.ticket = ticket; f.kind = d.kind; f.nblk = d.nblk ? d.nblk : nblk; f.N = d.N ? d.N : N; f.C = d.C ? d.C : C; f.G = d.G; f.V = V; f.eps = d.eps; f.s2_sign = d.s2_sign;
     f.gamma = d.gamma; f.beta = d.beta; f.mean = d.mean; f.rstd = d.rstd; f.scale = d.scale; f.shift = d.shift; f.bst_k = d.bst_k;
@@ -610,6 +615,23 @@
     return walk_result(A, conv1_l_walk(a, w, stat_floats, nblk, inst, A, (hipStream_t)stream));
 }
 
+extern "C" size_t ru_conv1_up_l_workspace_bytes(int C0, int C1, int Cout) {
+    Conv1Args a{};
+    a.C0 = C0; a.C1 = C1; a.Cout = Cout;
+    return kSlack + dry_need([&](Arena& A) { return conv1_l_walk(a, nullptr, 0, nullptr, nullptr, A, nullptr); });
+}
+extern "C" int ru_conv1_up_l(const float* x0, int C0, const float* up_src, int C1, const float* w, int ldw, float* y, const float* add, float out_slope,
+                             int N, int Cout, int up_D, int up_H, int up_W, float up_slope, int* inst, void* ws, size_t ws_bytes, ru_stream_t stream) {
+    RU_REQUIRE(x0 && up_src && w && y, "ru_conv1_up_l: null argument");
+    RU_REQUIRE(N > 0 && up_D > 0 && up_H > 0 && up_W > 0, "ru_conv1_up_l: bad shape");
+    Conv1Args a{};
+    a.x0 = x0; a.C0 = C0; a.C1 = C1; a.wT = w; a.ldw = ldw; a.y = y; a.add = add; a.out_slope = out_slope;
+    a.N = N; a.Cout = Cout; a.V = (size_t)up_D * up_H * up_W * 8;
+    a.up_src = up_src; a.up_D = up_D; a.up_H = up_H; a.up_W = up_W; a.up_slope = up_slope;
+    Arena A = arena_over(ws, ws_bytes);
+    return walk_result(A, conv1_l_walk(a, w, 0, nullptr, inst, A, (hipStream_t)stream));
+}
+
 static int wgrad1_l_walk(Wgrad1Args a, int* inst, Arena& A, hipStream_t s) {
     a.ws_bytes = wgrad1_workspace_bytes(a.N, a.Cin, a.Cout, a.V);
     a.ws = A.alloc(a.ws_bytes / 4);
diff --git a/brats2019_amd/csrc/pointwise_c16.hip b/brats2019_amd/csrc/pointwise_c16.hip
--- a/brats2019_amd/csrc/pointwise_c16.hip
+++ b/brats2019_amd/csrc/pointwise_c16.hip
@@ -221,7 +221,7 @@
         const int ky = (int)(r % (H + 1)) - 1;
         const int kz = (int)(r / (H + 1)) - 1;
         int x0, x1; float lx0, lx1;
-        up2_src(xo, W, x0, x1, lx0, lx1);
+        up2_cell(xo, W, x0, x1, lx0, lx1);
         const int zA = kz < 0 ? 0 : kz, zB = kz + 1 > D - 1 ? D - 1 : kz + 1;
         const int yA = ky < 0 ? 0 : ky, yB = ky + 1 > H - 1 ? H - 1 : ky + 1;
         const size_t rAA = ((size_t)zA * H + yA) * W, rAB = ((size_t)zA * H + yB) * W, rBA = ((size_t)zB * H + yA) * W, rBB = ((size_t)zB * H + yB) * W;
@@ -229,26 +229,20 @@
         const float4 a01 = xp[(rAB + x0) * 4 + q], b01 = xp[(rAB + x1) * 4 + q];
         const float4 a10 = xp[(rBA + x0) * 4 + q], b10 = xp[(rBA + x1) * 4 + q];
         const float4 a11 = xp[(rBB + x0) * 4 + q], b11 = xp[(rBB + x1) * 4 + q];
-        float4 e00, e01, e10, e11;
-#define RU_UPX(c) e00.c = lx0 * a00.c + lx1 * b00.c; e01.c = lx0 * a01.c + lx1 * b01.c; e10.c = lx0 * a10.c + lx1 * b10.c; e11.c = lx0 * a11.c + lx1 * b11.c
-        RU_UPX(x); RU_UPX(y); RU_UPX(z); RU_UPX(w);
-#undef RU_UPX
+        const float4 e00 = up2_lerp4(lx0, a00, lx1, b00), e01 = up2_lerp4(lx0, a01, lx1, b01), e10 = up2_lerp4(lx0, a10, lx1, b10), e11 = up2_lerp4(lx0, a11, lx1, b11);
 #pragma unroll
         for (int dz = 0; dz < 2; ++dz) {
             const int zo = 2 * kz + 1 + dz;
             if (zo < 0 || zo >= Do) continue;
             int z0, z1; float lz0, lz1;
-            up2_src(zo, D, z0, z1, lz0, lz1);
+            up2_cell(zo, D, z0, z1, lz0, lz1);
 #pragma unroll
             for (int dy = 0; dy < 2; ++dy) {
                 const int yo = 2 * ky + 1 + dy;
                 if (yo < 0 || yo >= Ho) continue;
                 int y0, y1; float ly0, ly1;
-                up2_src(yo, H, y0, y1, ly0, ly1);
-                float4 o;
-#define RU_UP2(c) o.c = lrelu(lz0 * (ly0 * e00.c + ly1 * e01.c) + lz1 * (ly0 * e10.c + ly1 * e11.c), slope)
-                RU_UP2(x); RU_UP2(y); RU_UP2(z); RU_UP2(w);
-#undef RU_UP2
+                up2_cell(yo, H, y0, y1, ly0, ly1);
+                const float4 o = up2_zy4(lz0, lz1, ly0, ly1, e00, e01, e10, e11, slope);
                 if (nt_out) __builtin_nontemporal_store(f32x4_c16{o.x, o.y, o.z, o.w}, reinterpret_cast<f32x4_c16*>(yp + (((size_t)zo * Ho + yo) * Wo + xo) * 4 + q));
                 else yp[(((size_t)zo * Ho + yo) * Wo + xo) * 4 + q] = o;
             }
@@ -269,20 +263,33 @@
 #define RU_UP2B_ZC 8
 #endif
 constexpr int UP2B_ZC = RU_UP2B_ZC;
-__global__ __launch_bounds__(256) void up2_bwd16_kernel(const float* __restrict__ dy, float* __restrict__ dx, int D, int H, int W) {
+constexpr int UP2B_PY = 4, UP2B_PX = 16;
+__global__ __launch_bounds__(256) void up2_bwd16_kernel(const float* __restrict__ dy, float* __restrict__ dx, int D, int H, int W, int patch) {
     const int Do = 2 * D, Ho = 2 * H, Wo = 2 * W;
     const size_t nb = blockIdx.y;
     const size_t Vi = (size_t)D * H * W, Vo = Vi * 8;
     const float4* dp = reinterpret_cast<const float4*>(dy) + nb * Vo * 4;
     float4* op = reinterpret_cast<float4*>(dx) + nb * Vi * 4;
     const int nch = (D + UP2B_ZC - 1) / UP2B_ZC;
-    const size_t total = (size_t)nch * H * W * 4;
-    for (size_t f = (size_t)blockIdx.x * 256 + threadIdx.x; f < total; f += (size_t)gridDim.x * 256) {
+    const int npx = (W + UP2B_PX - 1) / UP2B_PX, npy = (H + UP2B_PY - 1) / UP2B_PY;
+    const size_t total = patch ? (size_t)nch * npy * npx * 256 : (size_t)nch * H * W * 4;
+    const size_t lb = patch ? (size_t)(blockIdx.x & 7) * (gridDim.x >> 3) + (blockIdx.x >> 3) : (size_t)blockIdx.x;
+    for (size_t f = lb * 256 + threadIdx.x; f < total; f += (size_t)gridDim.x * 256) {
         const int q = (int)(f & 3);
         size_t r = f >> 2;
-        const int kx = (int)(r % W); r /= W;
-        const int ky = (int)(r % H);
-        const int k0 = (int)(r / H) * UP2B_ZC;
+        int kx, ky, k0;
+        if (patch) {
+            const int lx = (int)(r % UP2B_PX); r /= UP2B_PX;
+            const int ly = (int)(r % UP2B_PY); r /= UP2B_PY;
+            kx = (int)(r % npx) * UP2B_PX + lx; r /= npx;
+            ky = (int)(r % npy) * UP2B_PY + ly;
+            k0 = (int)(r / npy) * UP2B_ZC;
+            if (kx >= W || ky >= H) continue;
+        } else {
+            kx = (int)(r % W); r /= W;
+            ky = (int)(r % H);
+            k0 = (int)(r / H) * UP2B_ZC;
+        }
         const int k1 = k0 + UP2B_ZC < D ? k0 + UP2B_ZC : D;
         float wy[4], wx[4];
         size_t oy[4], ox[4];
@@ -322,12 +329,14 @@
         }
     }
 }
-int up2_bwd16_launch(const float* dy, float* dx, int N, int C, int D, int H, int W, hipStream_t s) {
+int up2_bwd16_launch(const float* dy, float* dx, int N, int C, int D, int H, int W, hipStream_t s, int patch) {
     RU_REQUIRE(C % 16 == 0, "up2_bwd16: C must be a multiple of 16");
-    const size_t total = (size_t)((D + UP2B_ZC - 1) / UP2B_ZC) * H * W * 4;
+    const size_t nch = (size_t)((D + UP2B_ZC - 1) / UP2B_ZC);
+    const size_t total = patch ? nch * ((H + UP2B_PY - 1) / UP2B_PY) * ((W + UP2B_PX - 1) / UP2B_PX) * 256 : nch * H * W * 4;
     size_t bx = (total + 255) / 256;
+    if (patch) bx = (bx + 7) / 8 * 8;
     if (bx > 16384) bx = 16384;
-    hipLaunchKernelGGL(up2_bwd16_kernel, dim3((unsigned)bx, (unsigned)(N * (C / 16))), dim3(256), 0, s, dy, dx, D, H, W);
+    hipLaunchKernelGGL(up2_bwd16_kernel, dim3((unsigned)bx, (unsigned)(N * (C / 16))), dim3(256), 0, s, dy, dx, D, H, W, patch);
     RU_CHECK_LAUNCH("up2_bwd16_kernel");
     return RU_OK;
 }
@@ -347,9 +356,10 @@
     return RU_OK;
 }
 
-template <int COB, int S2D, int NSLOT, bool PAIR = false>
+template <int COB, int S2D, int NSLOT, bool PAIR = false, bool UPF = false>
 __global__ __launch_bounds__(256, (PAIR || NSLOT > 0) ? 2 : 1) void conv1_16_kernel(const Conv1Args a, int nvt) {
     static_assert(!PAIR || (S2D == 2 && COB == 4 && (NSLOT == 1 || NSLOT == 2)), "paired stores: the scatter mode with statistics, four blocks per workgroup");
+    static_assert(!UPF || (S2D == 0 && NSLOT == 0 && !PAIR), "interpolated second input: the plain mode without statistics");
     constexpr bool BST = NSLOT > 0;
     constexpr int NSL = BST ? NSLOT : 1;
     __shared__ float red[BST ? 4 * NSL * 16 * 2 : 1];
@@ -380,9 +390,42 @@
     if (live) {
     const size_t v0 = (size_t)vt * 64;
     size_t vb[4], fv[4];
+    size_t uvx[UPF ? 4 : 1];
+    bool uok[UPF ? 4 : 1];
+    unsigned ucn[UPF ? 8 : 1];
+    float ulx0 = 0.f, ulx1 = 0.f, ulz0[2] = {0.f, 0.f}, ulz1[2] = {0.f, 0.f}, uly0[2] = {0.f, 0.f}, uly1[2] = {0.f, 0.f};
+    if constexpr (UPF) {
+        const int Dc = a.up_D, Hc = a.up_H, Wc = a.up_W, Do = 2 * Dc, Ho = 2 * Hc, Wo = 2 * Wc;
+        const int nx16 = (Wo + 15) >> 4;
+        const int xs = vt % nx16, rz = vt / nx16;
+        const int ky = rz % (Hc + 1) - 1, kz = rz / (Hc + 1) - 1;
+        const int xo_raw = xs * 16 + r, xo = xo_raw < Wo ? xo_raw : Wo - 1;
+        int xA, xB;
+        up2_cell(xo, Wc, xA, xB, ulx0, ulx1);
+        const int zA = kz < 0 ? 0 : kz, zB = kz + 1 > Dc - 1 ? Dc - 1 : kz + 1;
+        const int yA = ky < 0 ? 0 : ky, yB = ky + 1 > Hc - 1 ? Hc - 1 : ky + 1;
+        const unsigned rAA = (unsigned)((zA * Hc + yA) * Wc), rAB = (unsigned)((zA * Hc + yB) * Wc), rBA = (unsigned)((zB * Hc + yA) * Wc), rBB = (unsigned)((zB * Hc + yB) * Wc);
+        ucn[0] = (rAA + xA) * 4 + g; ucn[1] = (rAA + xB) * 4 + g; ucn[2] = (rAB + xA) * 4 + g; ucn[3] = (rAB + xB) * 4 + g;
+        ucn[4] = (rBA + xA) * 4 + g; ucn[5] = (rBA + xB) * 4 + g; ucn[6] = (rBB + xA) * 4 + g; ucn[7] = (rBB + xB) * 4 + g;
+#pragma unroll
+        for (int d = 0; d < 2; ++d) {
+            const int zo = 2 * kz + 1 + d, yo = 2 * ky + 1 + d;
+            int i0, i1;
+            up2_cell(zo < 0 ? 0 : zo, Dc, i0, i1, ulz0[d], ulz1[d]);
+            up2_cell(yo < 0 ? 0 : yo, Hc, i0, i1, uly0[d], uly1[d]);
+        }
+#pragma unroll
+        for (int t = 0; t < 4; ++t) {
+            const int zo = 2 * kz + 1 + (t >> 1), yo = 2 * ky + 1 + (t & 1);
+            uok[t] = zo >= 0 && zo < Do && yo >= 0 && yo < Ho && xo_raw < Wo;
+            const int zc = zo < 0 ? 0 : (zo >= Do ? Do - 1 : zo), yc = yo < 0 ? 0 : (yo >= Ho ? Ho - 1 : yo);
+            uvx[t] = ((size_t)zc * Ho + yc) * Wo + xo;
+        }
+    }
 #pragma unroll
     for (int t = 0; t < 4; ++t) {
         size_t v = v0 + 16 * t + r;
+        if constexpr (UPF) v = uvx[t];
         if (v >= V) v = V - 1;
         vb[t] = v * 16 + 4 * g;
         fv[t] = 0;
@@ -413,8 +456,14 @@
             const float* src = a.x0 + ((size_t)(n * CBf_in + cbf) * Vf) * 16 + 4 * g;
 #pragma unroll
             for (int t = 0; t < 4; ++t) xb[t] = *reinterpret_cast<const float4*>(src + (fv[t] + toff) * 16);
+        } else if (UPF && kb >= nkb0) {
+            const float4* cp = reinterpret_cast<const float4*>(a.up_src) + (size_t)(n * nkb1 + kb - nkb0) * ((size_t)a.up_D * a.up_H * a.up_W) * 4;
+            const float4 a00 = cp[ucn[0]], b00 = cp[ucn[1]], a01 = cp[ucn[2]], b01 = cp[ucn[3]], a10 = cp[ucn[4]], b10 = cp[ucn[5]], a11 = cp[ucn[6]], b11 = cp[ucn[7]];
+            const float4 e00 = up2_lerp4(ulx0, a00, ulx1, b00), e01 = up2_lerp4(ulx0, a01, ulx1, b01), e10 = up2_lerp4(ulx0, a10, ulx1, b10), e11 = up2_lerp4(ulx0, a11, ulx1, b11);
+#pragma unroll
+            for (int t = 0; t < 4; ++t) xb[t] = up2_zy4(ulz0[t >> 1], ulz1[t >> 1], uly0[t & 1], uly1[t & 1], e00, e01, e10, e11, a.up_slope);
         } else {
-            const float* src = kb < nkb0 ? a.x0 + ((size_t)(n * nkb0 + kb) * V) * 16 : a.x1 + ((size_t)(n * nkb1 + kb - nkb0) * V) * 16;
+            const float* src = (UPF || kb < nkb0) ? a.x0 + ((size_t)(n * nkb0 + kb) * V) * 16 : a.x1 + ((size_t)(n * nkb1 + kb - nkb0) * V) * 16;
 #pragma unroll
             for (int t = 0; t < 4; ++t) xb[t] = *reinterpret_cast<const float4*>(src + vb[t]);
         }
@@ -577,7 +626,8 @@
     } else {
 #pragma unroll
     for (int t = 0; t < 4; ++t) {
-        const size_t v = v0 + 16 * t + r;
+        size_t v = v0 + 16 * t + r;
+        if constexpr (UPF) { v = uvx[t]; if (!uok[t]) continue; }
         if (v >= V) continue;
 #pragma unroll
         for (int cb = 0; cb < COB; ++cb) {
@@ -670,6 +720,7 @@
     }
     if (a.bst_y) c.nslot = a.s2d == 2 ? (CBo >> 3) : c.cob;
     c.pair = a.s2d == 2 && a.bst_y && !env_c1_pair_off() && a.Wc % 8 == 0 && c.cob == 4 && !a.mask && (c.nslot == 1 || c.nslot == 2);
+    c.upf = a.up_src ? 1 : 0;
     return c;
 }
 int conv1_16_bst_nblk(const Conv1Args& a) {
@@ -693,7 +744,14 @@
         RU_REQUIRE(a.Dc > 0 && a.Hc > 0 && a.Wc > 0 && (size_t)a.Dc * a.Hc * a.Wc == a.V && a.C1 == 0, "conv1_16: bad stride-2 geometry");
         RU_REQUIRE(a.s2d == 1 ? a.C0 % 128 == 0 : a.Cout % 128 == 0, "conv1_16: stride-2 modes need 8 x (multiple of 16) channels");
     }
-    const int nvt = (int)((a.V + 63) / 64), CBo = a.Cout / 16;
+    int nvt = (int)((a.V + 63) / 64);
+    const int CBo = a.Cout / 16;
+    if (a.up_src) {
+        RU_REQUIRE(!a.s2d && !a.x1 && a.C1 > 0 && !a.bst_y && !a.y1, "conv1_16: an interpolated second input needs the plain mode, no second tensor, no statistics and one output");
+        RU_REQUIRE(a.up_D > 0 && a.up_H > 0 && a.up_W > 0 && (size_t)a.up_D * a.up_H * a.up_W * 8 == a.V && a.V * 4 < ((size_t)1 << 31),
+                   "conv1_16: the interpolated input's coarse extents must be half the output's");
+        nvt = (a.up_D + 1) * (a.up_H + 1) * ((2 * a.up_W + 15) / 16);
+    }
     const Conv1Inst c = conv1_16_choose(a);
     const bool bst = a.bst_y != nullptr;
     RU_REQUIRE(!bst || (a.bst_k && a.stat_partials && a.s2d != 1 && !a.y1 && conv1_16_bst_nblk(a) > 0), "conv1_16: fused GroupNorm-backward statistics need the plain or scatter mode with whole channel blocks per workgroup");
@@ -711,6 +769,12 @@
         RU_C1_CASE(4, 2, 1, 0); RU_C1_CASE(4, 2, 2, 0); RU_C1_CASE(4, 2, 4, 0);
         RU_C1_CASE(2, 2, 1, 0); RU_C1_CASE(2, 2, 2, 0); RU_C1_CASE(1, 2, 1, 0);
 #undef RU_C1_CASE
+#define RU_C1_CASE_UP(COB_)                                                                                        \
+    case COB_ | (1 << 13):                                                                                          \
+        hipLaunchKernelGGL((conv1_16_kernel<COB_, 0, 0, false, true>), grid, dim3(256), 0, s, a, nvt);              \
+        break
+        RU_C1_CASE_UP(4); RU_C1_CASE_UP(2); RU_C1_CASE_UP(1);
+#undef RU_C1_CASE_UP
     default:
         set_error("conv1_16: no kernel for cob %d, mode %d, %d statistic slots", c.cob, c.s2d, c.nslot);
         return RU_EINVAL;
diff --git a/brats2019_amd/csrc/pw_helpers.hpp b/brats2019_amd/csrc/pw_helpers.hpp
--- a/brats2019_amd/csrc/pw_helpers.hpp
+++ b/brats2019_amd/csrc/pw_helpers.hpp
@@ -56,6 +56,24 @@
     i1 = i0 + (i0 < n - 1 ? 1 : 0);
 }
 
+__device__ __forceinline__ void up2_cell(int o, int n, int& kA, int& kB, float& l0, float& l1) {
+    const int k = ((o + 1) >> 1) - 1;
+    kA = k < 0 ? 0 : k;
+    kB = k + 1 > n - 1 ? n - 1 : k + 1;
+    int i0, i1;
+    up2_src(o, n, i0, i1, l0, l1);
+}
+__device__ __forceinline__ float up2_lerp(float l0, float a, float l1, float b) { return __fmaf_rn(l1, b, __fmul_rn(l0, a)); }
+__device__ __forceinline__ float4 up2_lerp4(float l0, const float4& a, float l1, const float4& b) {
+    return make_float4(up2_lerp(l0, a.x, l1, b.x), up2_lerp(l0, a.y, l1, b.y), up2_lerp(l0, a.z, l1, b.z), up2_lerp(l0, a.w, l1, b.w));
+}
+__device__ __forceinline__ float4 up2_zy4(float lz0, float lz1, float ly0, float ly1, const float4& e00, const float4& e01, const float4& e10, const float4& e11,
+                                          float slope) {
+    const float4 fA = up2_lerp4(ly0, e00, ly1, e01), fB = up2_lerp4(ly0, e10, ly1, e11);
+    const float4 o = up2_lerp4(lz0, fA, lz1, fB);
+    return make_float4(lrelu(o.x, slope), lrelu(o.y, slope), lrelu(o.z, slope), lrelu(o.w, slope));
+}
+
 __device__ __forceinline__ float up2_coef(int o, int n, int k) {
     int i0, i1; float l0, l1;
     up2_src(o, n, i0, i1, l0, l1);
diff --git a/brats2019_amd/csrc/ru_common.h b/brats2019_amd/csrc/ru_common.h
--- a/brats2019_amd/csrc/ru_common.h
+++ b/brats2019_amd/csrc/ru_common.h
@@ -302,6 +302,9 @@
     const float* bst_k;
     float bst_slope;
     float* stat_partials;
+    const float* up_src;
+    int up_D, up_H, up_W;
+    float up_slope;
 };
 int conv1_16_bst_nblk(const Conv1Args& a);
 int conv1_launch(const Conv1Args& a, hipStream_t s);
@@ -352,10 +355,10 @@
 int gn_bwd_apply16_launch(const float* x, const float* dy, const float* scale, const float* shift, const float* coef, float slope, float* dx,
                           int N, int C, size_t V, int split, hipStream_t s);
 int up2_fwd16_launch(const float* x, float* y, int N, int C, int D, int H, int W, float slope, hipStream_t s);
-int up2_bwd16_launch(const float* dy, float* dx, int N, int C, int D, int H, int W, hipStream_t s);
+int up2_bwd16_launch(const float* dy, float* dx, int N, int C, int D, int H, int W, hipStream_t s, int patch = 1);
 int pack_down16_launch(const float* w, float* wd, float* wdT, int Cout, int Cin, hipStream_t s);
 int conv1_16_launch(const Conv1Args& a, hipStream_t s);
-struct Conv1Inst { int cob, s2d, nslot, pair; int packed() const { return cob | (s2d << 4) | (nslot << 8) | (pair << 12); } };
+struct Conv1Inst { int cob, s2d, nslot, pair; int upf = 0; int packed() const { return cob | (s2d << 4) | (nslot << 8) | (pair << 12) | (upf << 13); } };
 Conv1Inst conv1_16_choose(const Conv1Args& a);
 
 int crit_tiles(size_t total);
diff --git a/brats2019_amd/csrc/switches.hpp b/brats2019_amd/csrc/switches.hpp
--- a/brats2019_amd/csrc/switches.hpp
+++ b/brats2019_amd/csrc/switches.hpp
@@ -4,8 +4,9 @@
 
 struct Switches {
     bool wz = true, wz32 = true, mx = true, mx_wz = true, mxg = true, head_form = true, head_res = true;
+    bool upfuse = true;
     int pack_bits() const { return (wz ? 1 : 0) | (wz32 ? 2 : 0) | (mx ? 4 : 0) | (mx_wz ? 8 : 0) | (mxg ? 16 : 0); }
-    bool operator==(const Switches& o) const { return pack_bits() == o.pack_bits() && head_form == o.head_form && head_res == o.head_res; }
+    bool operator==(const Switches& o) const { return pack_bits() == o.pack_bits() && head_form == o.head_form && head_res == o.head_res && upfuse == o.upfuse; }
 };
 Switches switches_from_env();
 
diff --git a/brats2019_amd/ops.py b/brats2019_amd/ops.py
--- a/brats2019_amd/ops.py
+++ b/brats2019_amd/ops.py
@@ -1068,6 +1068,15 @@
     dx = _out(out, (n, cb, d2 // 2, h2 // 2, w2 // 2, 16), dy.device)
     L.check(L.load().ru_upsample2x_trilinear_bwd_l(L.f32(dy), L.f32(dx), n, cb * 16, d2 // 2, h2 // 2, w2 // 2, L.stream()),
             "ru_upsample2x_trilinear_bwd_l")
+    return dx
+
+
+def upsample2x_bwd_c16_mapped(dy, patch):
+    dy = _prep(dy)
+    n, cb, d2, h2, w2, _ = (int(v) for v in dy.shape)
+    dx = torch.empty((n, cb, d2 // 2, h2 // 2, w2 // 2, 16), dtype=torch.float32, device=dy.device)
+    L.check(L.load().ru_upsample2x_trilinear_bwd_map_l(L.f32(dy), L.f32(dx), n, cb * 16, d2 // 2, h2 // 2, w2 // 2, int(patch), L.stream()),
+            "ru_upsample2x_trilinear_bwd_map_l")
     return dx
 
 
@@ -1180,6 +1189,20 @@
     return Wgrad1Result(dw, dx0, dx1, inst.value)
 
 
+def conv1x1_up_c16(x0, w, up_src, add=None, out_slope=1.0, up_slope=LEAKY_SLOPE):
+    x0, w, up_src, add = (_prep(t) for t in (x0, w, up_src, add))
+    lib = L.load()
+    n, cb1, d, h, wd, _ = (int(v) for v in up_src.shape)
+    c0, c1, cout, ldw = int(x0.shape[1]) * 16, cb1 * 16, int(w.shape[0]), int(w.shape[1])
+    assert tuple(x0.shape[2:5]) == (2 * d, 2 * h, 2 * wd) and int(x0.shape[0]) == n
+    y = torch.empty((n, cout // 16, 2 * d, 2 * h, 2 * wd, 16), dtype=torch.float32, device=x0.device)
+    ws = L.workspace(lib.ru_conv1_up_l_workspace_bytes(c0, c1, cout), x0.device)
+    inst = C.c_int(0)
+    L.check(lib.ru_conv1_up_l(L.f32(x0), c0, L.f32(up_src), c1, L.f32(w), ldw, L.f32(y), L.ptr(add, True), float(out_slope), n, cout, d, h, wd, float(up_slope),
+                              C.byref(inst), L.ptr(ws), ws.numel(), L.stream()), "ru_conv1_up_l")
+    return Conv1Result(y, None, None, 0, inst.value)
+
+
 Conv3Result = collections.namedtuple("Conv3Result", "y in_sum partials nblk route fin", defaults=(None,))
 GnStats = collections.namedtuple("GnStats", "mean rstd scale shift bst_k")
 GnBwdCoef = collections.namedtuple("GnBwdCoef", "coef dgamma dbeta")
diff --git a/include/resunet_hip.h b/include/resunet_hip.h
--- a/include/resunet_hip.h
+++ b/include/resunet_hip.h
@@ -294,6 +294,10 @@
                            void* ws, size_t ws_bytes, ru_stream_t stream);
 
 size_t ru_conv1_l_workspace_bytes(int C0, int Cout, int s2d);
+size_t ru_conv1_up_l_workspace_bytes(int C0, int C1, int Cout);
+int ru_conv1_up_l(const float* x0, int C0, const float* up_src, int C1, const float* w, int ldw, float* y, const float* add, float out_slope,
+                  int N, int Cout, int up_D, int up_H, int up_W, float up_slope, int* inst, void* ws, size_t ws_bytes, ru_stream_t stream);
+
 int ru_conv1_l(const float* x0, int C0, const float* x1, int C1, const float* w, int ldw, float* y, float* y1, int Cout0,
                const float* add, float out_slope, const float* mask, float mask_slope, int N, int Cout, size_t V,
                int s2d, int Dc, int Hc, int Wc, const float* bst_y, const float* bst_k, float bst_slope,
@@ -345,6 +349,7 @@
 
 int ru_upsample2x_trilinear_fwd_l(const float* x, float* y, int N, int C, int D, int H, int W, float out_slope, ru_stream_t stream);
 int ru_upsample2x_trilinear_bwd_l(const float* dy, float* dx, int N, int C, int D, int H, int W, ru_stream_t stream);
+int ru_upsample2x_trilinear_bwd_map_l(const float* dy, float* dx, int N, int C, int D, int H, int W, int patch, ru_stream_t stream);
 
 int ru_dice_counts(const float* p, const float* g, unsigned long long* counts, int N, int C, size_t V, ru_stream_t stream);
 int ru_dice_accumulate(const unsigned long long* counts, double* acc, int N, int C, int nacc, ru_stream_t stream);
```

After: 274.1, median of 4. About the same (+0.6%).
